# bruniss/multi-task-3d-resencoder-unet

Hardware: AMD Instinct MI355X
Metric: train patches/sec (b,c,z,y,x) ResEncM 1x128^3 (higher is better)
Workload: dtype bf16; 1 GPU; cfg2: ResEncM (6 stages, feats [32, 64, 128, 256, 512, 512], blocks [1, 3, 4, 6, 6, 6]), 1-in, heads ['sheet'], patch 128x128x128, batch 2/GPU, full train step (fwd+loss+bwd+allreduce+clip+AdamW); global_batch=2, parallelism=dp1

## Files before the change

include/rxunet.h:

```cpp
#ifndef RXUNET_H
#define RXUNET_H

#include <stddef.h>
#include <stdint.h>

#ifdef __cplusplus
extern "C" {
#endif

#define RX_OK 0
#define RX_EINVAL (-1)
#define RX_EUNSUPPORTED (-2)
#define RX_ELAUNCH (-3)
#define RX_EWORKSPACE (-4)

typedef enum { RX_F32 = 0, RX_BF16 = 1, RX_F16 = 2 } rx_dtype;
typedef enum { RX_ACT_NONE = 0, RX_ACT_SIGMOID = 1, RX_ACT_SOFTMAX = 2 } rx_head_act;

typedef struct {
  void* ptr;
  int32_t n, z, y, x, c, ld;
  int64_t cs;
} rx_act;

int rx_abi_version(void);
const char* rx_last_error(void);
int rx_device_arch_ok(void);
const char* rx_last_conv_kernel(void);

int rx_pack_conv_weight(rx_dtype dt, const float* w, int co, int ci, int taps, void* w_fwd, void* w_bwd,
                        void* stream);
int rx_pack_convT_weight(rx_dtype dt, const float* w, int ci, int co, int taps, void* w_fwd, void* w_bwd,
                         void* stream);
int rx_pack_multi(rx_dtype dt, int count, const float* const* w, const int* kind, const int* A, const int* B,
                  const int* taps, void* const* w_fwd, void* const* w_bwd, void* stream);

size_t rx_conv_workspace_hint(void);
int rx_conv3d_fwd(rx_dtype dt, const rx_act* x, const void* w_fwd, const float* bias, const rx_act* y,
                  const int32_t kernel[3], const int32_t stride[3], void* ws, size_t ws_bytes, void* stream);
int rx_conv3d_fwd_stats(rx_dtype dt, const rx_act* x, const void* w_fwd, const float* bias, const rx_act* y,
                        const int32_t kernel[3], const int32_t stride[3], float eps, float* stats, void* ws,
                        size_t ws_bytes, void* stream);
int rx_conv3d_bwd_data(rx_dtype dt, const rx_act* dy, const void* w_bwd, const rx_act* dx,
                       const int32_t kernel[3], const int32_t stride[3], int accumulate, void* ws,
                       size_t ws_bytes, void* stream);
int rx_conv3d_bwd_data_instats(rx_dtype dt, const rx_act* dy, const void* w_bwd, const rx_act* dx,
                               const int32_t kernel[3], const int32_t stride[3], int accumulate, const rx_act* in_y,
                               const float* in_stats, float slope, float* m12, int* fused, void* ws, size_t ws_bytes,
                               void* stream);
size_t rx_conv3d_bwd_weight_workspace(const rx_act* x, const rx_act* dy, const int32_t kernel[3]);
int rx_conv3d_bwd_weight(rx_dtype dt, const rx_act* x, const rx_act* dy, float* dw, const int32_t kernel[3],
                         const int32_t stride[3], void* ws, size_t ws_bytes, void* stream);

int rx_convT3d_fwd(rx_dtype dt, const rx_act* x, const void* w_fwd, const float* bias, const rx_act* y,
                   const int32_t stride[3], void* ws, size_t ws_bytes, void* stream);
int rx_convT3d_bwd_data(rx_dtype dt, const rx_act* dy, const void* w_bwd, const rx_act* dx,
                        const int32_t stride[3], int accumulate, void* ws, size_t ws_bytes, void* stream);
size_t rx_convT3d_bwd_weight_workspace(const rx_act* x, const rx_act* dy, const int32_t stride[3]);
int rx_convT3d_bwd_weight(rx_dtype dt, const rx_act* x, const rx_act* dy, float* dw, const int32_t stride[3],
                          void* ws, size_t ws_bytes, void* stream);

size_t rx_instnorm_stats_workspace(const rx_act* y);
int rx_instnorm_stats(rx_dtype dt, const rx_act* y, float eps, float* stats, void* ws, size_t ws_bytes,
                      void* stream);
int rx_instnorm_stats_mask(float* stats, const float* keep, int count, void* stream);
int rx_instnorm_act_fwd(rx_dtype dt, const rx_act* y, const float* stats, const rx_act* residual,
                        const rx_act* out, float slope, void* stream);
int rx_instnorm_fwd(rx_dtype dt, const rx_act* y, float eps, float* stats, const rx_act* residual,
                    const rx_act* out, float slope, void* ws, size_t ws_bytes, void* stream);
int rx_instnorm_act_bwd(rx_dtype dt, const rx_act* g, const rx_act* y, const float* stats, const rx_act* out,
                        float slope, const rx_act* dy, const rx_act* d_residual, int accumulate_residual,
                        void* ws, size_t ws_bytes, void* stream);

int rx_instnorm_act_bwd_res(rx_dtype dt, const rx_act* g, const rx_act* y, const float* stats, const rx_act* out,
                            float slope, const rx_act* pool_dy, const int32_t pool_stride[3], const rx_act* d_residual,
                            const rx_act* dy, void* ws, size_t ws_bytes, void* stream);

int rx_instnorm_act_bwd_apply(rx_dtype dt, const rx_act* g, const rx_act* y, const float* stats, const rx_act* out,
                              float slope, const float* m12, const rx_act* dy, const rx_act* d_residual,
                              int accumulate_residual, void* stream);

typedef struct {
  const float* w1;
  const float* b1;
  const float* w2;
  const float* b2;
  int32_t rd;
  int32_t keep_x;
} rx_se_params;
size_t rx_se_workspace(const rx_act* y);
int rx_se_gate_fwd(rx_dtype dt, const rx_act* y, const float* stats, const float* path_scale, const rx_se_params* se,
                   float* pooled, float* hidden, float* gate, float* mult, void* ws, size_t ws_bytes, void* stream);
int rx_instnorm_gate_act_fwd(rx_dtype dt, const rx_act* y, const float* stats, const float* mult, int keep_x,
                             const rx_act* residual, const rx_act* out, float slope, void* stream);
int rx_se_gate_bwd(rx_dtype dt, const rx_act* g, const rx_act* y, const float* stats, const rx_act* out, float slope,
                   const float* path_scale, const rx_se_params* se, const float* pooled, const float* hidden,
                   const float* gate, const float* mult, float* dadd, float* m12, float* dw1, float* db1, float* dw2,
                   float* db2, void* ws, size_t ws_bytes, void* stream);
int rx_instnorm_gate_act_bwd(rx_dtype dt, const rx_act* g, const rx_act* y, const float* stats, const rx_act* out,
                             float slope, const float* mult, const float* dadd, const float* m12, int keep_x,
                             const rx_act* dy, const rx_act* d_residual, int accumulate_residual, void* stream);

int rx_avgpool_fwd(rx_dtype dt, const rx_act* x, const rx_act* y, const int32_t stride[3], void* stream);
int rx_instnorm_act_pool_fwd(rx_dtype dt, const rx_act* y, const float* stats, const rx_act* residual,
                             const rx_act* out, const rx_act* pooled, const int32_t stride[3], float slope,
                             void* stream);
int rx_avgpool_bwd(rx_dtype dt, const rx_act* dy, const rx_act* dx, const int32_t stride[3], int accumulate,
                   void* stream);

int rx_stem_conv_fwd(rx_dtype dt, const float* x_ncdhw, int n, int cin, int z, int y, int x, const float* w,
                     const float* bias, const rx_act* out, const int32_t kernel[3], void* stream);
int rx_stem_conv_fwd_stats(rx_dtype dt, const float* x_ncdhw, int n, int cin, int z, int y, int x, const float* w,
                           const float* bias, const rx_act* out, const int32_t kernel[3], float eps, float* stats,
                           void* ws, size_t ws_bytes, void* stream);
size_t rx_stem_conv_bwd_weight_workspace(int cin, int cout, int taps);
int rx_stem_conv_bwd_weight(rx_dtype dt, const float* x_ncdhw, int n, int cin, int z, int y, int x,
                            const rx_act* dy, float* dw, const int32_t kernel[3], void* ws, size_t ws_bytes,
                            void* stream);

int rx_head_fwd(rx_dtype dt, const rx_act* x, const float* w, const float* b, int k, float* out_ncdhw,
                int act, void* stream);
size_t rx_head_bwd_workspace(const rx_act* x, int k);
int rx_head_bwd(rx_dtype dt, const float* dout_ncdhw, const rx_act* x, const float* w, int k, const rx_act* dx,
                float* dw, float* db, void* ws, size_t ws_bytes, void* stream);

int rx_instnorm_act_head_fwd(rx_dtype dt, const rx_act* y, const float* stats, const rx_act* out, float slope,
                             const float* head_w, const float* head_b, int k, float* out_ncdhw, int act, void* stream);

int rx_instnorm_act_bwd_head(rx_dtype dt, const float* dout_ncdhw, int k, const float* head_w, const rx_act* y,
                             const float* stats, float slope, const rx_act* dy, float* head_dw, float* head_db, void* ws,
                             size_t ws_bytes, void* stream);

size_t rx_channel_sum_workspace(const rx_act* x);
int rx_channel_sum(rx_dtype dt, const rx_act* x, float* out, void* ws, size_t ws_bytes, void* stream);

size_t rx_loss_workspace(int n, int c, long v);
int rx_bce_dice_loss_fwd(const float* logits, const float* target, int n, int c, long v, float alpha, float beta,
                         float smoothing, float eps, float* loss, float* coef, void* ws, size_t ws_bytes,
                         void* stream);
int rx_bce_dice_loss_bwd(const float* logits, const float* target, int n, int c, long v, float alpha, float beta,
                         float smoothing, const float* coef, const float* grad_loss, float* dlogits, void* stream);
int rx_masked_cosine_loss_fwd(const float* pred, const float* target, int n, int c, long v, float* loss, float* coef,
                              void* ws, size_t ws_bytes, void* stream);
int rx_masked_cosine_loss_bwd(const float* pred, const float* target, int n, int c, long v, const float* coef,
                              const float* grad_loss, float* dpred, void* stream);

int rx_adamw_pack(rx_dtype dt, float* p, const float* grad, float* exp_avg, float* exp_avg_sq, const float* clip, double lr,
                  double beta1, double beta2, double eps, double weight_decay, int step, int kind, int A, int B, int taps,
                  void* w_fwd, void* w_bwd, void* stream);
int rx_adamw_flat(float* p, const float* grad, float* exp_avg, float* exp_avg_sq, const float* clip, double lr, double beta1,
                  double beta2, double eps, double weight_decay, int step, long n, void* stream);
long rx_grad_norm_clip_partials(int count, const long* numel);
int rx_grad_norm_clip(int count, const float* const* grad, const long* numel, float max_norm, float* partial, long partial_len,
                      float* out, void* stream);
int rx_adamw_flat_multi(int count, float* const* p, const float* const* grad, float* const* exp_avg,
                        float* const* exp_avg_sq, const long* numel, const float* clip, double lr, double beta1,
                        double beta2, double eps, double weight_decay, int step, void* stream);

typedef struct rx_prog rx_prog;
rx_prog* rx_prog_create(void);
void rx_prog_destroy(rx_prog* p);
int rx_prog_begin(rx_prog* p, void* const* streams, int n_streams);
int rx_prog_end(rx_prog* p);
int rx_prog_len(const rx_prog* p);
const char* rx_prog_cmd_name(const rx_prog* p, int i);
const char* rx_prog_cmd_kernel(const rx_prog* p, int i);
int rx_prog_cmd_stream(const rx_prog* p, int i);
int rx_prog_run(rx_prog* p, int first, int last, void* const* streams, int n_streams, float* ms);
int rx_event_new(void);
int rx_event_free(int slot);
int rx_event_slots_in_use(void);
int rx_event_record(int slot, void* stream);
int rx_stream_wait(int slot, void* stream);

typedef enum { RX_SW_U8 = 0, RX_SW_U16 = 1, RX_SW_F32 = 2 } rx_sw_in_dtype;
typedef enum { RX_SW_SCALE = 0, RX_SW_ZSCORE = 1 } rx_sw_norm;
typedef enum { RX_SW_BLEND_AVERAGE = 0, RX_SW_BLEND_UNIT = 1, RX_SW_BLEND_NONE = 2 } rx_sw_blend;
typedef enum { RX_SW_CAST_U8 = 0, RX_SW_CAST_U16 = 1 } rx_sw_cast;
size_t rx_sw_gather_workspace(int batch, int cin, int pz, int py, int px);
int rx_sw_gather(int in_dtype, const void* slab, int cin, int ring, int y, int x, int batch, const int32_t* origins, int pz,
                 int py, int px, int norm, float* out, void* ws, size_t ws_bytes, void* stream);
int rx_sw_accumulate(const float* logits, int batch, int valid, int c, int pz, int py, int px, const int32_t* origins, int act,
                     const float* weight, float* sum, float* wsum, int ring, int y, int x, void* stream);
int rx_sw_finalize(float* sum, float* wsum, int c, int ring, int y, int x, int z0, int rows, int blend, int cast, int reset,
                   float* blended, void* final_out, float* wsum_out, void* stream);

#define RX_AUG_MAX_K 21
#define RX_AUG_MAX_BOXES 4
typedef enum { RX_AUG_PW_NONE = 0, RX_AUG_PW_AFFINE = 1, RX_AUG_PW_PLANE = 2, RX_AUG_PW_NOISE = 3 } rx_aug_pw_mode;
typedef enum { RX_AUG_G3_NONE = 0, RX_AUG_G3_FILTER = 1, RX_AUG_G3_DOWNSCALE = 2 } rx_aug_g3_mode;
typedef struct {
  int32_t pw_mode[2];
  float pw_a[2], pw_b[2];
  int32_t pw_off[2];
  uint32_t key_lo, key_hi;
  int32_t g3_mode, k, g3_off;
  int32_t nbox;
  int32_t box[RX_AUG_MAX_BOXES][6];
  float fill;
  int32_t pad_;
} rx_aug_sample;
size_t rx_aug_workspace(int batch, int c, int z, int y, int x);
int rx_aug_pointwise(const float* in, float* out, float* scratch, size_t scratch_bytes, int batch, int c, int z, int y, int x,
                     const rx_aug_sample* host_table, const void* table, long pool_words, void* stream);
int rx_aug_filter_zy(const float* scratch, float* out, int batch, int c, int z, int y, int x, const rx_aug_sample* host_table,
                     const void* table, long pool_words, void* stream);
int rx_aug_philox_u32(uint64_t key, long n, uint32_t* out, void* stream);

typedef struct {
  int32_t src_axis[3];
  int32_t flip[3];
  int32_t ch_src[3];
  int32_t ch_neg[3];
} rx_geom_sample;
int rx_geom_apply(const float* in, float* out, int batch, int c, int z, int y, int x, const rx_geom_sample* host_table,
                  int vector, void* stream);

#ifdef __cplusplus
}
#endif
#endif
```

multi-task-3d-resencoder-unet_amd/csrc/rx_elementwise.hip:

```cpp
#include <stdarg.h>

#include <math.h>

#include "rx_common.h"
#include <cstdlib>

static thread_local char g_err[512] = "";
void rx_set_error(const char* fmt, ...) {
  va_list ap;
  va_start(ap, fmt);
  vsnprintf(g_err, sizeof(g_err), fmt, ap);
  va_end(ap);
}
extern "C" const char* rx_last_error(void) { return g_err; }
static thread_local const char* g_last_kernel = "";
static thread_local int g_note_seq_ = 0;
void rx_note_kernel(const char* name) { g_last_kernel = name; ++g_note_seq_; }
int rx_note_seq(void) { return g_note_seq_; }
extern "C" const char* rx_last_conv_kernel(void) { return g_last_kernel; }
extern "C" int rx_abi_version(void) { return 1; }
extern "C" int rx_device_arch_ok(void) {
  int dev = 0;
  if (hipGetDevice(&dev) != hipSuccess) return 0;
  hipDeviceProp_t p;
// ... 284 lines not shown
  for (; i < total; i += step) {
    long v = i / CV;
    Vec16<T> a = ld16(yn + v * ldy + cv * P);
    Vec16<T> r;
    if (HAS_RES) r = ld16(rn + v * ldr + cv * P);
    Vec16<T> o;
#pragma unroll
    for (int j = 0; j < P; ++j) {
      float f = (Elem<T>::to_f(a.v[j]) - mean[j]) * rstd[j];
      if (HAS_RES) f += Elem<T>::to_f(r.v[j]);
      f = f > 0.f ? f : f * slope;
      o.v[j] = Elem<T>::from_f(f);
    }
    st16(on + v * ldo + cv * P, o);
  }
}

static inline int sweep_grid(long total_vec, int CV) {
  int g = CV, d = 256;
  while (g % 2 == 0 && d > 1) {
    g /= 2;
    d /= 2;
  }
  long want = (total_vec + 256 * 8 - 1) / (256 * 8);
  if (want < 1) want = 1;
  if (want > 2048) want = 2048;
  long G = (want + g - 1) / g * g;
  return (int)G;
}

static int same_geom(const rx_act* a, const rx_act* b) {
  return a->n == b->n && a->z == b->z && a->y == b->y && a->x == b->x && a->c == b->c;
}

extern "C" int rx_instnorm_act_fwd(rx_dtype dt, const rx_act* y, const float* stats, const rx_act* residual,
                                   const rx_act* out, float slope, void* stream) {
  RX_RECORD(stream, [=, y_ = RxActV(y), residual_ = RxActV(residual), out_ = RxActV(out)](void* s) { return rx_instnorm_act_fwd(dt, y_.p(), stats, residual_.p(), out_.p(), slope, s); });
  int rc = check_vec_channels(y, dt, "rx_instnorm_act_fwd(y)");
  if (rc) return rc;
  rc = check_vec_channels(out, dt, "rx_instnorm_act_fwd(out)");
  if (rc) return rc;
  if (!stats || !same_geom(y, out)) RX_FAIL(RX_EINVAL, "rx_instnorm_act_fwd: geometry mismatch / null stats");
  if (residual) {
    rc = check_vec_channels(residual, dt, "rx_instnorm_act_fwd(residual)");
    if (rc) return rc;
    if (!same_geom(y, residual)) RX_FAIL(RX_EINVAL, "rx_instnorm_act_fwd: residual geometry mismatch");
  }
  const long V = rx_act_voxels(y);
  hipStream_t st = (hipStream_t)stream;
  RX_DISPATCH_DTYPE(dt, T, {
    constexpr int P = Elem<T>::PER16;
    int CV = y->c / P;
    int G = sweep_grid(V * CV, CV);
    if (residual)
      hipLaunchKernelGGL((in_act_fwd_kernel<T, true>), dim3(G, y->n), dim3(256), 0, st, (const T*)y->ptr, y->ld, V * y->ld, stats,
                         (const T*)residual->ptr, residual->ld, V * residual->ld, (T*)out->ptr, out->ld, V * out->ld, (int)V,
                         y->c, slope);
    else
      hipLaunchKernelGGL((in_act_fwd_kernel<T, false>), dim3(G, y->n), dim3(256), 0, st, (const T*)y->ptr, y->ld, V * y->ld, stats,
                         (const T*)nullptr, 0, 0L, (T*)out->ptr, out->ld, V * out->ld, (int)V, y->c, slope);
  });
  RX_CHECK_LAUNCH("rx_instnorm_act_fwd");
  return RX_OK;
}

template <typename T>
struct InBwdOp {
  ActView<T> g, y, out;
  const float* stats;
  int C;
  float slope;
  bool use_mask;
  bool mask_xhat;
  float mean[Elem<T>::PER16], rstd[Elem<T>::PER16];
  __device__ inline void prepare(int n, int c0) {
#pragma unroll
    for (int j = 0; j < Elem<T>::PER16; ++j) {
      mean[j] = stats[2 * ((size_t)n * C + c0 + j)];
      rstd[j] = stats[2 * ((size_t)n * C + c0 + j) + 1];
    }
  }
  __device__ inline void accumulate(int n, int v, int c0, float (&acc)[2][Elem<T>::PER16]) const {
    constexpr int P = Elem<T>::PER16;
    Vec16<T> gv = ld16(g.at(n, v, c0));
    Vec16<T> yv = ld16(y.at(n, v, c0));
    Vec16<T> ov;
    if (use_mask) ov = ld16(out.at(n, v, c0));
#pragma unroll
    for (int j = 0; j < P; ++j) {
      float gg = Elem<T>::to_f(gv.v[j]);
      float xh = (Elem<T>::to_f(yv.v[j]) - mean[j]) * rstd[j];
      if (use_mask && !(Elem<T>::to_f(ov.v[j]) > 0.f)) gg *= slope;
      if (mask_xhat && !(xh > 0.f)) gg *= slope;
      acc[0][j] += gg;
      acc[1][j] += gg * xh;
    }
  }
};

template <typename T, bool HAS_DRES, bool ACC_DRES>
__global__ __launch_bounds__(256) void in_act_bwd_apply_kernel(const T* __restrict__ g, int ldg, long sg, const T* __restrict__ y, int ldy,
                                                               long sy, const T* __restrict__ out, int ldo, long so,
                                                               const float* __restrict__ stats, const float* __restrict__ m12,
                                                               T* __restrict__ dy, int lddy, long sdy, T* __restrict__ dres, int lddr,
                                                               long sdr, int V, int C, float slope, int use_mask) {
  constexpr int P = Elem<T>::PER16;
  const int CV = C / P;
  const int n = blockIdx.y;
  const long total = (long)V * CV;
  long i = (long)blockIdx.x * 256 + threadIdx.x;
  const long step = (long)gridDim.x * 256;
  const int cv = (int)(i % CV);
  float mean[P], rstd[P], m1[P], m2[P];
#pragma unroll
  for (int j = 0; j < P; ++j) {
    size_t k = (size_t)n * C + cv * P + j;
    mean[j] = stats[2 * k];
    rstd[j] = stats[2 * k + 1];
    m1[j] = m12[2 * k];
    m2[j] = m12[2 * k + 1];
  }
  for (; i < total; i += step) {
    long v = i / CV;
    Vec16<T> gv = ld16(g + n * sg + v * ldg + cv * P);
    Vec16<T> yv = ld16(y + n * sy + v * ldy + cv * P);
    Vec16<T> ov;
    if (use_mask == 1) ov = ld16(out + n * so + v * ldo + cv * P);
    Vec16<T> dv, rv;
    if (HAS_DRES && ACC_DRES) rv = ld16(dres + n * sdr + v * lddr + cv * P);
#pragma unroll
    for (int j = 0; j < P; ++j) {
      float gg = Elem<T>::to_f(gv.v[j]);
      float xh = (Elem<T>::to_f(yv.v[j]) - mean[j]) * rstd[j];
      if (use_mask == 1 && !(Elem<T>::to_f(ov.v[j]) > 0.f)) gg *= slope;
      if (use_mask == 2 && !(xh > 0.f)) gg *= slope;
      dv.v[j] = Elem<T>::from_f(rstd[j] * (gg - m1[j] - xh * m2[j]));
      if (HAS_DRES) {
        float r = gg;
        if (ACC_DRES) r += Elem<T>::to_f(rv.v[j]);
        rv.v[j] = Elem<T>::from_f(r);
      }
    }
    st16(dy + n * sdy + v * lddy + cv * P, dv);
    if (HAS_DRES) st16(dres + n * sdr + v * lddr + cv * P, rv);
  }
}

#define RX_LAUNCH_APPLY(HD, AD)                                                                                                   \
  hipLaunchKernelGGL((in_act_bwd_apply_kernel<T, HD, AD>), dim3(G, N), dim3(256), 0, st, (const T*)g->ptr, g->ld, V * g->ld,     \
                     (const T*)y->ptr, y->ld, V * y->ld, outp, ldo, V * ldo, stats, (const float*)m12, (T*)dy->ptr, dy->ld,       \
                     V * dy->ld, d_residual ? (T*)d_residual->ptr : (T*)nullptr, d_residual ? d_residual->ld : 0,                 \
                     d_residual ? V * d_residual->ld : 0L, (int)V, C, slope, use_mask ? 1 : (mask_xhat ? 2 : 0))

template <typename T, int G, bool HAS_RES>
__global__ __launch_bounds__(256) void in_small_fwd_kernel(const T* __restrict__ y, int ldy, long sy, const T* __restrict__ res, int ldr,
                                                           long sr, T* __restrict__ out, int ldo, long so, float* __restrict__ stats, int V,
                                                           int C, float eps, float slope) {
  constexpr int P = Elem<T>::PER16;
  constexpr int CPG = G / P;
  __shared__ double red[4][2][G];
  __shared__ float mr[2][G];
  const int tid = threadIdx.x, lane = tid & 63, wave = tid >> 6;
  const int n = blockIdx.y, c0 = blockIdx.x * G;
  const int ck = tid % CPG, vl = tid / CPG;
  const int VL = 256 / CPG;
  const T* yn = y + n * sy + c0 + ck * P;
  float s[P], q[P];
#pragma unroll
  for (int j = 0; j < P; ++j) s[j] = q[j] = 0.f;
  for (int v = vl; v < V; v += VL) {
    Vec16<T> a = ld16(yn + (long)v * ldy);
#pragma unroll
    for (int j = 0; j < P; ++j) {
      float f = Elem<T>::to_f(a.v[j]);
      s[j] += f;
      q[j] += f * f;
    }
  }
  for (int o = CPG; o < 64; o <<= 1) {
#pragma unroll
    for (int j = 0; j < P; ++j) {
      s[j] += __shfl_xor(s[j], o, 64);
      q[j] += __shfl_xor(q[j], o, 64);
    }
  }
  if (lane < CPG) {
#pragma unroll
    for (int j = 0; j < P; ++j) {
      red[wave][0][lane * P + j] = (double)s[j];
      red[wave][1][lane * P + j] = (double)q[j];
    }
  }
  __syncthreads();
  if (tid < G) {
    double s0 = red[0][0][tid] + red[1][0][tid] + red[2][0][tid] + red[3][0][tid];
    double s1 = red[0][1][tid] + red[1][1][tid] + red[2][1][tid] + red[3][1][tid];
    double mean = s0 / V, var = s1 / V - mean * mean;
    if (var < 0.0) var = 0.0;
    float m = (float)mean, r = (float)(1.0 / sqrt(var + (double)eps));
    mr[0][tid] = m;
    mr[1][tid] = r;
    stats[2 * ((size_t)n * C + c0 + tid)] = m;
    stats[2 * ((size_t)n * C + c0 + tid) + 1] = r;
  }
  __syncthreads();
  float mean[P], rstd[P];
#pragma unroll
  for (int j = 0; j < P; ++j) {
    mean[j] = mr[0][ck * P + j];
    rstd[j] = mr[1][ck * P + j];
  }
  const T* rn = HAS_RES ? res + n * sr + c0 + ck * P : nullptr;
  T* on = out + n * so + c0 + ck * P;
  for (int v = vl; v < V; v += VL) {
    Vec16<T> a = ld16(yn + (long)v * ldy);
    Vec16<T> r;
    if (HAS_RES) r = ld16(rn + (long)v * ldr);
    Vec16<T> o;
#pragma unroll
    for (int j = 0; j < P; ++j) {
      float f = (Elem<T>::to_f(a.v[j]) - mean[j]) * rstd[j];
      if (HAS_RES) f += Elem<T>::to_f(r.v[j]);
      f = f > 0.f ? f : f * slope;
      o.v[j] = Elem<T>::from_f(f);
    }
    st16(on + (long)v * ldo, o);
  }
}

template <typename T, int G>
__global__ __launch_bounds__(256) void in_small_bwd_kernel(const T* __restrict__ g, int ldg, long sg, const T* __restrict__ y, int ldy, long sy,
                                                           const T* __restrict__ out, int ldo, long so, const float* __restrict__ stats,
                                                           T* __restrict__ dy, int lddy, long sdy, T* __restrict__ dres, int lddr, long sdr,
                                                           int acc_res, int V, int C, float slope, int mask_mode) {
  constexpr int P = Elem<T>::PER16;
  constexpr int CPG = G / P;
  __shared__ double red[4][2][G];
  __shared__ float mm[2][G];
  const int tid = threadIdx.x, lane = tid & 63, wave = tid >> 6;
  const int n = blockIdx.y, c0 = blockIdx.x * G;
  const int ck = tid % CPG, vl = tid / CPG;
  const int VL = 256 / CPG;
  const long co = c0 + ck * P;
  float mean[P], rstd[P];
#pragma unroll
  for (int j = 0; j < P; ++j) {
    mean[j] = stats[2 * ((size_t)n * C + co + j)];
    rstd[j] = stats[2 * ((size_t)n * C + co + j) + 1];
  }
  auto gprime = [&](int v, float (&gg)[P], float (&xh)[P]) {
    Vec16<T> gv = ld16(g + n * sg + (long)v * ldg + co);
    Vec16<T> yv = ld16(y + n * sy + (long)v * ldy + co);
    Vec16<T> ov;
    if (mask_mode == 1) ov = ld16(out + n * so + (long)v * ldo + co);
#pragma unroll
    for (int j = 0; j < P; ++j) {
      gg[j] = Elem<T>::to_f(gv.v[j]);
      xh[j] = (Elem<T>::to_f(yv.v[j]) - mean[j]) * rstd[j];
      if (mask_mode == 1 && !(Elem<T>::to_f(ov.v[j]) > 0.f)) gg[j] *= slope;
      if (mask_mode == 2 && !(xh[j] > 0.f)) gg[j] *= slope;
    }
  };
  float s[P], q[P];
#pragma unroll
  for (int j = 0; j < P; ++j) s[j] = q[j] = 0.f;
  for (int v = vl; v < V; v += VL) {
    float gg[P], xh[P];
    gprime(v, gg, xh);
#pragma unroll
    for (int j = 0; j < P; ++j) {
      s[j] += gg[j];
      q[j] += gg[j] * xh[j];
    }
  }
  for (int o = CPG; o < 64; o <<= 1) {
#pragma unroll
    for (int j = 0; j < P; ++j) {
      s[j] += __shfl_xor(s[j], o, 64);
      q[j] += __shfl_xor(q[j], o, 64);
    }
  }
  if (lane < CPG) {
#pragma unroll
    for (int j = 0; j < P; ++j) {
      red[wave][0][lane * P + j] = (double)s[j];
      red[wave][1][lane * P + j] = (double)q[j];
    }
  }
  __syncthreads();
  if (tid < G) {
    mm[0][tid] = (float)((red[0][0][tid] + red[1][0][tid] + red[2][0][tid] + red[3][0][tid]) / V);
    mm[1][tid] = (float)((red[0][1][tid] + red[1][1][tid] + red[2][1][tid] + red[3][1][tid]) / V);
  }
  __syncthreads();
  float m1[P], m2[P];
#pragma unroll
  for (int j = 0; j < P; ++j) {
    m1[j] = mm[0][ck * P + j];
    m2[j] = mm[1][ck * P + j];
  }
  for (int v = vl; v < V; v += VL) {
    float gg[P], xh[P];
    gprime(v, gg, xh);
    Vec16<T> dv, rv;
    if (dres && acc_res) rv = ld16(dres + n * sdr + (long)v * lddr + co);
#pragma unroll
    for (int j = 0; j < P; ++j) {
      dv.v[j] = Elem<T>::from_f(rstd[j] * (gg[j] - m1[j] - xh[j] * m2[j]));
      if (dres) {
        float r = gg[j];
        if (acc_res) r += Elem<T>::to_f(rv.v[j]);
        rv.v[j] = Elem<T>::from_f(r);
      }
    }
    st16(dy + n * sdy + (long)v * lddy + co, dv);
    if (dres) st16(dres + n * sdr + (long)v * lddr + co, rv);
  }
}

constexpr long RX_IN_SMALL_MAX_VOXELS = 512;
constexpr long RX_IN_SMALL_NARROW_VOXELS = 256;

extern "C" int rx_instnorm_act_bwd(rx_dtype dt, const rx_act* g, const rx_act* y, const float* stats, const rx_act* out,
                                   float slope, const rx_act* dy, const rx_act* d_residual, int accumulate_residual, void* ws,
                                   size_t ws_bytes, void* stream) {
  RX_RECORD(stream, [=, g_ = RxActV(g), y_ = RxActV(y), out_ = RxActV(out), dy_ = RxActV(dy), d_residual_ = RxActV(d_residual)](void* s) { return rx_instnorm_act_bwd(dt, g_.p(), y_.p(), stats, out_.p(), slope, dy_.p(), d_residual_.p(), accumulate_residual, ws, ws_bytes, s); });
  int rc;
  if ((rc = check_vec_channels(g, dt, "rx_instnorm_act_bwd(g)"))) return rc;
  if ((rc = check_vec_channels(y, dt, "rx_instnorm_act_bwd(y)"))) return rc;
  if ((rc = check_vec_channels(dy, dt, "rx_instnorm_act_bwd(dy)"))) return rc;
  const bool mask_xhat = slope != 1.0f && out == nullptr;
  const bool use_mask = slope != 1.0f && out != nullptr;
  if (use_mask) {
    if ((rc = check_vec_channels(out, dt, "rx_instnorm_act_bwd(out)"))) return rc;
    if (!same_geom(y, out)) RX_FAIL(RX_EINVAL, "rx_instnorm_act_bwd: out geometry mismatch");
  }
  if (d_residual) {
    if ((rc = check_vec_channels(d_residual, dt, "rx_instnorm_act_bwd(d_residual)"))) return rc;
    if (!same_geom(y, d_residual)) RX_FAIL(RX_EINVAL, "rx_instnorm_act_bwd: d_residual geometry mismatch");
  }
  if (!stats || !ws || !same_geom(y, g) || !same_geom(y, dy)) RX_FAIL(RX_EINVAL, "rx_instnorm_act_bwd: bad arguments");
  const long V = rx_act_voxels(y);
  const int N = y->n, C = y->c;
  if (V <= RX_IN_SMALL_MAX_VOXELS && C % 32 == 0) {
    hipStream_t st1 = (hipStream_t)stream;
    const int mode = use_mask ? 1 : (mask_xhat ? 2 : 0);
    const bool narrow = dt != RX_F32 && V >= RX_IN_SMALL_NARROW_VOXELS;
    dim3 grid1(narrow ? C / 8 : C / 32, N);
#define RX_LAUNCH_IN_SMALL_BWD(G)                                                                                                     \
  hipLaunchKernelGGL((in_small_bwd_kernel<T, G>), grid1, dim3(256), 0, st1, (const T*)g->ptr, g->ld, V * g->ld, (const T*)y->ptr, y->ld, \
                     V * y->ld, use_mask ? (const T*)out->ptr : (const T*)nullptr, use_mask ? out->ld : 0,                           \
                     use_mask ? V * out->ld : 0L, stats, (T*)dy->ptr, dy->ld, V * dy->ld,                                             \
                     d_residual ? (T*)d_residual->ptr : (T*)nullptr, d_residual ? d_residual->ld : 0,                                 \
                     d_residual ? V * d_residual->ld : 0L, accumulate_residual, (int)V, C, slope, mode)
    RX_DISPATCH_DTYPE(dt, T, {
      if (narrow) RX_LAUNCH_IN_SMALL_BWD(8);
      else RX_LAUNCH_IN_SMALL_BWD(32);
    });
    RX_CHECK_LAUNCH("rx_instnorm_act_bwd(small)");
    return RX_OK;
  }
  size_t need = rx_reduce_ws_bytes(N, V, C, 2) + (size_t)N * C * 2 * sizeof(float);
  if (ws_bytes < need) RX_FAIL(RX_EWORKSPACE, "rx_instnorm_act_bwd: workspace too small (%zu < %zu)", ws_bytes, need);
  float* partial = (float*)ws;
  float* m12 = (float*)((char*)ws + rx_align_up(rx_reduce_ws_bytes(N, V, C, 2) - 256, 256));
  hipStream_t st = (hipStream_t)stream;
  RX_DISPATCH_DTYPE(dt, T, {
    constexpr int P = Elem<T>::PER16;
    ReducePlan p = rx_reduce_plan(V, C, P);
    int CV = C / P, VP = 256 / CV;
    InBwdOp<T> op{make_view<T>(g), make_view<T>(y), use_mask ? make_view<T>(out) : make_view<T>(y), stats, C, slope, use_mask, mask_xhat, {}, {}};
    size_t lds = (size_t)2 * (VP > 4 ? VP : 4) * C * sizeof(float);
    hipLaunchKernelGGL((colreduce_kernel<T, 2, InBwdOp<T>>), dim3(p.nchunks, N), dim3(256), lds, st, op, (int)V, C, p.chunk_vox,
                       partial);
    fin_launch(st, (const float*)partial, N, p.nchunks, 2, C,
                       (double)V, 0.f, (int)FIN_MEAN2, m12);
    int G = sweep_grid(V * CV, CV);
    const T* outp = use_mask ? (const T*)out->ptr : nullptr;
    int ldo = use_mask ? out->ld : 0;
    if (!d_residual)
      RX_LAUNCH_APPLY(false, false);
    else if (accumulate_residual)
      RX_LAUNCH_APPLY(true, true);
    else
      RX_LAUNCH_APPLY(true, false);
  });
  RX_CHECK_LAUNCH("rx_instnorm_act_bwd");
  return RX_OK;
}


template <typename T, bool POOL>
struct InBwdResOp {
  ActView<T> g, y, out, pool;
  T* gp;
  long gp_ss;
  int gp_ld;
  const float* stats;
  int C;
  float slope;
  int Yi, Xi, Yo, Xo, fz, fy, fx;
  float inv;
  float mean[Elem<T>::PER16], rstd[Elem<T>::PER16];
  __device__ inline void prepare(int n, int c0) {
#pragma unroll
    for (int j = 0; j < Elem<T>::PER16; ++j) {
      mean[j] = stats[2 * ((size_t)n * C + c0 + j)];
      rstd[j] = stats[2 * ((size_t)n * C + c0 + j) + 1];
    }
  }
  __device__ inline void accumulate(int n, int v, int c0, float (&acc)[2][Elem<T>::PER16]) const {
    constexpr int P = Elem<T>::PER16;
    Vec16<T> gv = ld16(g.at(n, v, c0));
    Vec16<T> yv = ld16(y.at(n, v, c0));
    Vec16<T> ov = ld16(out.at(n, v, c0));
    Vec16<T> pv;
    if (POOL) {
      const int xi = v % Xi, t = v / Xi;
      const int yi = t % Yi, zi = t / Yi;
      const int vo = ((zi / fz) * Yo + (yi / fy)) * Xo + (xi / fx);
      pv = ld16(pool.at(n, vo, c0));
    }
    Vec16<T> w;
#pragma unroll
    for (int j = 0; j < P; ++j) {
      float gg = Elem<T>::to_f(gv.v[j]);
      if (POOL) gg += Elem<T>::to_f(pv.v[j]) * inv;
      if (!(Elem<T>::to_f(ov.v[j]) > 0.f)) gg *= slope;
      w.v[j] = Elem<T>::from_f(gg);
      gg = Elem<T>::to_f(w.v[j]);
      const float xh = (Elem<T>::to_f(yv.v[j]) - mean[j]) * rstd[j];
      acc[0][j] += gg;
      acc[1][j] += gg * xh;
    }
    st16(gp + n * gp_ss + (long)v * gp_ld + c0, w);
  }
};

static int check_pool(const rx_act* big, const rx_act* small, const int32_t f[3], const char* who);

extern "C" int rx_instnorm_act_bwd_res(rx_dtype dt, const rx_act* g, const rx_act* y, const float* stats, const rx_act* out, float slope,
                                       const rx_act* pool_dy, const int32_t pool_stride[3], const rx_act* d_residual, const rx_act* dy,
                                       void* ws, size_t ws_bytes, void* stream) {
  static const int32_t one3[3] = {1, 1, 1};
  if (!pool_stride) pool_stride = one3;
  RX_RECORD(stream, [=, g_ = RxActV(g), y_ = RxActV(y), out_ = RxActV(out), pool_dy_ = RxActV(pool_dy), pool_stride_ = RxI3V(pool_stride), d_residual_ = RxActV(d_residual), dy_ = RxActV(dy)](void* s) { return rx_instnorm_act_bwd_res(dt, g_.p(), y_.p(), stats, out_.p(), slope, pool_dy_.p(), pool_stride_.v, d_residual_.p(), dy_.p(), ws, ws_bytes, s); });
  int rc;
  if ((rc = check_vec_channels(g, dt, "rx_instnorm_act_bwd_res(g)"))) return rc;
  if ((rc = check_vec_channels(y, dt, "rx_instnorm_act_bwd_res(y)"))) return rc;
  if ((rc = check_vec_channels(out, dt, "rx_instnorm_act_bwd_res(out)"))) return rc;
  if ((rc = check_vec_channels(dy, dt, "rx_instnorm_act_bwd_res(dy)"))) return rc;
  if ((rc = check_vec_channels(d_residual, dt, "rx_instnorm_act_bwd_res(d_residual)"))) return rc;
  if (!stats || !ws || !same_geom(y, g) || !same_geom(y, dy) || !same_geom(y, out) || !same_geom(y, d_residual))
    RX_FAIL(RX_EINVAL, "rx_instnorm_act_bwd_res: bad arguments");
  if (d_residual->ptr == dy->ptr) RX_FAIL(RX_EINVAL, "rx_instnorm_act_bwd_res: d_residual and dy must be different buffers");
  if (pool_dy) {
    if ((rc = check_vec_channels(pool_dy, dt, "rx_instnorm_act_bwd_res(pool_dy)"))) return rc;
    if ((rc = check_pool(y, pool_dy, pool_stride, "rx_instnorm_act_bwd_res"))) return rc;
  }
  const long V = rx_act_voxels(y);
  const int N = y->n, C = y->c;
  size_t need = rx_reduce_ws_bytes(N, V, C, 2) + (size_t)N * C * 2 * sizeof(float);
  if (ws_bytes < need) RX_FAIL(RX_EWORKSPACE, "rx_instnorm_act_bwd_res: workspace too small (%zu < %zu)", ws_bytes, need);
  float* partial = (float*)ws;
  float* m12 = (float*)((char*)ws + rx_align_up(rx_reduce_ws_bytes(N, V, C, 2) - 256, 256));
  hipStream_t st = (hipStream_t)stream;
  RX_DISPATCH_DTYPE(dt, T, {
    constexpr int P = Elem<T>::PER16;
    ReducePlan p = rx_reduce_plan(V, C, P);
    int CV = C / P, VP = 256 / CV;
    size_t lds = (size_t)2 * (VP > 4 ? VP : 4) * C * sizeof(float);
    if (pool_dy) {
      InBwdResOp<T, true> op{make_view<T>(g), make_view<T>(y), make_view<T>(out), make_view<T>(pool_dy), (T*)d_residual->ptr,
                             V * (long)d_residual->ld, d_residual->ld, stats, C, slope, y->y, y->x, pool_dy->y, pool_dy->x,
                             pool_stride[0], pool_stride[1], pool_stride[2], 1.f / (float)(pool_stride[0] * pool_stride[1] * pool_stride[2]), {}, {}};
      hipLaunchKernelGGL((colreduce_kernel<T, 2, InBwdResOp<T, true>>), dim3(p.nchunks, N), dim3(256), lds, st, op, (int)V, C, p.chunk_vox, partial);
    } else {
      InBwdResOp<T, false> op{make_view<T>(g), make_view<T>(y), make_view<T>(out), make_view<T>(y), (T*)d_residual->ptr,
                              V * (long)d_residual->ld, d_residual->ld, stats, C, slope, y->y, y->x, 1, 1, 1, 1, 1, 1.f, {}, {}};
      hipLaunchKernelGGL((colreduce_kernel<T, 2, InBwdResOp<T, false>>), dim3(p.nchunks, N), dim3(256), lds, st, op, (int)V, C, p.chunk_vox, partial);
    }
    fin_launch(st, (const float*)partial, N, p.nchunks, 2, C, (double)V, 0.f, (int)FIN_MEAN2, m12);
    int G = sweep_grid(V * CV, CV);
    hipLaunchKernelGGL((in_act_bwd_apply_kernel<T, false, false>), dim3(G, N), dim3(256), 0, st, (const T*)d_residual->ptr, d_residual->ld,
                       V * d_residual->ld, (const T*)y->ptr, y->ld, V * y->ld, (const T*)nullptr, 0, 0L, stats, (const float*)m12,
                       (T*)dy->ptr, dy->ld, V * dy->ld, (T*)nullptr, 0, 0L, (int)V, C, slope, 0);
  });
  RX_CHECK_LAUNCH("rx_instnorm_act_bwd_res");
  return RX_OK;
}

__global__ __launch_bounds__(256) void inbwd_fused_finalize(const float* __restrict__ partial, int N, int nchunks, int C, double V,
                                                            const float* __restrict__ stats, float* __restrict__ m12) {
  const int lane = threadIdx.x & 63;
  const int i = blockIdx.x * 4 + (threadIdx.x >> 6);
  if (i >= N * C) return;
  const int n = i / C, c = i - n * C;
  double s0 = 0.0, s1 = 0.0;
  for (int k = lane; k < nchunks; k += 64) {
    const float* p = partial + ((size_t)(n * nchunks + k) * 2) * C + c;
    s0 += (double)p[0];
    s1 += (double)p[C];
  }
  s0 = wave_sum_d(s0);
  s1 = wave_sum_d(s1);
  if (lane != 0) return;
  m12[2 * i] = (float)(s0 / V);
  m12[2 * i + 1] = (float)((double)stats[2 * i + 1] * s1 / V);
}
void rx_inbwd_fused_finalize_launch(const float* partial, int N, int nchunks, int C, double V, const float* stats, float* m12, hipStream_t st) {
  hipLaunchKernelGGL(inbwd_fused_finalize, dim3((N * C + 3) / 4), dim3(256), 0, st, partial, N, nchunks, C, V, stats, m12);
}

extern "C" int rx_instnorm_act_bwd_apply(rx_dtype dt, const rx_act* g, const rx_act* y, const float* stats, const rx_act* out, float slope,
                                         const float* m12, const rx_act* dy, const rx_act* d_residual, int accumulate_residual,
                                         void* stream) {
  RX_RECORD(stream, [=, g_ = RxActV(g), y_ = RxActV(y), out_ = RxActV(out), dy_ = RxActV(dy), d_residual_ = RxActV(d_residual)](void* s) { return rx_instnorm_act_bwd_apply(dt, g_.p(), y_.p(), stats, out_.p(), slope, m12, dy_.p(), d_residual_.p(), accumulate_residual, s); });
  int rc;
  if ((rc = check_vec_channels(g, dt, "rx_instnorm_act_bwd_apply(g)"))) return rc;
  if ((rc = check_vec_channels(y, dt, "rx_instnorm_act_bwd_apply(y)"))) return rc;
  if ((rc = check_vec_channels(dy, dt, "rx_instnorm_act_bwd_apply(dy)"))) return rc;
  const bool mask_xhat = slope != 1.0f && out == nullptr;
  const bool use_mask = slope != 1.0f && out != nullptr;
  if (use_mask) {
    if ((rc = check_vec_channels(out, dt, "rx_instnorm_act_bwd_apply(out)"))) return rc;
    if (!same_geom(y, out)) RX_FAIL(RX_EINVAL, "rx_instnorm_act_bwd_apply: out geometry mismatch");
  }
  if (d_residual) {
    if ((rc = check_vec_channels(d_residual, dt, "rx_instnorm_act_bwd_apply(d_residual)"))) return rc;
    if (!same_geom(y, d_residual)) RX_FAIL(RX_EINVAL, "rx_instnorm_act_bwd_apply: d_residual geometry mismatch");
  }
  if (!stats || !m12 || !same_geom(y, g) || !same_geom(y, dy)) RX_FAIL(RX_EINVAL, "rx_instnorm_act_bwd_apply: bad arguments");
  const long V = rx_act_voxels(y);
  const int N = y->n, C = y->c;
  hipStream_t st = (hipStream_t)stream;
  RX_DISPATCH_DTYPE(dt, T, {
    constexpr int P = Elem<T>::PER16;
    int CV = C / P;
    int G = sweep_grid(V * CV, CV);
    const T* outp = use_mask ? (const T*)out->ptr : nullptr;
    int ldo = use_mask ? out->ld : 0;
    if (!d_residual)
      RX_LAUNCH_APPLY(false, false);
    else if (accumulate_residual)
      RX_LAUNCH_APPLY(true, true);
    else
      RX_LAUNCH_APPLY(true, false);
  });
  RX_CHECK_LAUNCH("rx_instnorm_act_bwd_apply");
  return RX_OK;
}

extern "C" int rx_instnorm_fwd(rx_dtype dt, const rx_act* y, float eps, float* stats, const rx_act* residual, const rx_act* out,
                               float slope, void* ws, size_t ws_bytes, void* stream) {
  RX_RECORD(stream, [=, y_ = RxActV(y), residual_ = RxActV(residual), out_ = RxActV(out)](void* s) { return rx_instnorm_fwd(dt, y_.p(), eps, stats, residual_.p(), out_.p(), slope, ws, ws_bytes, s); });
  int rc;
  if ((rc = check_vec_channels(y, dt, "rx_instnorm_fwd(y)"))) return rc;
  const long V = rx_act_voxels(y);
  if (V > RX_IN_SMALL_MAX_VOXELS || y->c % 32) {
    if ((rc = rx_instnorm_stats(dt, y, eps, stats, ws, ws_bytes, stream))) return rc;
    return rx_instnorm_act_fwd(dt, y, stats, residual, out, slope, stream);
  }
  if ((rc = check_vec_channels(out, dt, "rx_instnorm_fwd(out)"))) return rc;
  if (!stats || !same_geom(y, out)) RX_FAIL(RX_EINVAL, "rx_instnorm_fwd: geometry mismatch / null stats");
  if (residual) {
    if ((rc = check_vec_channels(residual, dt, "rx_instnorm_fwd(residual)"))) return rc;
    if (!same_geom(y, residual)) RX_FAIL(RX_EINVAL, "rx_instnorm_fwd: residual geometry mismatch");
  }
  hipStream_t st = (hipStream_t)stream;
  const bool narrow = dt != RX_F32 && V >= RX_IN_SMALL_NARROW_VOXELS;
  dim3 grid(narrow ? y->c / 8 : y->c / 32, y->n);
#define RX_LAUNCH_IN_SMALL_FWD(G, RES)                                                                                              \
  hipLaunchKernelGGL((in_small_fwd_kernel<T, G, RES>), grid, dim3(256), 0, st, (const T*)y->ptr, y->ld, V * y->ld,                  \
                     RES ? (const T*)residual->ptr : (const T*)nullptr, RES ? residual->ld : 0, RES ? V * residual->ld : 0L,         \
                     (T*)out->ptr, out->ld, V * out->ld, stats, (int)V, y->c, eps, slope)
  RX_DISPATCH_DTYPE(dt, T, {
    if (residual && narrow) RX_LAUNCH_IN_SMALL_FWD(8, true);
    else if (residual) RX_LAUNCH_IN_SMALL_FWD(32, true);
    else if (narrow) RX_LAUNCH_IN_SMALL_FWD(8, false);
    else RX_LAUNCH_IN_SMALL_FWD(32, false);
  });
  RX_CHECK_LAUNCH("rx_instnorm_fwd");
  return RX_OK;
}

template <typename T>
__global__ __launch_bounds__(256) void avgpool_fwd_kernel(const T* __restrict__ x, int ldx, long sx, T* __restrict__ y, int ldy, long sy,
                                                          int Zo, int Yo, int Xo, int Yi, int Xi, int C, int fz, int fy, int fx) {
  constexpr int P = Elem<T>::PER16;
  const int CV = C / P;
  const int n = blockIdx.y;
  const long total = (long)Zo * Yo * Xo * CV;
  const float inv = 1.f / (float)(fz * fy * fx);
  for (long i = (long)blockIdx.x * 256 + threadIdx.x; i < total; i += (long)gridDim.x * 256) {
    int cv = (int)(i % CV);
    long vo = i / CV;
    int xo = (int)(vo % Xo);
    int yo = (int)((vo / Xo) % Yo);
    int zo = (int)(vo / ((long)Xo * Yo));
    float acc[P];
#pragma unroll
    for (int j = 0; j < P; ++j) acc[j] = 0.f;
    for (int a = 0; a < fz; ++a)
      for (int b = 0; b < fy; ++b)
        for (int c = 0; c < fx; ++c) {
          long vi = ((long)(zo * fz + a) * Yi + (yo * fy + b)) * Xi + (xo * fx + c);
          Vec16<T> t = ld16(x + n * sx + vi * ldx + cv * P);
#pragma unroll
          for (int j = 0; j < P; ++j) acc[j] += Elem<T>::to_f(t.v[j]);
        }
    Vec16<T> o;
#pragma unroll
    for (int j = 0; j < P; ++j) o.v[j] = Elem<T>::from_f(acc[j] * inv);
    st16(y + n * sy + vo * ldy + cv * P, o);
  }
}

template <typename T, bool ACC>
__global__ __launch_bounds__(256) void avgpool_bwd_kernel(const T* __restrict__ dy, int ldy, long sy, T* __restrict__ dx, int ldx, long sx,
                                                          int Zi, int Yi, int Xi, int Yo, int Xo, int C, int fz, int fy, int fx) {
  constexpr int P = Elem<T>::PER16;
  const int CV = C / P;
  const int n = blockIdx.y;
  const long total = (long)Zi * Yi * Xi * CV;
  const float inv = 1.f / (float)(fz * fy * fx);
  for (long i = (long)blockIdx.x * 256 + threadIdx.x; i < total; i += (long)gridDim.x * 256) {
    int cv = (int)(i % CV);
    long vi = i / CV;
    int xi = (int)(vi % Xi);
    int yi = (int)((vi / Xi) % Yi);
    int zi = (int)(vi / ((long)Xi * Yi));
    long vo = ((long)(zi / fz) * Yo + (yi / fy)) * Xo + (xi / fx);
    Vec16<T> t = ld16(dy + n * sy + vo * ldy + cv * P);
    Vec16<T> o;
    if (ACC) o = ld16(dx + n * sx + vi * ldx + cv * P);
#pragma unroll
    for (int j = 0; j < P; ++j) {
      float f = Elem<T>::to_f(t.v[j]) * inv;
      if (ACC) f += Elem<T>::to_f(o.v[j]);
      o.v[j] = Elem<T>::from_f(f);
    }
    st16(dx + n * sx + vi * ldx + cv * P, o);
  }
}

static int check_pool(const rx_act* big, const rx_act* small, const int32_t f[3], const char* who) {
  for (int i = 0; i < 3; ++i)
    if (f[i] < 1 || f[i] > RX_MAX_STRIDE) RX_FAIL(RX_EUNSUPPORTED, "%s: pool factor must be 1..%d per axis", who, RX_MAX_STRIDE);
  if (big->n != small->n || big->c != small->c || big->z != small->z * f[0] || big->y != small->y * f[1] || big->x != small->x * f[2])
    RX_FAIL(RX_EINVAL, "%s: geometry mismatch (%d,%d,%d)/(%d,%d,%d)", who, big->z, big->y, big->x, small->z, small->y, small->x);
  return RX_OK;
}

extern "C" int rx_avgpool_fwd(rx_dtype dt, const rx_act* x, const rx_act* y, const int32_t stride[3], void* stream) {
  RX_RECORD(stream, [=, x_ = RxActV(x), y_ = RxActV(y), stride_ = RxI3V(stride)](void* s) { return rx_avgpool_fwd(dt, x_.p(), y_.p(), stride_.v, s); });
  int rc;
  if ((rc = check_vec_channels(x, dt, "rx_avgpool_fwd(x)"))) return rc;
  if ((rc = check_vec_channels(y, dt, "rx_avgpool_fwd(y)"))) return rc;
  if ((rc = check_pool(x, y, stride, "rx_avgpool_fwd"))) return rc;
  hipStream_t st = (hipStream_t)stream;
  RX_DISPATCH_DTYPE(dt, T, {
    constexpr int P = Elem<T>::PER16;
    long total = rx_act_voxels(y) * (y->c / P);
    int G = (int)((total + 255) / 256 > 4096 ? 4096 : (total + 255) / 256);
    hipLaunchKernelGGL((avgpool_fwd_kernel<T>), dim3(G, x->n), dim3(256), 0, st, (const T*)x->ptr, x->ld, rx_act_voxels(x) * x->ld,
                       (T*)y->ptr, y->ld, rx_act_voxels(y) * y->ld, y->z, y->y, y->x, x->y, x->x, x->c, stride[0], stride[1], stride[2]);
  });
  RX_CHECK_LAUNCH("rx_avgpool_fwd");
  return RX_OK;
}

template <typename T, bool HAS_RES>
__global__ __launch_bounds__(256) void in_act_pool_fwd_kernel(const T* __restrict__ y, int ldy, long sy, const float* __restrict__ stats,
                                                              const T* __restrict__ res, int ldr, long sr, T* __restrict__ out, int ldo, long so,
                                                              T* __restrict__ pooled, int ldp, long sp, int Zo, int Yo, int Xo, int Yi, int Xi,
                                                              int C, int fz, int fy, int fx, float slope) {
  constexpr int P = Elem<T>::PER16;
  const int CV = C / P, n = blockIdx.y;
  const long total = (long)Zo * Yo * Xo * CV, step = (long)gridDim.x * 256;
  long i = (long)blockIdx.x * 256 + threadIdx.x;
  const int cv = (int)(i % CV);
  float mean[P], rstd[P];
#pragma unroll
  for (int j = 0; j < P; ++j) {
    mean[j] = stats[2 * ((size_t)n * C + cv * P + j)];
    rstd[j] = stats[2 * ((size_t)n * C + cv * P + j) + 1];
  }
  const float inv = 1.f / (float)(fz * fy * fx);
  for (; i < total; i += step) {
    const long vo = i / CV;
    const int xo = (int)(vo % Xo), yo = (int)((vo / Xo) % Yo), zo = (int)(vo / ((long)Xo * Yo));
    float acc[P];
#pragma unroll
    for (int j = 0; j < P; ++j) acc[j] = 0.f;
    for (int a = 0; a < fz; ++a)
      for (int b = 0; b < fy; ++b)
        for (int c = 0; c < fx; ++c) {
          const long vi = ((long)(zo * fz + a) * Yi + (yo * fy + b)) * Xi + (xo * fx + c);
          Vec16<T> t = ld16(y + n * sy + vi * ldy + cv * P), r, o;
          if (HAS_RES) r = ld16(res + n * sr + vi * ldr + cv * P);
#pragma unroll
          for (int j = 0; j < P; ++j) {
            float f = (Elem<T>::to_f(t.v[j]) - mean[j]) * rstd[j];
            if (HAS_RES) f += Elem<T>::to_f(r.v[j]);
            f = f > 0.f ? f : f * slope;
            o.v[j] = Elem<T>::from_f(f);
            acc[j] += Elem<T>::to_f(o.v[j]);
          }
          st16(out + n * so + vi * ldo + cv * P, o);
        }
    Vec16<T> p;
#pragma unroll
    for (int j = 0; j < P; ++j) p.v[j] = Elem<T>::from_f(acc[j] * inv);
    st16(pooled + n * sp + vo * ldp + cv * P, p);
  }
}

extern "C" int rx_instnorm_act_pool_fwd(rx_dtype dt, const rx_act* y, const float* stats, const rx_act* residual, const rx_act* out,
                                        const rx_act* pooled, const int32_t stride[3], float slope, void* stream) {
  RX_RECORD(stream, [=, y_ = RxActV(y), residual_ = RxActV(residual), out_ = RxActV(out), pooled_ = RxActV(pooled), stride_ = RxI3V(stride)](void* s) { return rx_instnorm_act_pool_fwd(dt, y_.p(), stats, residual_.p(), out_.p(), pooled_.p(), stride_.v, slope, s); });
  int rc;
  if ((rc = check_vec_channels(y, dt, "rx_instnorm_act_pool_fwd(y)"))) return rc;
  if ((rc = check_vec_channels(out, dt, "rx_instnorm_act_pool_fwd(out)"))) return rc;
  if ((rc = check_vec_channels(pooled, dt, "rx_instnorm_act_pool_fwd(pooled)"))) return rc;
  if (!stats || !same_geom(y, out)) RX_FAIL(RX_EINVAL, "rx_instnorm_act_pool_fwd: geometry mismatch / null stats");
  if ((rc = check_pool(out, pooled, stride, "rx_instnorm_act_pool_fwd"))) return rc;
  if (residual) {
    if ((rc = check_vec_channels(residual, dt, "rx_instnorm_act_pool_fwd(residual)"))) return rc;
    if (!same_geom(y, residual)) RX_FAIL(RX_EINVAL, "rx_instnorm_act_pool_fwd: residual geometry mismatch");
  }
  const long V = rx_act_voxels(y), Vp = rx_act_voxels(pooled);
  hipStream_t st = (hipStream_t)stream;
  RX_DISPATCH_DTYPE(dt, T, {
    constexpr int P = Elem<T>::PER16;
    const int CV = y->c / P;
// ... 1404 lines not shown
```

multi-task-3d-resencoder-unet_amd/csrc/rx_igemm.hip:

```cpp
#include <stdlib.h>

#include "rx_common.h"


struct IgemmPhase {
  int Qz, Qy, Qx, Vq;
  int opz, opy, opx;
  int tap0, ntaps;
  int mtile0, mtiles;
  long slab_off;
};

struct IgemmGeom {
  int Zi, Yi, Xi, Ci, ldi;
  long in_ss;
  int isz, isy, isx;
  int Zo, Yo, Xo, Co, ldo;
  long out_ss;
  int osz, osy, osx;
  int accumulate, ksplit, nph, total_mtiles;
  IgemmPhase ph[8];
  RxTap taps[RX_MAX_TAPS];
};

// ... 198 lines not shown
  u32x4* sX = reinterpret_cast<u32x4*>(smem_f);
  u32x4* sW = sX + BM * KC;

  const int tid = threadIdx.x, lane = tid & 63, wave = tid >> 6;
  const int mtiles = (NV + BM - 1) / BM;
  const int lid = rx_xcd_remap(blockIdx.y * gridDim.x + blockIdx.x, gridDim.x * gridDim.y);
  const int mtile = lid % mtiles, rest = lid / mtiles;
  const int split = rest % g.ksplit, n0 = (rest / g.ksplit) * BN;
  const IgemmPhase P_ = g.ph[0];
  const int chunk = tid & 15, rbase = tid >> 4;

  int gz[XP], gy[XP], gx[XP];
  long gbase[XP];
  bool rok[XP];
#pragma unroll
  for (int p = 0; p < XP; ++p) {
    const int Q = mtile * BM + rbase + 16 * p;
    rok[p] = Q < NV;
    const int n = Q / P_.Vq, q = Q - n * P_.Vq;
    const int qx = q % P_.Qx, t = q / P_.Qx;
    const int qy = t % P_.Qy, qz = t / P_.Qy;
    gz[p] = qz * g.isz, gy[p] = qy * g.isy, gx[p] = qx * g.isx;
    gbase[p] = (long)n * g.in_ss + chunk * P;
  }
  const int nkc = g.Ci / KE;
  const int st_begin = (int)((long)nsteps_total * split / g.ksplit);
  const int st_end = (int)((long)nsteps_total * (split + 1) / g.ksplit);

  u32x4 xr[XP], wr[WP];
  int xo[XP], wo = 0, cur_tap = -1;
  auto load_step = [&](int st) {
    const int tap = st / nkc, cc = st - tap * nkc;
    if (tap != cur_tap) {
      cur_tap = tap;
      const RxTap tp = g.taps[P_.tap0 + tap];
#pragma unroll
      for (int p = 0; p < XP; ++p) {
        const int z = gz[p] + tp.dz, y = gy[p] + tp.dy, x = gx[p] + tp.dx;
        const bool ok = rok[p] & ((unsigned)z < (unsigned)g.Zi) & ((unsigned)y < (unsigned)g.Yi) & ((unsigned)x < (unsigned)g.Xi);
        xo[p] = ok ? (int)(gbase[p] + ((long)(z * g.Yi + y) * g.Xi + x) * g.ldi) : -1;
      }
      wo = (int)(((long)tp.w * g.Co + n0 + rbase) * g.Ci + chunk * P);
    }
    const int ko = cc * KE;
    if (ABL & 1) {
#pragma unroll
      for (int p = 0; p < XP; ++p) xr[p] = u32x4{(unsigned)(xo[p] + ko), 1u, 2u, 3u};
#pragma unroll
      for (int p = 0; p < WP; ++p) wr[p] = u32x4{(unsigned)(wo + ko), 1u, 2u, 3u};
      return;
    }
#pragma unroll
    for (int p = 0; p < XP; ++p) {
      const int o = xo[p] < 0 ? 0 : xo[p] + ko;
      const u32x4 v = *reinterpret_cast<const u32x4*>(in + o);
      xr[p] = xo[p] < 0 ? u32x4{0u, 0u, 0u, 0u} : v;
    }
#pragma unroll
    for (int p = 0; p < WP; ++p) wr[p] = *reinterpret_cast<const u32x4*>(w + wo + (long)(16 * p) * g.Ci + ko);
  };
  auto store_step = [&]() {
    if (ABL & 4) {
      if (xr[0][0] == 0x7fffffffu && wr[0][0] == 0x7ffffffeu) sX[0] = xr[1];
      return;
    }
#pragma unroll
    for (int p = 0; p < XP; ++p) {
      const int row = rbase + 16 * p;
      sX[row * KC + (chunk ^ (row & 15))] = xr[p];
    }
#pragma unroll
    for (int p = 0; p < WP; ++p) {
      const int row = rbase + 16 * p;
      sW[row * KC + (chunk ^ (row & 15))] = wr[p];
    }
  };

  f32x16 acc[2];
#pragma unroll
  for (int a = 0; a < 2; ++a)
#pragma unroll
    for (int r = 0; r < 16; ++r) acc[a][r] = 0.f;

  const int fr = lane & 31, fh = lane >> 5;
  const int vrow = wave * 32 + lane_voxel_ig(fr);
  const u32x4* xrow = sX + vrow * KC;
  const u32x4* wrow0 = sW + fr * KC;
  const u32x4* wrow1 = sW + (32 + fr) * KC;
  const int xm = vrow & 15, wm = fr & 15;

  if (st_begin < st_end) load_step(st_begin);
  for (int st = st_begin; st < st_end; ++st) {
    __syncthreads();
    store_step();
    __syncthreads();
    if (st + 1 < st_end) load_step(st + 1);
#pragma unroll
    for (int ks = 0; ks < KC / 2; ++ks) {
      const int c = ks * 2 + fh;
      u32x4 b, a0, a1;
      if (ABL & 4) {
        b = u32x4{(unsigned)c, (unsigned)st, 2u, 3u}, a0 = b, a1 = b;
      } else {
        b = xrow[c ^ xm];
        a0 = wrow0[c ^ wm], a1 = wrow1[c ^ wm];
      }
      if (ABL & 2) {
        acc[0][ks] += __builtin_bit_cast(float, a0[0] ^ b[1]);
        acc[1][ks] += __builtin_bit_cast(float, a1[2] ^ b[3]);
      } else {
        Mma<T>::run(acc[0], a0, b);
        Mma<T>::run(acc[1], a1, b);
      }
    }
  }

  const int Q = mtile * BM + vrow;
  if (Q < NV) {
    float* sp = slab + ((long)split * NV + Q) * g.Co + n0;
#pragma unroll
    for (int a = 0; a < 2; ++a)
#pragma unroll
      for (int g4 = 0; g4 < 4; ++g4) {
        f32x4 v = {acc[a][4 * g4], acc[a][4 * g4 + 1], acc[a][4 * g4 + 2], acc[a][4 * g4 + 3]};
        *reinterpret_cast<f32x4*>(sp + a * 32 + 8 * g4 + 4 * fh) = v;
      }
  }
}


template <typename T>
static void igemm_dispatch_tile(int BM, int BN, dim3 grid, hipStream_t st, const void* in, const void* w, const float* bias, void* out,
                                void* ws, const IgemmGeom& g, int N, int ks) {
  rx_note_kernel(BM == 256 ? (BN == 64 ? "igemm_kernel<256,64>" : "igemm_kernel<256,32>")
                            : (BN == 64 ? "igemm_kernel<128,64>" : "igemm_kernel<128,32>"));
  if (BM == 256 && BN == 64)
    hipLaunchKernelGGL((igemm_kernel<T, 256, 64>), grid, dim3(256), 0, st, (const T*)in, (const T*)w, bias, (T*)out, (float*)ws, g);
  else if (BM == 256 && BN == 32)
    hipLaunchKernelGGL((igemm_kernel<T, 256, 32>), grid, dim3(256), 0, st, (const T*)in, (const T*)w, bias, (T*)out, (float*)ws, g);
  else if (BM == 128 && BN == 64)
    hipLaunchKernelGGL((igemm_kernel<T, 128, 64>), grid, dim3(256), 0, st, (const T*)in, (const T*)w, bias, (T*)out, (float*)ws, g);
  else
    hipLaunchKernelGGL((igemm_kernel<T, 128, 32>), grid, dim3(256), 0, st, (const T*)in, (const T*)w, bias, (T*)out, (float*)ws, g);
  if (ks > 1) {
    int vmax = 0;
    for (int i = 0; i < g.nph; ++i) vmax = g.ph[i].Vq > vmax ? g.ph[i].Vq : vmax;
    long total = (long)N * vmax * (g.Co / 4);
    int G = (int)((total + 255) / 256 > 2048 ? 2048 : (total + 255) / 256);
    hipLaunchKernelGGL((igemm_splitk_reduce<T>), dim3(G, g.nph), dim3(256), 0, st, (const float*)ws, bias, (T*)out, g, N);
  }
}

static int igemm_launch(rx_dtype dt, const void* in, const void* w, const float* bias, void* out, IgemmGeom& g, int N, void* ws,
                        size_t ws_bytes, hipStream_t st) {
  const int per16 = dt == RX_F32 ? 4 : 8;
  const int KB = 4 * per16;
  if (g.Ci % KB) RX_FAIL(RX_EUNSUPPORTED, "igemm: input channels must be a multiple of %d (got %d)", KB, g.Ci);
  if (g.Co % 32) RX_FAIL(RX_EUNSUPPORTED, "igemm: output channels must be a multiple of 32 (got %d)", g.Co);
  if (g.ldi % per16 || g.ldo % 4 || ((uintptr_t)in & 15) || ((uintptr_t)out & 7) || ((uintptr_t)w & 15))
    RX_FAIL(RX_EUNSUPPORTED, "igemm: misaligned operand (ldi=%d ldo=%d)", g.ldi, g.ldo);
  int vmax = 0, nkt_max = 0;
  for (int i = 0; i < g.nph; ++i) {
    vmax = g.ph[i].Vq > vmax ? g.ph[i].Vq : vmax;
    nkt_max = g.ph[i].ntaps > nkt_max ? g.ph[i].ntaps : nkt_max;
  }
  nkt_max *= g.Ci / KB;
  if (vmax <= 0 || g.nph <= 0) return RX_OK;
  {
    const int KE = 16 * per16;
    const long NV = (long)N * g.ph[0].Vq;
    if (dt != RX_F32 && g.nph == 1 && g.Ci % KE == 0 && g.Co % 64 == 0 && NV <= 2048 && ws &&
        g.ph[0].ntaps * (g.Ci / KE) >= 8 && g.ph[0].opz == 0 && g.ph[0].opy == 0 && g.ph[0].opx == 0 && g.osz == 1 && g.osy == 1 &&
        g.osx == 1) {
      const int mtiles = (int)((NV + 127) / 128);
      const int nsteps = g.ph[0].ntaps * (g.Ci / KE);
      const long base_wgs = (long)mtiles * (g.Co / 64);
      int ks = (int)((512 + base_wgs - 1) / base_wgs);
      if (ks > nsteps / 4) ks = nsteps / 4;
      if (ks < 1) ks = 1;
      while (ks > 1 && (size_t)ks * NV * g.Co * sizeof(float) > ws_bytes) --ks;
      if ((size_t)ks * NV * g.Co * sizeof(float) <= ws_bytes) {
        g.ksplit = ks;
        g.total_mtiles = mtiles;
        g.ph[0].mtile0 = 0, g.ph[0].mtiles = mtiles, g.ph[0].slab_off = 0;
        const size_t lds = (size_t)(128 + 64) * 256;
        rx_note_kernel("igemm_fat_kernel");
        dim3 grid(mtiles * ks, g.Co / 64);
        if (dt == RX_BF16) {
          (void)hipFuncSetAttribute(reinterpret_cast<const void*>(&igemm_fat_kernel<bf16_t>), hipFuncAttributeMaxDynamicSharedMemorySize, (int)lds);
#if RX_ABLATION
          {
            static const int abl = rx_env_mask("RX_FAT_ABL");
#define RX_FAT_L(A)                                                                                                                     \
  case A:                                                                                                                               \
    (void)hipFuncSetAttribute(reinterpret_cast<const void*>(&igemm_fat_kernel<bf16_t, A>), hipFuncAttributeMaxDynamicSharedMemorySize, (int)lds); \
    hipLaunchKernelGGL((igemm_fat_kernel<bf16_t, A>), grid, dim3(256), lds, st, (const bf16_t*)in, (const bf16_t*)w, (float*)ws, g, (int)NV, nsteps); \
    break;
            switch (abl) {
              RX_FAT_L(1) RX_FAT_L(2) RX_FAT_L(3) RX_FAT_L(4) RX_FAT_L(5) RX_FAT_L(6) RX_FAT_L(7)
              default:
                hipLaunchKernelGGL((igemm_fat_kernel<bf16_t>), grid, dim3(256), lds, st, (const bf16_t*)in, (const bf16_t*)w, (float*)ws, g, (int)NV, nsteps);
            }
#undef RX_FAT_L
          }
#else
          hipLaunchKernelGGL((igemm_fat_kernel<bf16_t>), grid, dim3(256), lds, st, (const bf16_t*)in, (const bf16_t*)w, (float*)ws, g, (int)NV, nsteps);
#endif
        } else {
          (void)hipFuncSetAttribute(reinterpret_cast<const void*>(&igemm_fat_kernel<f16_t>), hipFuncAttributeMaxDynamicSharedMemorySize, (int)lds);
          hipLaunchKernelGGL((igemm_fat_kernel<f16_t>), grid, dim3(256), lds, st, (const f16_t*)in, (const f16_t*)w, (float*)ws, g, (int)NV, nsteps);
        }
        const long total = NV * (g.Co / 4);
        const int G = (int)((total + 255) / 256 > 2048 ? 2048 : (total + 255) / 256);
        RX_DISPATCH_DTYPE(dt, T, hipLaunchKernelGGL((igemm_splitk_reduce<T>), dim3(G, 1), dim3(256), 0, st, (const float*)ws, bias, (T*)out, g, N));
        RX_CHECK_LAUNCH("igemm_fat");
        return RX_OK;
      }
    }
  }
  const int BN = (g.Co % 64 == 0) ? 64 : 32;
  const int BM = (vmax <= 128) ? 128 : 256;
  g.total_mtiles = 0;
  long vsum = 0;
  for (int i = 0; i < g.nph; ++i) {
    g.ph[i].mtile0 = g.total_mtiles;
    g.ph[i].mtiles = (g.ph[i].Vq + BM - 1) / BM;
    g.total_mtiles += g.ph[i].mtiles;
    vsum += g.ph[i].Vq;
  }
  const long wgs = (long)g.total_mtiles * (g.Co / BN) * N;
  int ks = 1;
  if (wgs < 192 && nkt_max >= 16 && ws) {
    ks = (int)((512 + wgs - 1) / wgs);
    if (ks > nkt_max / 4) ks = nkt_max / 4;
    if (ks > 32) ks = 32;
    size_t need = (size_t)ks * N * vsum * g.Co * sizeof(float);
    while (ks > 1 && need > ws_bytes) {
      --ks;
      need = (size_t)ks * N * vsum * g.Co * sizeof(float);
    }
    if (ks < 1) ks = 1;
  }
  long off = 0;
  for (int i = 0; i < g.nph; ++i) {
    g.ph[i].slab_off = off;
    off += (long)ks * N * g.ph[i].Vq * g.Co;
  }
  g.ksplit = ks;
  dim3 grid(g.total_mtiles * ks, g.Co / BN, N);
  RX_DISPATCH_DTYPE(dt, T, igemm_dispatch_tile<T>(BM, BN, grid, st, in, w, bias, out, ws, g, N, ks));
  RX_CHECK_LAUNCH("igemm");
  return RX_OK;
}

int rx_conv_halo_try(rx_dtype dt, const rx_act* in, const void* w, const float* bias, const rx_act* out, int flip, int accumulate,
                     hipStream_t st, float* stat_part, size_t stat_bytes, int* stat_chunks, const RxBwdStat* bs);
void rx_inbwd_fused_finalize_launch(const float* partial, int N, int nchunks, int C, double V, const float* stats, float* m12, hipStream_t st);
int rx_pointwise_try(rx_dtype dt, const rx_act* in, const void* w, const float* bias, const rx_act* out, const int32_t stride[3],
                     int accumulate, hipStream_t st);
int rx_dgrad_s2_halo_try(rx_dtype dt, const rx_act* dy, const void* w_bwd, const rx_act* dx, int accumulate, hipStream_t st);
void rx_stats_finalize_launch(const float* partial, int N, int nchunks, int C, double V, float eps, float* stats, hipStream_t st);
static bool is_333_s1(const int32_t k[3], const int32_t s[3]) {
  return k[0] == 3 && k[1] == 3 && k[2] == 3 && s[0] == 1 && s[1] == 1 && s[2] == 1;
}

static int check13(const int32_t k[3], const int32_t s[3], const char* who) {
  for (int i = 0; i < 3; ++i) {
    if (k[i] < 1 || k[i] > RX_MAX_KERNEL) RX_FAIL(RX_EUNSUPPORTED, "%s: kernel sizes must be 1..%d per axis (got %d)", who, RX_MAX_KERNEL, k[i]);
    if (s[i] < 1 || s[i] > RX_MAX_STRIDE) RX_FAIL(RX_EUNSUPPORTED, "%s: strides must be 1..%d per axis (got %d)", who, RX_MAX_STRIDE, s[i]);
  }
  return RX_OK;
}
static int conv_out_dim(int in, int k, int s) { return (in + 2 * ((k - 1) / 2) - k) / s + 1; }

static void geom_in(IgemmGeom& g, const rx_act* a) {
  g.Zi = a->z, g.Yi = a->y, g.Xi = a->x, g.Ci = a->c, g.ldi = a->ld;
  g.in_ss = rx_act_voxels(a) * (long)a->ld;
}
static void geom_out(IgemmGeom& g, const rx_act* a) {
  g.Zo = a->z, g.Yo = a->y, g.Xo = a->x, g.Co = a->c, g.ldo = a->ld;
  g.out_ss = rx_act_voxels(a) * (long)a->ld;
}

extern "C" int rx_conv3d_fwd(rx_dtype dt, const rx_act* x, const void* w_fwd, const float* bias, const rx_act* y,
                             const int32_t kernel[3], const int32_t stride[3], void* ws, size_t wsb, void* stream) {
  RX_RECORD(stream, [=, x_ = RxActV(x), y_ = RxActV(y), kernel_ = RxI3V(kernel), stride_ = RxI3V(stride)](void* s) { return rx_conv3d_fwd(dt, x_.p(), w_fwd, bias, y_.p(), kernel_.v, stride_.v, ws, wsb, s); });
  if (!rx_act_ok_planar(x) || !rx_act_ok(y) || !w_fwd) RX_FAIL(RX_EINVAL, "rx_conv3d_fwd: bad arguments");
  int rc = check13(kernel, stride, "rx_conv3d_fwd");
  if (rc) return rc;
  if (y->n != x->n || y->z != conv_out_dim(x->z, kernel[0], stride[0]) || y->y != conv_out_dim(x->y, kernel[1], stride[1]) ||
      y->x != conv_out_dim(x->x, kernel[2], stride[2]))
    RX_FAIL(RX_EINVAL, "rx_conv3d_fwd: output geometry mismatch");
  if (is_333_s1(kernel, stride)) {
    rc = rx_conv_halo_try(dt, x, w_fwd, bias, y, 0, 0, (hipStream_t)stream, nullptr, 0, nullptr, nullptr);
    if (rc < 0) return rc;
    if (rc == 1) return RX_OK;
  }
  if (x->cs) RX_FAIL(RX_EUNSUPPORTED, "rx_conv3d_fwd: a planar-concat input needs the 3x3x3 stride-1 halo kernel (Co = 32, X >= 16)");
  if (kernel[0] == 1 && kernel[1] == 1 && kernel[2] == 1 && stride[0] == 1 && stride[1] == 1 && stride[2] == 1) {
    const int32_t one[3] = {1, 1, 1};
    if (rx_pointwise_try(dt, x, w_fwd, bias, y, one, 0, (hipStream_t)stream) == 1) {
      RX_CHECK_LAUNCH("rx_conv3d_fwd(pointwise)");
      return RX_OK;
    }
  }
  IgemmGeom g;
  memset(&g, 0, sizeof(g));
  geom_in(g, x);
  geom_out(g, y);
  g.nph = 1;
  IgemmPhase& P = g.ph[0];
  P.Qz = y->z, P.Qy = y->y, P.Qx = y->x, P.Vq = (int)rx_act_voxels(y);
  g.isz = stride[0], g.isy = stride[1], g.isx = stride[2];
  g.osz = g.osy = g.osx = 1;
  const int pz = (kernel[0] - 1) / 2, py = (kernel[1] - 1) / 2, px = (kernel[2] - 1) / 2;
  for (int a = 0; a < kernel[0]; ++a)
    for (int b = 0; b < kernel[1]; ++b)
      for (int c = 0; c < kernel[2]; ++c) {
        RxTap& t = g.taps[P.ntaps];
        t.dz = (int8_t)(a - pz), t.dy = (int8_t)(b - py), t.dx = (int8_t)(c - px);
        t.w = (uint16_t)P.ntaps;
        ++P.ntaps;
      }
  return igemm_launch(dt, x->ptr, w_fwd, bias, y->ptr, g, x->n, ws, wsb, (hipStream_t)stream);
}

extern "C" int rx_conv3d_bwd_data_instats(rx_dtype dt, const rx_act* dy, const void* w_bwd, const rx_act* dx, const int32_t kernel[3],
                                          const int32_t stride[3], int accumulate, const rx_act* in_y, const float* in_stats, float slope,
                                          float* m12, int* fused, void* ws, size_t wsb, void* stream) {
  RX_RECORD(stream, [=, dy_ = RxActV(dy), dx_ = RxActV(dx), kernel_ = RxI3V(kernel), stride_ = RxI3V(stride), in_y_ = RxActV(in_y)](void* s) { int fused_dummy = 0; return rx_conv3d_bwd_data_instats(dt, dy_.p(), w_bwd, dx_.p(), kernel_.v, stride_.v, accumulate, in_y_.p(), in_stats, slope, m12, &fused_dummy, ws, wsb, s); });
  if (!fused || !m12 || !in_stats || !rx_act_ok(in_y) || !ws) RX_FAIL(RX_EINVAL, "rx_conv3d_bwd_data_instats: bad arguments");
  *fused = 0;
  if (!rx_act_ok(dy) || !rx_act_ok(dx) || !w_bwd) RX_FAIL(RX_EINVAL, "rx_conv3d_bwd_data_instats: bad arguments");
  int rc = check13(kernel, stride, "rx_conv3d_bwd_data_instats");
  if (rc) return rc;
  const bool same = in_y->n == dx->n && in_y->z == dx->z && in_y->y == dx->y && in_y->x == dx->x && in_y->c == dx->c;
  if (same && is_333_s1(kernel, stride) && dx->z == dy->z && dx->y == dy->y && dx->x == dy->x && in_y->ld % 4 == 0 &&
      !((uintptr_t)in_y->ptr & 7)) {
    RxBwdStat bs{in_y, in_stats, slope};
    int chunks = 0;
    rc = rx_conv_halo_try(dt, dy, w_bwd, nullptr, dx, 1, accumulate, (hipStream_t)stream, (float*)ws, wsb, &chunks, &bs);
    if (rc < 0) return rc;
    if (rc == 1) {
      if (chunks > 0) {
        rx_inbwd_fused_finalize_launch((const float*)ws, dx->n, chunks, dx->c, (double)rx_act_voxels(dx), in_stats, m12, (hipStream_t)stream);
        hipError_t e = hipGetLastError();
        if (e != hipSuccess) RX_FAIL(RX_ELAUNCH, "rx_conv3d_bwd_data_instats(finalize): %s", hipGetErrorString(e));
        *fused = 1;
      }
      return RX_OK;
    }
  }
  return rx_conv3d_bwd_data(dt, dy, w_bwd, dx, kernel, stride, accumulate, ws, wsb, stream);
}

extern "C" int rx_conv3d_fwd_stats(rx_dtype dt, const rx_act* x, const void* w_fwd, const float* bias, const rx_act* y,
                                   const int32_t kernel[3], const int32_t stride[3], float eps, float* stats, void* ws, size_t wsb,
                                   void* stream) {
  RX_RECORD(stream, [=, x_ = RxActV(x), y_ = RxActV(y), kernel_ = RxI3V(kernel), stride_ = RxI3V(stride)](void* s) { return rx_conv3d_fwd_stats(dt, x_.p(), w_fwd, bias, y_.p(), kernel_.v, stride_.v, eps, stats, ws, wsb, s); });
  if (!rx_act_ok_planar(x) || !rx_act_ok(y) || !w_fwd || !stats || !ws) RX_FAIL(RX_EINVAL, "rx_conv3d_fwd_stats: bad arguments");
  int rc = check13(kernel, stride, "rx_conv3d_fwd_stats");
  if (rc) return rc;
  if (is_333_s1(kernel, stride) && y->n == x->n && y->z == x->z && y->y == x->y && y->x == x->x) {
    int chunks = 0;
    rc = rx_conv_halo_try(dt, x, w_fwd, bias, y, 0, 0, (hipStream_t)stream, (float*)ws, wsb, &chunks, nullptr);
    if (rc < 0) return rc;
    if (rc == 1 && chunks > 0) {
      rx_stats_finalize_launch((const float*)ws, y->n, chunks, y->c, (double)rx_act_voxels(y), eps, stats, (hipStream_t)stream);
      hipError_t e = hipGetLastError();
      if (e != hipSuccess) RX_FAIL(RX_ELAUNCH, "rx_conv3d_fwd_stats(finalize): %s", hipGetErrorString(e));
      return RX_OK;
    }
    if (rc == 1) return rx_instnorm_stats(dt, y, eps, stats, ws, wsb, stream);
  }
  rc = rx_conv3d_fwd(dt, x, w_fwd, bias, y, kernel, stride, ws, wsb, stream);
  if (rc) return rc;
  return rx_instnorm_stats(dt, y, eps, stats, ws, wsb, stream);
}

extern "C" int rx_conv3d_bwd_data(rx_dtype dt, const rx_act* dy, const void* w_bwd, const rx_act* dx, const int32_t kernel[3],
                                  const int32_t stride[3], int accumulate, void* ws, size_t wsb, void* stream) {
  RX_RECORD(stream, [=, dy_ = RxActV(dy), dx_ = RxActV(dx), kernel_ = RxI3V(kernel), stride_ = RxI3V(stride)](void* s) { return rx_conv3d_bwd_data(dt, dy_.p(), w_bwd, dx_.p(), kernel_.v, stride_.v, accumulate, ws, wsb, s); });
  if (!rx_act_ok(dy) || !rx_act_ok_planar(dx) || !w_bwd) RX_FAIL(RX_EINVAL, "rx_conv3d_bwd_data: bad arguments");
  int rc = check13(kernel, stride, "rx_conv3d_bwd_data");
  if (rc) return rc;
  if (dy->n != dx->n || dy->z != conv_out_dim(dx->z, kernel[0], stride[0]) || dy->y != conv_out_dim(dx->y, kernel[1], stride[1]) ||
      dy->x != conv_out_dim(dx->x, kernel[2], stride[2]))
    RX_FAIL(RX_EINVAL, "rx_conv3d_bwd_data: geometry mismatch");
  if (is_333_s1(kernel, stride)) {
    rc = rx_conv_halo_try(dt, dy, w_bwd, nullptr, dx, 1, accumulate, (hipStream_t)stream, nullptr, 0, nullptr, nullptr);
    if (rc < 0) return rc;
    if (rc == 1) return RX_OK;
  }
  if (dx->cs) RX_FAIL(RX_EUNSUPPORTED, "rx_conv3d_bwd_data: a planar-concat dx needs the wave-specialised 64-channel halo kernel");
  if (kernel[0] == 1 && kernel[1] == 1 && kernel[2] == 1 && stride[0] == 1 && stride[1] == 1 && stride[2] == 1) {
    const int32_t one[3] = {1, 1, 1};
    if (rx_pointwise_try(dt, dy, w_bwd, nullptr, dx, one, accumulate, (hipStream_t)stream) == 1) {
      RX_CHECK_LAUNCH("rx_conv3d_bwd_data(pointwise)");
      return RX_OK;
    }
  }
  if (kernel[0] == 3 && kernel[1] == 3 && kernel[2] == 3 && stride[0] == 2 && stride[1] == 2 && stride[2] == 2) {
    rc = rx_dgrad_s2_halo_try(dt, dy, w_bwd, dx, accumulate, (hipStream_t)stream);
    if (rc < 0) return rc;
    if (rc == 1) return RX_OK;
  }
  const int k[3] = {kernel[0], kernel[1], kernel[2]}, s[3] = {stride[0], stride[1], stride[2]};
  const int p[3] = {(k[0] - 1) / 2, (k[1] - 1) / 2, (k[2] - 1) / 2};
  const int din[3] = {dx->z, dx->y, dx->x};
  IgemmGeom g;
  auto reset = [&]() {
    memset(&g, 0, sizeof(g));
    geom_in(g, dy);
    geom_out(g, dx);
    g.isz = g.isy = g.isx = 1;
    g.osz = s[0], g.osy = s[1], g.osx = s[2];
    g.accumulate = accumulate;
  };
  reset();
  int ntap_total = 0;
  for (int r0 = 0; r0 < s[0]; ++r0)
    for (int r1 = 0; r1 < s[1]; ++r1)
      for (int r2 = 0; r2 < s[2]; ++r2) {
        const int r[3] = {r0, r1, r2};
        int Q[3];
        for (int a = 0; a < 3; ++a) Q[a] = (din[a] - r[a] + s[a] - 1) / s[a];
        if (Q[0] * Q[1] * Q[2] <= 0) continue;
        int cnt = 0;
        for (int a = 0; a < k[0]; ++a)
          if ((r0 + p[0] - a) % s[0] == 0)
            for (int b = 0; b < k[1]; ++b)
              if ((r1 + p[1] - b) % s[1] == 0)
                for (int c = 0; c < k[2]; ++c)
                  if ((r2 + p[2] - c) % s[2] == 0) ++cnt;
        if (g.nph == 8 || ntap_total + cnt > RX_MAX_TAPS) {
          rc = igemm_launch(dt, dy->ptr, w_bwd, nullptr, dx->ptr, g, dx->n, ws, wsb, (hipStream_t)stream);
          if (rc) return rc;
          reset();
          ntap_total = 0;
        }
        IgemmPhase& P = g.ph[g.nph++];
        P.Qz = Q[0], P.Qy = Q[1], P.Qx = Q[2], P.Vq = Q[0] * Q[1] * Q[2];
        P.opz = r0, P.opy = r1, P.opx = r2;
        P.tap0 = ntap_total;
        for (int a = 0; a < k[0]; ++a) {
          if ((r0 + p[0] - a) % s[0]) continue;
          for (int b = 0; b < k[1]; ++b) {
            if ((r1 + p[1] - b) % s[1]) continue;
            for (int c = 0; c < k[2]; ++c) {
              if ((r2 + p[2] - c) % s[2]) continue;
              RxTap& t = g.taps[ntap_total++];
              t.dz = (int8_t)((r0 + p[0] - a) / s[0]);
              t.dy = (int8_t)((r1 + p[1] - b) / s[1]);
              t.dx = (int8_t)((r2 + p[2] - c) / s[2]);
              t.w = (uint16_t)((a * k[1] + b) * k[2] + c);
              ++P.ntaps;
            }
          }
        }
      }
  return igemm_launch(dt, dy->ptr, w_bwd, nullptr, dx->ptr, g, dx->n, ws, wsb, (hipStream_t)stream);
}

static int checkT(const int32_t s[3], const rx_act* small, const rx_act* big, const char* who) {
  for (int i = 0; i < 3; ++i)
    if (s[i] < 1 || s[i] > RX_MAX_STRIDE) RX_FAIL(RX_EUNSUPPORTED, "%s: strides must be 1..%d per axis", who, RX_MAX_STRIDE);
  if (small->n != big->n || big->z != small->z * s[0] || big->y != small->y * s[1] || big->x != small->x * s[2])
    RX_FAIL(RX_EINVAL, "%s: geometry mismatch", who);
  return RX_OK;
}

extern "C" int rx_convT3d_fwd(rx_dtype dt, const rx_act* x, const void* w_fwd, const float* bias, const rx_act* y,
                              const int32_t stride[3], void* ws, size_t wsb, void* stream) {
  RX_RECORD(stream, [=, x_ = RxActV(x), y_ = RxActV(y), stride_ = RxI3V(stride)](void* s) { return rx_convT3d_fwd(dt, x_.p(), w_fwd, bias, y_.p(), stride_.v, ws, wsb, s); });
  if (!rx_act_ok(x) || !rx_act_ok(y) || !w_fwd) RX_FAIL(RX_EINVAL, "rx_convT3d_fwd: bad arguments");
  int rc = checkT(stride, x, y, "rx_convT3d_fwd");
  if (rc) return rc;
  if (rx_pointwise_try(dt, x, w_fwd, bias, y, stride, 0, (hipStream_t)stream) == 1) {
    RX_CHECK_LAUNCH("rx_convT3d_fwd(pointwise)");
    return RX_OK;
  }
  IgemmGeom g;
  auto reset = [&]() {
    memset(&g, 0, sizeof(g));
    geom_in(g, x);
    geom_out(g, y);
    g.isz = g.isy = g.isx = 1;
    g.osz = stride[0], g.osy = stride[1], g.osx = stride[2];
  };
  reset();
  for (int a = 0; a < stride[0]; ++a)
    for (int b = 0; b < stride[1]; ++b)
      for (int c = 0; c < stride[2]; ++c) {
        if (g.nph == 8) {
          rc = igemm_launch(dt, x->ptr, w_fwd, bias, y->ptr, g, x->n, ws, wsb, (hipStream_t)stream);
          if (rc) return rc;
          reset();
        }
        IgemmPhase& P = g.ph[g.nph];
        P.Qz = x->z, P.Qy = x->y, P.Qx = x->x, P.Vq = (int)rx_act_voxels(x);
        P.opz = a, P.opy = b, P.opx = c;
        P.tap0 = g.nph, P.ntaps = 1;
        RxTap& t = g.taps[g.nph];
        t.dz = t.dy = t.dx = 0;
        t.w = (uint16_t)((a * stride[1] + b) * stride[2] + c);
        ++g.nph;
      }
  return igemm_launch(dt, x->ptr, w_fwd, bias, y->ptr, g, x->n, ws, wsb, (hipStream_t)stream);
}

extern "C" int rx_convT3d_bwd_data(rx_dtype dt, const rx_act* dy, const void* w_bwd, const rx_act* dx, const int32_t stride[3],
                                   int accumulate, void* ws, size_t wsb, void* stream) {
  RX_RECORD(stream, [=, dy_ = RxActV(dy), dx_ = RxActV(dx), stride_ = RxI3V(stride)](void* s) { return rx_convT3d_bwd_data(dt, dy_.p(), w_bwd, dx_.p(), stride_.v, accumulate, ws, wsb, s); });
  if (!rx_act_ok(dy) || !rx_act_ok(dx) || !w_bwd) RX_FAIL(RX_EINVAL, "rx_convT3d_bwd_data: bad arguments");
  int rc = checkT(stride, dx, dy, "rx_convT3d_bwd_data");
  if (rc) return rc;
  IgemmGeom g;
  memset(&g, 0, sizeof(g));
  geom_in(g, dy);
  geom_out(g, dx);
  g.nph = 1;
  IgemmPhase& P = g.ph[0];
  P.Qz = dx->z, P.Qy = dx->y, P.Qx = dx->x, P.Vq = (int)rx_act_voxels(dx);
  g.isz = stride[0], g.isy = stride[1], g.isx = stride[2];
  g.osz = g.osy = g.osx = 1;
  g.accumulate = accumulate;
  for (int a = 0; a < stride[0]; ++a)
    for (int b = 0; b < stride[1]; ++b)
      for (int c = 0; c < stride[2]; ++c) {
        RxTap& t = g.taps[P.ntaps];
        t.dz = (int8_t)a, t.dy = (int8_t)b, t.dx = (int8_t)c;
        t.w = (uint16_t)P.ntaps;
        ++P.ntaps;
      }
  return igemm_launch(dt, dy->ptr, w_bwd, nullptr, dx->ptr, g, dx->n, ws, wsb, (hipStream_t)stream);
}

extern "C" size_t rx_conv_workspace_hint(void) { return (size_t)96 << 20; }
```

multi-task-3d-resencoder-unet_amd/engine/lib.py:

```python
import ctypes
import os
from ctypes import POINTER, c_char_p, c_double, c_float, c_int, c_int32, c_long, c_size_t, c_void_p

import torch

_HERE = os.path.dirname(os.path.abspath(__file__))
LIB_PATH = os.environ.get("RX_LIBRARY") or os.path.join(os.path.dirname(_HERE), "csrc", "librxunet.so")

RX_F32, RX_BF16, RX_F16 = 0, 1, 2
RX_ACT_NONE, RX_ACT_SIGMOID, RX_ACT_SOFTMAX = 0, 1, 2
DTYPE_CODE = {torch.float32: RX_F32, torch.bfloat16: RX_BF16, torch.float16: RX_F16}
RX_SW_U8, RX_SW_U16, RX_SW_F32 = 0, 1, 2
RX_SW_SCALE, RX_SW_ZSCORE = 0, 1
RX_SW_BLEND_AVERAGE, RX_SW_BLEND_UNIT, RX_SW_BLEND_NONE = 0, 1, 2
RX_SW_CAST_U8, RX_SW_CAST_U16 = 0, 1
RX_AUG_PW_NONE, RX_AUG_PW_AFFINE, RX_AUG_PW_PLANE, RX_AUG_PW_NOISE = 0, 1, 2, 3
RX_AUG_G3_NONE, RX_AUG_G3_FILTER, RX_AUG_G3_DOWNSCALE = 0, 1, 2
RX_AUG_MAX_K, RX_AUG_MAX_BOXES = 21, 4


class RxError(RuntimeError):
    pass


class RxAct(ctypes.Structure):
    _fields_ = [("ptr", c_void_p), ("n", c_int32), ("z", c_int32), ("y", c_int32), ("x", c_int32),
                ("c", c_int32), ("ld", c_int32), ("cs", ctypes.c_int64)]


class RxSeParams(ctypes.Structure):
    _fields_ = [("w1", c_void_p), ("b1", c_void_p), ("w2", c_void_p), ("b2", c_void_p), ("rd", c_int32),
                ("keep_x", c_int32)]


I3 = c_int32 * 3
_P = POINTER(RxAct)
_PSE = POINTER(RxSeParams)

_SIGNATURES = {
    "rx_abi_version": (c_int, []),
    "rx_last_error": (c_char_p, []),
    "rx_device_arch_ok": (c_int, []),
    "rx_last_conv_kernel": (c_char_p, []),
    "rx_pack_conv_weight": (c_int, [c_int, c_void_p, c_int, c_int, c_int, c_void_p, c_void_p, c_void_p]),
    "rx_pack_convT_weight": (c_int, [c_int, c_void_p, c_int, c_int, c_int, c_void_p, c_void_p, c_void_p]),
    "rx_pack_multi": (c_int, [c_int, c_int, c_void_p, c_void_p, c_void_p, c_void_p, c_void_p, c_void_p, c_void_p, c_void_p]),
    "rx_conv_workspace_hint": (c_size_t, []),
    "rx_conv3d_fwd": (c_int, [c_int, _P, c_void_p, c_void_p, _P, I3, I3, c_void_p, c_size_t, c_void_p]),
    "rx_conv3d_fwd_stats": (c_int, [c_int, _P, c_void_p, c_void_p, _P, I3, I3, c_float, c_void_p, c_void_p, c_size_t, c_void_p]),
    "rx_conv3d_bwd_data": (c_int, [c_int, _P, c_void_p, _P, I3, I3, c_int, c_void_p, c_size_t, c_void_p]),
    "rx_conv3d_bwd_data_instats": (c_int, [c_int, _P, c_void_p, _P, I3, I3, c_int, _P, c_void_p, c_float, c_void_p, POINTER(c_int),
                                           c_void_p, c_size_t, c_void_p]),
    "rx_instnorm_act_bwd_apply": (c_int, [c_int, _P, _P, c_void_p, _P, c_float, c_void_p, _P, _P, c_int, c_void_p]),
    "rx_conv3d_bwd_weight_workspace": (c_size_t, [_P, _P, I3]),
    "rx_conv3d_bwd_weight": (c_int, [c_int, _P, _P, c_void_p, I3, I3, c_void_p, c_size_t, c_void_p]),
    "rx_convT3d_fwd": (c_int, [c_int, _P, c_void_p, c_void_p, _P, I3, c_void_p, c_size_t, c_void_p]),
    "rx_convT3d_bwd_data": (c_int, [c_int, _P, c_void_p, _P, I3, c_int, c_void_p, c_size_t, c_void_p]),
    "rx_convT3d_bwd_weight_workspace": (c_size_t, [_P, _P, I3]),
    "rx_convT3d_bwd_weight": (c_int, [c_int, _P, _P, c_void_p, I3, c_void_p, c_size_t, c_void_p]),
    "rx_instnorm_stats_workspace": (c_size_t, [_P]),
    "rx_instnorm_stats": (c_int, [c_int, _P, c_float, c_void_p, c_void_p, c_size_t, c_void_p]),
    "rx_instnorm_act_fwd": (c_int, [c_int, _P, c_void_p, _P, _P, c_float, c_void_p]),
    "rx_instnorm_stats_mask": (c_int, [c_void_p, c_void_p, c_int, c_void_p]),
    "rx_instnorm_fwd": (c_int, [c_int, _P, c_float, c_void_p, _P, _P, c_float, c_void_p, c_size_t, c_void_p]),
    "rx_instnorm_act_bwd": (c_int, [c_int, _P, _P, c_void_p, _P, c_float, _P, _P, c_int, c_void_p, c_size_t,
                                    c_void_p]),
    "rx_instnorm_act_bwd_res": (c_int, [c_int, _P, _P, c_void_p, _P, c_float, _P, I3, _P, _P, c_void_p, c_size_t, c_void_p]),
    "rx_se_workspace": (c_size_t, [_P]),
    "rx_se_gate_fwd": (c_int, [c_int, _P, c_void_p, c_void_p, _PSE, c_void_p, c_void_p, c_void_p, c_void_p, c_void_p, c_size_t,
                               c_void_p]),
    "rx_instnorm_gate_act_fwd": (c_int, [c_int, _P, c_void_p, c_void_p, c_int, _P, _P, c_float, c_void_p]),
    "rx_se_gate_bwd": (c_int, [c_int, _P, _P, c_void_p, _P, c_float, c_void_p, _PSE, c_void_p, c_void_p, c_void_p, c_void_p,
                               c_void_p, c_void_p, c_void_p, c_void_p, c_void_p, c_void_p, c_void_p, c_size_t, c_void_p]),
    "rx_instnorm_gate_act_bwd": (c_int, [c_int, _P, _P, c_void_p, _P, c_float, c_void_p, c_void_p, c_void_p, c_int, _P, _P,
                                         c_int, c_void_p]),
    "rx_avgpool_fwd": (c_int, [c_int, _P, _P, I3, c_void_p]),
    "rx_instnorm_act_pool_fwd": (c_int, [c_int, _P, c_void_p, _P, _P, _P, I3, c_float, c_void_p]),
    "rx_avgpool_bwd": (c_int, [c_int, _P, _P, I3, c_int, c_void_p]),
    "rx_stem_conv_fwd": (c_int, [c_int, c_void_p, c_int, c_int, c_int, c_int, c_int, c_void_p, c_void_p, _P, I3,
                                 c_void_p]),
    "rx_stem_conv_fwd_stats": (c_int, [c_int, c_void_p, c_int, c_int, c_int, c_int, c_int, c_void_p, c_void_p, _P, I3,
                                       c_float, c_void_p, c_void_p, c_size_t, c_void_p]),
    "rx_stem_conv_bwd_weight_workspace": (c_size_t, [c_int, c_int, c_int]),
    "rx_stem_conv_bwd_weight": (c_int, [c_int, c_void_p, c_int, c_int, c_int, c_int, c_int, _P, c_void_p, I3,
                                        c_void_p, c_size_t, c_void_p]),
    "rx_head_fwd": (c_int, [c_int, _P, c_void_p, c_void_p, c_int, c_void_p, c_int, c_void_p]),
    "rx_head_bwd_workspace": (c_size_t, [_P, c_int]),
    "rx_instnorm_act_head_fwd": (c_int, [c_int, _P, c_void_p, _P, c_float, c_void_p, c_void_p, c_int, c_void_p, c_int, c_void_p]),
    "rx_instnorm_act_bwd_head": (c_int, [c_int, c_void_p, c_int, c_void_p, _P, c_void_p, c_float, _P, c_void_p, c_void_p, c_void_p, c_size_t,
                                         c_void_p]),
    "rx_grad_norm_clip_partials": (ctypes.c_long, [c_int, c_void_p]),
    "rx_grad_norm_clip": (c_int, [c_int, c_void_p, c_void_p, c_float, c_void_p, ctypes.c_long, c_void_p, c_void_p]),
    "rx_head_bwd": (c_int, [c_int, c_void_p, _P, c_void_p, c_int, _P, c_void_p, c_void_p, c_void_p, c_size_t,
                            c_void_p]),
    "rx_channel_sum_workspace": (c_size_t, [_P]),
    "rx_channel_sum": (c_int, [c_int, _P, c_void_p, c_void_p, c_size_t, c_void_p]),
    "rx_loss_workspace": (c_size_t, [c_int, c_int, c_long]),
    "rx_bce_dice_loss_fwd": (c_int, [c_void_p, c_void_p, c_int, c_int, c_long, c_float, c_float, c_float, c_float, c_void_p,
                                     c_void_p, c_void_p, c_size_t, c_void_p]),
    "rx_bce_dice_loss_bwd": (c_int, [c_void_p, c_void_p, c_int, c_int, c_long, c_float, c_float, c_float, c_void_p, c_void_p,
                                     c_void_p, c_void_p]),
    "rx_masked_cosine_loss_fwd": (c_int, [c_void_p, c_void_p, c_int, c_int, c_long, c_void_p, c_void_p, c_void_p, c_size_t,
                                          c_void_p]),
    "rx_masked_cosine_loss_bwd": (c_int, [c_void_p, c_void_p, c_int, c_int, c_long, c_void_p, c_void_p, c_void_p, c_void_p]),
    "rx_adamw_pack": (c_int, [c_int, c_void_p, c_void_p, c_void_p, c_void_p, c_void_p, c_double, c_double, c_double, c_double, c_double,
                              c_int, c_int, c_int, c_int, c_int, c_void_p, c_void_p, c_void_p]),
    "rx_adamw_flat_multi": (c_int, [c_int, c_void_p, c_void_p, c_void_p, c_void_p, c_void_p, c_void_p, c_double, c_double, c_double,
                                    c_double, c_double, c_int, c_void_p]),
    "rx_prog_create": (c_void_p, []),
    "rx_prog_destroy": (None, [c_void_p]),
    "rx_prog_begin": (c_int, [c_void_p, c_void_p, c_int]),
    "rx_prog_end": (c_int, [c_void_p]),
    "rx_prog_len": (c_int, [c_void_p]),
    "rx_prog_cmd_name": (c_char_p, [c_void_p, c_int]),
    "rx_prog_cmd_kernel": (c_char_p, [c_void_p, c_int]),
    "rx_prog_cmd_stream": (c_int, [c_void_p, c_int]),
    "rx_prog_run": (c_int, [c_void_p, c_int, c_int, c_void_p, c_int, c_void_p]),
    "rx_event_new": (c_int, []),
    "rx_event_free": (c_int, [c_int]),
    "rx_event_slots_in_use": (c_int, []),
    "rx_event_record": (c_int, [c_int, c_void_p]),
    "rx_stream_wait": (c_int, [c_int, c_void_p]),
    "rx_adamw_flat": (c_int, [c_void_p, c_void_p, c_void_p, c_void_p, c_void_p, c_double, c_double, c_double, c_double, c_double, c_int,
                              c_long, c_void_p]),
    "rx_sw_gather_workspace": (c_size_t, [c_int, c_int, c_int, c_int, c_int]),
    "rx_sw_gather": (c_int, [c_int, c_void_p, c_int, c_int, c_int, c_int, c_int, c_void_p, c_int, c_int, c_int, c_int, c_void_p,
                             c_void_p, c_size_t, c_void_p]),
    "rx_sw_accumulate": (c_int, [c_void_p, c_int, c_int, c_int, c_int, c_int, c_int, c_void_p, c_int, c_void_p, c_void_p, c_void_p,
                                 c_int, c_int, c_int, c_void_p]),
    "rx_sw_finalize": (c_int, [c_void_p, c_void_p, c_int, c_int, c_int, c_int, c_int, c_int, c_int, c_int, c_int, c_void_p, c_void_p,
                               c_void_p, c_void_p]),
    "rx_aug_workspace": (c_size_t, [c_int, c_int, c_int, c_int, c_int]),
    "rx_aug_pointwise": (c_int, [c_void_p, c_void_p, c_void_p, c_size_t, c_int, c_int, c_int, c_int, c_int, c_void_p, c_void_p, c_long,
                                 c_void_p]),
    "rx_aug_filter_zy": (c_int, [c_void_p, c_void_p, c_int, c_int, c_int, c_int, c_int, c_void_p, c_void_p, c_long, c_void_p]),
    "rx_aug_philox_u32": (c_int, [ctypes.c_uint64, c_long, c_void_p, c_void_p]),
    "rx_geom_apply": (c_int, [c_void_p, c_void_p, c_int, c_int, c_int, c_int, c_int, c_void_p, c_int, c_void_p]),
}

_lib = None


def load():
    global _lib
    if _lib is not None:
        return _lib
    if not os.path.exists(LIB_PATH):
        raise RxError(f"{LIB_PATH} not found: build it with `python __graft_entry__.py` "
                      "(hipcc --offload-arch=gfx950); this engine has no PyTorch/CPU fallback")
    lib = ctypes.CDLL(LIB_PATH)
    for name, (res, args) in _SIGNATURES.items():
        fn = getattr(lib, name)
        fn.restype = res
        fn.argtypes = args
    _lib = lib
    return lib


def exported_symbols():
    return sorted(_SIGNATURES)


def check(rc, what=""):
    if rc != 0:
        msg = load().rx_last_error().decode("utf-8", "replace")
        raise RxError(f"{what} failed with status {rc}: {msg}")


def require_device():
    if not torch.cuda.is_available():
        raise RxError("no HIP device visible: the rxunet engine runs only on an MI355X (gfx950)")
    if not load().rx_device_arch_ok():
        raise RxError("current HIP device is not gfx950")


_raw_stream = getattr(torch._C, "_cuda_getCurrentRawStream", None)
_cur_device = getattr(torch._C, "_cuda_getDevice", None)


def stream_ptr():
    if _raw_stream is not None and _cur_device is not None:
        return c_void_p(_raw_stream(_cur_device()))
    return c_void_p(torch.cuda.current_stream().cuda_stream)
```

multi-task-3d-resencoder-unet_amd/engine/ops.py:

```python
from ctypes import byref, c_void_p

import numpy as np
import torch

from . import lib as _l
from .lib import I3, RxAct, check, load, stream_ptr

_WS = {}
_PROF = None


def set_profiler(p):
    global _PROF
    _PROF = p


class LaunchProfiler:

    def __init__(self):
        self.pending = []
        self.groups = {}
        self.pending_hbm = []
        self.hbm = {}

# ... 145 lines not shown
        return Act(torch.empty((n, z, y, x, c), dtype=dtype, device=device))

    @staticmethod
    def zeros(n, z, y, x, c, dtype, device="cuda"):
        return Act(torch.zeros((n, z, y, x, c), dtype=dtype, device=device))

    def slice(self, c0, c):
        if self.is_planar_cat:
            assert c == 32 and c0 % 32 == 0, "a planar concat is sliced plane by plane"
            return Act.planar(self.root, c0 // 32)
        a = Act(self.t, self.c0 + c0, c)
        a.root, a.plane = self.root, self.plane
        return a

    @property
    def dtype(self):
        return self.t.dtype

    @property
    def dims(self):
        return tuple(self.t.shape[:4])

    @property
    def voxels(self):
        s = self.t.shape
        return s[1] * s[2] * s[3]

    def desc(self):
        d = self._d
        if d is None:
            s = self.t.shape
            if self.is_planar_cat:
                d = RxAct(self.root.data_ptr(), s[0], s[1], s[2], s[3], self.c, 32, self.root.stride(0))
            else:
                d = RxAct(self.t.data_ptr() + self.c0 * self.t.element_size(), s[0], s[1], s[2], s[3], self.c, s[4], 0)
            self._d = d
        return d

    def like(self, root_or_t):
        if self.root is not None:
            return Act.planar(root_or_t, self.plane)
        return Act(root_or_t, self.c0, self.c)

    def tensor(self):
        if self.is_planar_cat:
            return torch.cat(list(self.root), dim=-1)
        return self.t[..., self.c0:self.c0 + self.c]

    def to_ncdhw(self):
        return self.tensor().permute(0, 4, 1, 2, 3).contiguous()

    @staticmethod
    def from_ncdhw(x, dtype=None):
        return Act(x.permute(0, 2, 3, 4, 1).contiguous().to(dtype or x.dtype))


def _code(dtype):
    return _l.DTYPE_CODE[dtype]


def _ptr(t):
    return c_void_p(t.data_ptr()) if t is not None else c_void_p(0)


def _ws_args(ws):
    return c_void_p(ws.data_ptr()), ws.numel()


def pack_conv_weight(w, dtype, w_fwd=None, w_bwd=None, want_fwd=True, want_bwd=True):
    co, ci = w.shape[0], w.shape[1]
    taps = w[0, 0].numel()
    if want_fwd and w_fwd is None:
        w_fwd = torch.empty((taps, co, ci), dtype=dtype, device=w.device)
    if want_bwd and w_bwd is None:
        w_bwd = torch.empty((taps, ci, co), dtype=dtype, device=w.device)
    check(load().rx_pack_conv_weight(_code(dtype), _ptr(w), co, ci, taps, _ptr(w_fwd if want_fwd else None),
                                     _ptr(w_bwd if want_bwd else None), stream_ptr()), "rx_pack_conv_weight")
    return w_fwd, w_bwd


def pack_convT_weight(w, dtype, w_fwd=None, w_bwd=None, want_fwd=True, want_bwd=True):
    ci, co = w.shape[0], w.shape[1]
    taps = w[0, 0].numel()
    if want_fwd and w_fwd is None:
        w_fwd = torch.empty((taps, co, ci), dtype=dtype, device=w.device)
    if want_bwd and w_bwd is None:
        w_bwd = torch.empty((taps, ci, co), dtype=dtype, device=w.device)
    check(load().rx_pack_convT_weight(_code(dtype), _ptr(w), ci, co, taps, _ptr(w_fwd if want_fwd else None),
                                      _ptr(w_bwd if want_bwd else None), stream_ptr()), "rx_pack_convT_weight")
    return w_fwd, w_bwd


def pack_weights_multi(items, dtype):
    import ctypes
    n = len(items)
    if n == 0:
        return
    VP, IA = ctypes.c_void_p * n, ctypes.c_int * n
    wp = VP(*[w.data_ptr() for w, _, _, _ in items])
    kind = IA(*[k for _, k, _, _ in items])
    A = IA(*[w.shape[0] for w, _, _, _ in items])
    B = IA(*[w.shape[1] for w, _, _, _ in items])
    T = IA(*[w[0, 0].numel() for w, _, _, _ in items])
    fw = VP(*[(f.data_ptr() if f is not None else None) for _, _, f, _ in items])
    bw = VP(*[(b.data_ptr() if b is not None else None) for _, _, _, b in items])
    esz = torch.empty((), dtype=dtype).element_size()
    nbytes = sum(w.numel() * (4 + (esz if f is not None else 0) + (esz if b is not None else 0)) for w, _, f, b in items)
    timed_bytes("pack", nbytes, lambda: check(load().rx_pack_multi(_code(dtype), n, wp, kind, A, B, T, fw, bw, stream_ptr()),
                                             "rx_pack_multi"))


def _taps(kernel):
    return kernel[0] * kernel[1] * kernel[2]


def conv3d_fwd(x, w_fwd, bias, y, kernel, stride, ws=None):
    ws = workspace() if ws is None else ws

    def go():
        check(load().rx_conv3d_fwd(_code(x.dtype), byref(x.desc()), _ptr(w_fwd), _ptr(bias), byref(y.desc()),
                                   I3(*kernel), I3(*stride), *_ws_args(ws), stream_ptr()), "rx_conv3d_fwd")
    if _PROF is None:
        return go()
    n = y.dims[0]
    _PROF.run("fwd:" + LaunchProfiler.igemm_name(y.voxels, y.c), 2.0 * n * y.voxels * y.c * x.c * _taps(kernel), 1, go)


def conv3d_fwd_stats(x, w_fwd, bias, y, kernel, stride, stats, eps=1e-5, ws=None):
    ws = workspace() if ws is None else ws

    def go():
        check(load().rx_conv3d_fwd_stats(_code(x.dtype), byref(x.desc()), _ptr(w_fwd), _ptr(bias), byref(y.desc()),
                                         I3(*kernel), I3(*stride), float(eps), _ptr(stats), *_ws_args(ws), stream_ptr()),
              "rx_conv3d_fwd_stats")
    if _PROF is None:
        return go()
    n = y.dims[0]
    _PROF.run("fwd:" + LaunchProfiler.igemm_name(y.voxels, y.c), 2.0 * n * y.voxels * y.c * x.c * _taps(kernel), 1, go)


def conv3d_bwd_data(dy, w_bwd, dx, kernel, stride, accumulate=False, ws=None):
    ws = workspace() if ws is None else ws

    def go():
        check(load().rx_conv3d_bwd_data(_code(dy.dtype), byref(dy.desc()), _ptr(w_bwd), byref(dx.desc()), I3(*kernel),
                                        I3(*stride), int(accumulate), *_ws_args(ws), stream_ptr()),
              "rx_conv3d_bwd_data")
    if _PROF is None:
        return go()
    n = dy.dims[0]
    _PROF.run("dgrad:" + LaunchProfiler.igemm_name(dx.voxels, dx.c), 2.0 * n * dy.voxels * dy.c * dx.c * _taps(kernel), 1, go)


def conv3d_bwd_data_instats(dy, w_bwd, dx, kernel, stride, accumulate, in_y, in_stats, slope, m12, ws=None):
    from ctypes import c_int
    ws = workspace() if ws is None else ws
    fused = c_int(0)

    def go():
        check(load().rx_conv3d_bwd_data_instats(_code(dy.dtype), byref(dy.desc()), _ptr(w_bwd), byref(dx.desc()), I3(*kernel),
                                                I3(*stride), int(accumulate), byref(in_y.desc()), _ptr(in_stats), float(slope),
                                                _ptr(m12), byref(fused), *_ws_args(ws), stream_ptr()), "rx_conv3d_bwd_data_instats")
    if _PROF is None:
        go()
    else:
        n = dx.dims[0]
        _PROF.run("dgrad:" + LaunchProfiler.igemm_name(dx.voxels, dx.c), 2.0 * n * dx.voxels * dx.c * dy.c * _taps(kernel), 1, go)
    return bool(fused.value)


def instnorm_act_bwd_apply(g, y, stats, out, dy, m12, slope=0.01, d_residual=None, accumulate_residual=False):
    check(load().rx_instnorm_act_bwd_apply(_code(y.dtype), byref(g.desc()), byref(y.desc()), _ptr(stats),
                                           byref(out.desc()) if out is not None else None, float(slope), _ptr(m12),
                                           byref(dy.desc()),
                                           byref(d_residual.desc()) if d_residual is not None else None,
                                           int(accumulate_residual), stream_ptr()), "rx_instnorm_act_bwd_apply")


def conv3d_bwd_weight(x, dy, dw, kernel, stride, ws=None):
    need = load().rx_conv3d_bwd_weight_workspace(byref(x.desc()), byref(dy.desc()), I3(*kernel))
    ws = workspace(need) if ws is None else ws

    def go():
        check(load().rx_conv3d_bwd_weight(_code(x.dtype), byref(x.desc()), byref(dy.desc()), _ptr(dw), I3(*kernel),
                                          I3(*stride), *_ws_args(ws), stream_ptr()), "rx_conv3d_bwd_weight")
    if _PROF is None:
        return go()
    n = dy.dims[0]
    name = f"wgrad:wgrad_kernel<{64 if dy.c % 64 == 0 else 32},{64 if x.c % 64 == 0 else 32}>"
    _PROF.run(name, 2.0 * n * dy.voxels * dy.c * x.c * _taps(kernel), 1, go)


def convT3d_fwd(x, w_fwd, bias, y, stride, ws=None):
    ws = workspace() if ws is None else ws
    check(load().rx_convT3d_fwd(_code(x.dtype), byref(x.desc()), _ptr(w_fwd), _ptr(bias), byref(y.desc()),
                                I3(*stride), *_ws_args(ws), stream_ptr()), "rx_convT3d_fwd")


def convT3d_bwd_data(dy, w_bwd, dx, stride, accumulate=False, ws=None):
    ws = workspace() if ws is None else ws
    check(load().rx_convT3d_bwd_data(_code(dy.dtype), byref(dy.desc()), _ptr(w_bwd), byref(dx.desc()), I3(*stride),
                                     int(accumulate), *_ws_args(ws), stream_ptr()), "rx_convT3d_bwd_data")


def convT3d_bwd_weight(x, dy, dw, stride, ws=None):
    need = load().rx_convT3d_bwd_weight_workspace(byref(x.desc()), byref(dy.desc()), I3(*stride))
    ws = workspace(need) if ws is None else ws
    check(load().rx_convT3d_bwd_weight(_code(x.dtype), byref(x.desc()), byref(dy.desc()), _ptr(dw), I3(*stride),
                                       *_ws_args(ws), stream_ptr()), "rx_convT3d_bwd_weight")


def instnorm_stats(y, stats, eps=1e-5, ws=None):
    ws = workspace() if ws is None else ws
    check(load().rx_instnorm_stats(_code(y.dtype), byref(y.desc()), eps, _ptr(stats), *_ws_args(ws), stream_ptr()),
          "rx_instnorm_stats")


def instnorm_stats_mask(stats, keep):
    check(load().rx_instnorm_stats_mask(_ptr(stats), _ptr(keep), int(keep.numel()), stream_ptr()), "rx_instnorm_stats_mask")


def instnorm_act_fwd(y, stats, out, slope=0.01, residual=None):
    check(load().rx_instnorm_act_fwd(_code(y.dtype), byref(y.desc()), _ptr(stats),
                                     byref(residual.desc()) if residual is not None else None, byref(out.desc()),
                                     float(slope), stream_ptr()), "rx_instnorm_act_fwd")


def instnorm_fwd(y, stats, out, slope=0.01, residual=None, eps=1e-5, ws=None):
    ws = workspace() if ws is None else ws
    check(load().rx_instnorm_fwd(_code(y.dtype), byref(y.desc()), eps, _ptr(stats),
                                 byref(residual.desc()) if residual is not None else None, byref(out.desc()),
                                 float(slope), *_ws_args(ws), stream_ptr()), "rx_instnorm_fwd")


def instnorm_act_bwd(g, y, stats, out, dy, slope=0.01, d_residual=None, accumulate_residual=False, ws=None):
    ws = workspace() if ws is None else ws
    check(load().rx_instnorm_act_bwd(_code(y.dtype), byref(g.desc()), byref(y.desc()), _ptr(stats),
                                     byref(out.desc()) if out is not None else None, float(slope), byref(dy.desc()),
                                     byref(d_residual.desc()) if d_residual is not None else None,
                                     int(accumulate_residual), *_ws_args(ws), stream_ptr()), "rx_instnorm_act_bwd")


def instnorm_act_bwd_res(g, y, stats, out, dy, d_residual, slope=0.01, pool_dy=None, pool_stride=(1, 1, 1), ws=None):
    ws = workspace() if ws is None else ws
    check(load().rx_instnorm_act_bwd_res(_code(y.dtype), byref(g.desc()), byref(y.desc()), _ptr(stats), byref(out.desc()),
                                         float(slope), byref(pool_dy.desc()) if pool_dy is not None else None, I3(*pool_stride),
                                         byref(d_residual.desc()), byref(dy.desc()), *_ws_args(ws), stream_ptr()),
          "rx_instnorm_act_bwd_res")


def _se_params(se):
    if se is None:
        return None
    return byref(_l.RxSeParams(se["w1"].data_ptr(), se["b1"].data_ptr(), se["w2"].data_ptr(), se["b2"].data_ptr(),
                               int(se["rd"]), int(se["keep_x"])))


def se_workspace_bytes(y):
    return load().rx_se_workspace(byref(y.desc()))


def se_gate_fwd(y, stats, se, pooled, hidden, gate, mult, path_scale=None, ws=None):
    ws = workspace(se_workspace_bytes(y)) if ws is None else ws
    check(load().rx_se_gate_fwd(_code(y.dtype), byref(y.desc()), _ptr(stats), _ptr(path_scale), _se_params(se), _ptr(pooled),
                                _ptr(hidden), _ptr(gate), _ptr(mult), *_ws_args(ws), stream_ptr()), "rx_se_gate_fwd")


def instnorm_gate_act_fwd(y, stats, mult, keep_x, out, slope=0.01, residual=None):
    check(load().rx_instnorm_gate_act_fwd(_code(y.dtype), byref(y.desc()), _ptr(stats), _ptr(mult), int(keep_x),
                                          byref(residual.desc()) if residual is not None else None, byref(out.desc()),
                                          float(slope), stream_ptr()), "rx_instnorm_gate_act_fwd")


def se_gate_bwd(g, y, stats, out, slope, se, pooled, hidden, gate, mult, dadd, m12, dw1=None, db1=None, dw2=None, db2=None,
                path_scale=None, ws=None):
    ws = workspace(se_workspace_bytes(y)) if ws is None else ws
    check(load().rx_se_gate_bwd(_code(y.dtype), byref(g.desc()), byref(y.desc()), _ptr(stats),
                                byref(out.desc()) if out is not None else None, float(slope), _ptr(path_scale), _se_params(se),
                                _ptr(pooled), _ptr(hidden), _ptr(gate), _ptr(mult), _ptr(dadd), _ptr(m12), _ptr(dw1), _ptr(db1),
                                _ptr(dw2), _ptr(db2), *_ws_args(ws), stream_ptr()), "rx_se_gate_bwd")


def instnorm_gate_act_bwd(g, y, stats, out, slope, mult, dadd, m12, keep_x, dy, d_residual=None, accumulate_residual=False):
    check(load().rx_instnorm_gate_act_bwd(_code(y.dtype), byref(g.desc()), byref(y.desc()), _ptr(stats),
                                          byref(out.desc()) if out is not None else None, float(slope), _ptr(mult), _ptr(dadd),
                                          _ptr(m12), int(keep_x), byref(dy.desc()),
                                          byref(d_residual.desc()) if d_residual is not None else None,
                                          int(accumulate_residual), stream_ptr()), "rx_instnorm_gate_act_bwd")


def avgpool_fwd(x, y, stride):
    check(load().rx_avgpool_fwd(_code(x.dtype), byref(x.desc()), byref(y.desc()), I3(*stride), stream_ptr()),
          "rx_avgpool_fwd")


def instnorm_act_pool_fwd(y, stats, out, pooled, stride, slope=0.01, residual=None):
    check(load().rx_instnorm_act_pool_fwd(_code(y.dtype), byref(y.desc()), _ptr(stats),
                                          byref(residual.desc()) if residual is not None else None, byref(out.desc()),
                                          byref(pooled.desc()), I3(*stride), float(slope), stream_ptr()), "rx_instnorm_act_pool_fwd")


def avgpool_bwd(dy, dx, stride, accumulate=False):
    check(load().rx_avgpool_bwd(_code(dy.dtype), byref(dy.desc()), byref(dx.desc()), I3(*stride), int(accumulate),
                                stream_ptr()), "rx_avgpool_bwd")


def stem_conv_fwd(x_ncdhw, w, bias, out, kernel):
    n, cin, z, y, x = x_ncdhw.shape
    assert x_ncdhw.dtype == torch.float32 and x_ncdhw.is_contiguous()
    check(load().rx_stem_conv_fwd(_code(out.dtype), _ptr(x_ncdhw), n, cin, z, y, x, _ptr(w), _ptr(bias),
                                  byref(out.desc()), I3(*kernel), stream_ptr()), "rx_stem_conv_fwd")


def stem_conv_fwd_stats(x_ncdhw, w, bias, out, kernel, stats, eps=1e-5, ws=None):
    n, cin, z, y, x = x_ncdhw.shape
    assert x_ncdhw.dtype == torch.float32 and x_ncdhw.is_contiguous()
    ws = workspace() if ws is None else ws
    check(load().rx_stem_conv_fwd_stats(_code(out.dtype), _ptr(x_ncdhw), n, cin, z, y, x, _ptr(w), _ptr(bias),
                                        byref(out.desc()), I3(*kernel), float(eps), _ptr(stats), *_ws_args(ws), stream_ptr()),
          "rx_stem_conv_fwd_stats")


def stem_conv_bwd_weight(x_ncdhw, dy, dw, kernel, ws=None):
    n, cin, z, y, x = x_ncdhw.shape
    need = load().rx_stem_conv_bwd_weight_workspace(cin, dy.c, 27)
    ws = workspace(need) if ws is None else ws
    check(load().rx_stem_conv_bwd_weight(_code(dy.dtype), _ptr(x_ncdhw), n, cin, z, y, x, byref(dy.desc()), _ptr(dw),
                                         I3(*kernel), *_ws_args(ws), stream_ptr()), "rx_stem_conv_bwd_weight")


def head_fwd(x, w, b, out_ncdhw, act=_l.RX_ACT_NONE):
    k = w.shape[0]
    check(load().rx_head_fwd(_code(x.dtype), byref(x.desc()), _ptr(w), _ptr(b), k, _ptr(out_ncdhw), int(act),
                             stream_ptr()), "rx_head_fwd")


def head_bwd(dout_ncdhw, x, w, dx, dw, db, ws=None):
    k = w.shape[0]
    need = load().rx_head_bwd_workspace(byref(x.desc()), k)
    ws = workspace(need) if ws is None else ws
    check(load().rx_head_bwd(_code(x.dtype), _ptr(dout_ncdhw), byref(x.desc()), _ptr(w), k,
                             byref(dx.desc()) if dx is not None else None, _ptr(dw), _ptr(db), *_ws_args(ws),
                             stream_ptr()), "rx_head_bwd")


def instnorm_act_head_fwd(y, stats, out, w, b, out_ncdhw, act, slope=0.01):
    check(load().rx_instnorm_act_head_fwd(_code(y.dtype), byref(y.desc()), _ptr(stats), byref(out.desc()) if out is not None else None,
                                          float(slope), _ptr(w), _ptr(b), w.shape[0], _ptr(out_ncdhw), int(act), stream_ptr()),
          "rx_instnorm_act_head_fwd")


def instnorm_act_bwd_head(dout_ncdhw, w, y, stats, dy, slope=0.01, ws=None, dw=None, db=None):
    ws = workspace() if ws is None else ws
    check(load().rx_instnorm_act_bwd_head(_code(y.dtype), _ptr(dout_ncdhw), w.shape[0], _ptr(w), byref(y.desc()), _ptr(stats),
                                          float(slope), byref(dy.desc()), _ptr(dw), _ptr(db), *_ws_args(ws), stream_ptr()),
          "rx_instnorm_act_bwd_head")


def channel_sum(x, out, ws=None):
    ws = workspace() if ws is None else ws
    check(load().rx_channel_sum(_code(x.dtype), byref(x.desc()), _ptr(out), *_ws_args(ws), stream_ptr()),
          "rx_channel_sum")


def _ncv(t):
    n, c = t.shape[0], t.shape[1]
    return n, c, t.numel() // (n * c)


def bce_dice_loss_fwd(logits, target, alpha, beta, smoothing=0.1, eps=1e-6):
    n, c, v = _ncv(logits)
    loss = torch.empty((), dtype=torch.float32, device=logits.device)
    coef = torch.empty(2 * c, dtype=torch.float32, device=logits.device)
    ws = workspace(load().rx_loss_workspace(n, c, v))
    check(load().rx_bce_dice_loss_fwd(_ptr(logits), _ptr(target), n, c, v, alpha, beta, smoothing, eps, _ptr(loss), _ptr(coef),
                                      *_ws_args(ws), stream_ptr()), "rx_bce_dice_loss_fwd")
    return loss, coef


def bce_dice_loss_bwd(logits, target, coef, grad_loss, alpha, beta, smoothing=0.1):
    n, c, v = _ncv(logits)
    dlogits = torch.empty_like(logits)
    check(load().rx_bce_dice_loss_bwd(_ptr(logits), _ptr(target), n, c, v, alpha, beta, smoothing, _ptr(coef), _ptr(grad_loss),
                                      _ptr(dlogits), stream_ptr()), "rx_bce_dice_loss_bwd")
    return dlogits


def masked_cosine_loss_fwd(pred, target):
    n, c, v = _ncv(pred)
    loss = torch.empty((), dtype=torch.float32, device=pred.device)
    coef = torch.empty(1, dtype=torch.float32, device=pred.device)
    ws = workspace(load().rx_loss_workspace(n, c, v))
    check(load().rx_masked_cosine_loss_fwd(_ptr(pred), _ptr(target), n, c, v, _ptr(loss), _ptr(coef), *_ws_args(ws), stream_ptr()),
          "rx_masked_cosine_loss_fwd")
    return loss, coef


def masked_cosine_loss_bwd(pred, target, coef, grad_loss):
    n, c, v = _ncv(pred)
    dpred = torch.empty_like(pred)
    check(load().rx_masked_cosine_loss_bwd(_ptr(pred), _ptr(target), n, c, v, _ptr(coef), _ptr(grad_loss), _ptr(dpred),
                                           stream_ptr()), "rx_masked_cosine_loss_bwd")
    return dpred


def aug_pointwise(image, out, scratch, host_table, table, pool_words):
    b, c, z, y, x = image.shape
    check(load().rx_aug_pointwise(_ptr(image), _ptr(out), _ptr(scratch) if scratch is not None else None,
                                  scratch.numel() * scratch.element_size() if scratch is not None else 0, b, c, z, y, x,
                                  c_void_p(host_table.data_ptr()), _ptr(table), pool_words, stream_ptr()), "rx_aug_pointwise")


def aug_filter_zy(scratch, out, host_table, table, pool_words):
    b, c, z, y, x = out.shape
    check(load().rx_aug_filter_zy(_ptr(scratch), _ptr(out), b, c, z, y, x, c_void_p(host_table.data_ptr()), _ptr(table), pool_words,
                                  stream_ptr()), "rx_aug_filter_zy")


def augment_batch(image, host_table, table, pool_words, any_group3):
    if not image.is_cuda:
        raise _l.RxError("augment_batch: the image batch must be a device tensor")
    out = torch.empty_like(image)
    scratch = None
    if any_group3:
        b, c, z, y, x = image.shape
        assert load().rx_aug_workspace(b, c, z, y, x) == image.numel() * 4
        scratch = torch.empty_like(image)
    aug_pointwise(image, out, scratch, host_table, table, pool_words)
    if any_group3:
        aug_filter_zy(scratch, out, host_table, table, pool_words)
    return out


def geom_table(geom_ops):
    rows = [o.row() if hasattr(o, "row") else o for o in geom_ops]
    table = np.ascontiguousarray(np.asarray(rows, dtype=np.int32).reshape(len(rows), 12))
    return table


def geom_apply(tensor, geom_ops, vector):
    if not isinstance(tensor, torch.Tensor) or not tensor.is_cuda:
        raise _l.RxError("geom_apply: the batch must be a device tensor (the host classes are training/transforms/geometric)")
    if tensor.dim() != 5 or tensor.dtype != torch.float32:
        raise _l.RxError(f"geom_apply: expected a float32 (B, C, Z, Y, X) batch, got {tensor.dtype} {tuple(tensor.shape)}")
    tensor = tensor.contiguous()
    table = geom_table(geom_ops)
    b, c, z, y, x = tensor.shape
    if table.shape[0] != b:
        raise _l.RxError(f"geom_apply: {table.shape[0]} records for a batch of {b}")
    out = torch.empty_like(tensor)
    check(load().rx_geom_apply(_ptr(tensor), _ptr(out), b, c, z, y, x, table.ctypes.data, 1 if vector else 0, stream_ptr()),
          "rx_geom_apply")
    return out


def aug_philox_u32(key, n, device):
    out = torch.empty(n, dtype=torch.int32, device=device)
    check(load().rx_aug_philox_u32(int(key), n, _ptr(out), stream_ptr()), "rx_aug_philox_u32")
    return out.to(torch.int64) & 0xFFFFFFFF


def timed_bytes(name, nbytes, fn):
    if _PROF is None:
        return fn()
    return _PROF.run_bytes(name, nbytes, fn)


def _tb(a):
    return 0 if a is None else a.dims[0] * a.voxels * a.c * a.t.element_size()


def _hbm(label, nbytes):
    def deco(f):
        def wrapped(*a, **k):
            if _PROF is None:
                return f(*a, **k)
            return _PROF.run_bytes(label, nbytes(*a, **k), lambda: f(*a, **k))
        wrapped.__name__, wrapped.__doc__ = f.__name__, f.__doc__
        return wrapped
    return deco


def _bwd_bytes(g, y, out, dy, d_residual, acc):
    return _tb(g) + _tb(y) + _tb(dy) + _tb(out) + _tb(d_residual) * (2 if acc else 1)


def _pack_bytes(w, dtype, w_fwd=None, w_bwd=None, want_fwd=True, want_bwd=True):
    e = torch.empty((), dtype=dtype).element_size()
    return w.numel() * (4 + (e if want_fwd else 0) + (e if want_bwd else 0))


instnorm_stats = _hbm("in_stats(colreduce)", lambda y, stats, eps=1e-5, ws=None: _tb(y))(instnorm_stats)
instnorm_act_fwd = _hbm("in_act_fwd", lambda y, stats, out, slope=0.01, residual=None: _tb(y) + _tb(out) + _tb(residual))(instnorm_act_fwd)
instnorm_fwd = _hbm("in_fwd(stats+apply)", lambda y, stats, out, slope=0.01, residual=None, eps=1e-5, ws=None:
                    _tb(y) + _tb(out) + _tb(residual))(instnorm_fwd)
instnorm_act_bwd = _hbm("in_act_bwd(colreduce+apply)",
                        lambda g, y, stats, out, dy, slope=0.01, d_residual=None, accumulate_residual=False, ws=None:
                        _bwd_bytes(g, y, out, dy, d_residual, accumulate_residual))(instnorm_act_bwd)
instnorm_act_bwd_res = _hbm("in_act_bwd_res(colreduce+apply)",
                            lambda g, y, stats, out, dy, d_residual, slope=0.01, pool_dy=None, pool_stride=(1, 1, 1), ws=None:
                            _tb(g) + _tb(y) + _tb(out) + _tb(dy) + _tb(d_residual) + _tb(pool_dy))(instnorm_act_bwd_res)
instnorm_act_bwd_apply = _hbm("in_act_bwd_apply",
                              lambda g, y, stats, out, dy, m12, slope=0.01, d_residual=None, accumulate_residual=False:
                              _bwd_bytes(g, y, out, dy, d_residual, accumulate_residual))(instnorm_act_bwd_apply)
se_gate_fwd = _hbm("se_gate_fwd(linesum+gate)", lambda y, *a, **k: _tb(y))(se_gate_fwd)
instnorm_gate_act_fwd = _hbm("in_gate_act_fwd", lambda y, stats, mult, keep_x, out, slope=0.01, residual=None:
                             _tb(y) + _tb(out) + _tb(residual))(instnorm_gate_act_fwd)
se_gate_bwd = _hbm("se_gate_bwd(linesums+gate)", lambda g, y, stats, out, *a, **k: _tb(g) + _tb(y) + _tb(out))(se_gate_bwd)
instnorm_gate_act_bwd = _hbm("in_gate_act_bwd",
                             lambda g, y, stats, out, slope, mult, dadd, m12, keep_x, dy, d_residual=None, accumulate_residual=False:
                             _bwd_bytes(g, y, out, dy, d_residual, accumulate_residual))(instnorm_gate_act_bwd)
avgpool_fwd = _hbm("avgpool_fwd", lambda x, y, stride: _tb(x) + _tb(y))(avgpool_fwd)
instnorm_act_pool_fwd = _hbm("in_act_pool_fwd", lambda y, stats, out, pooled, stride, slope=0.01, residual=None:
                             _tb(y) + _tb(out) + _tb(pooled) + _tb(residual))(instnorm_act_pool_fwd)
avgpool_bwd = _hbm("avgpool_bwd", lambda dy, dx, stride, accumulate=False: _tb(dy) + _tb(dx) * (2 if accumulate else 1))(avgpool_bwd)
head_fwd = _hbm("head_fwd", lambda x, w, b, out_ncdhw, act=0: _tb(x) + out_ncdhw.numel() * 4)(head_fwd)
head_bwd = _hbm("head_bwd", lambda dout_ncdhw, x, w, dx, dw, db, ws=None: dout_ncdhw.numel() * 4 + _tb(x) + _tb(dx))(head_bwd)
instnorm_act_head_fwd = _hbm("in_act_head_fwd", lambda y, stats, out, w, b, out_ncdhw, act, slope=0.01:
                             _tb(y) + _tb(out) + out_ncdhw.numel() * 4)(instnorm_act_head_fwd)
instnorm_act_bwd_head = _hbm("in_act_bwd_head(colreduce+apply)", lambda dout_ncdhw, w, y, stats, dy, slope=0.01, ws=None, dw=None, db=None:
                             dout_ncdhw.numel() * 4 + _tb(y) + _tb(dy))(instnorm_act_bwd_head)
channel_sum = _hbm("channel_sum", lambda x, out, ws=None: _tb(x))(channel_sum)
pack_conv_weight = _hbm("pack", _pack_bytes)(pack_conv_weight)
pack_convT_weight = _hbm("pack", _pack_bytes)(pack_convT_weight)
stem_conv_fwd = _hbm("stem_conv_fwd", lambda x_ncdhw, w, bias, out, kernel: x_ncdhw.numel() * 4 + _tb(out))(stem_conv_fwd)
stem_conv_fwd_stats = _hbm("stem_conv_fwd", lambda x_ncdhw, w, bias, out, kernel, stats, eps=1e-5, ws=None: x_ncdhw.numel() * 4 + _tb(out))(stem_conv_fwd_stats)
stem_conv_bwd_weight = _hbm("stem_conv_bwd_weight", lambda x_ncdhw, dy, dw, kernel, ws=None: x_ncdhw.numel() * 4 + _tb(dy))(stem_conv_bwd_weight)
convT3d_fwd = _hbm("convT_fwd", lambda x, w_fwd, bias, y, stride, ws=None: _tb(x) + _tb(y))(convT3d_fwd)
convT3d_bwd_data = _hbm("convT_bwd_data", lambda dy, w_bwd, dx, stride, accumulate=False, ws=None:
                        _tb(dy) + _tb(dx) * (2 if accumulate else 1))(convT3d_bwd_data)
convT3d_bwd_weight = _hbm("convT_bwd_weight", lambda x, dy, dw, stride, ws=None: _tb(x) + _tb(dy))(convT3d_bwd_weight)
```

multi-task-3d-resencoder-unet_amd/engine/plan.py:

```python
from dataclasses import dataclass, field
from typing import Callable, Dict, List, Optional

import os

import torch
from torch import nn

from . import lib as _l
from . import ops
from .ops import Act


class UnsupportedConfig(NotImplementedError):
    pass


_SIDE_STREAMS: Dict[str, "torch.cuda.Stream"] = {}


def side_stream(device):
    key = str(device)
    st = _SIDE_STREAMS.get(key)
    if st is None:
        st = _SIDE_STREAMS[key] = torch.cuda.Stream(device=device)
# ... 364 lines not shown
        if x is None and (not blk.skip_ops or isinstance(blk.skip_ops[0], (nn.AvgPool3d, nn.AvgPool2d))):
            r = self._image_act(tape)
        for op in blk.skip_ops:
            if isinstance(op, (nn.AvgPool3d, nn.AvgPool2d)):
                st = self._k3(op.stride if isinstance(op.stride, (list, tuple)) else [op.stride] * (2 if self.two_d else 3))
                odims = tuple(d // s for d, s in zip(r.act.dims[1:], st))
                p = self._new(odims, r.act.c, f"pool:{len(tape)}", needs_grad=r.needs_grad)
                tape.append(Rec("pool", dict(x=r, y=p, stride=st)))
                r = p
            else:
                r = self._emit_cdnr(tape, op, r)
        path = blk.main_path()
        h = x
        for m in path[:-1]:
            h = self._emit_cdnr(tape, m, h)
        se = blk.squeeze_excitation if getattr(blk, "apply_se", False) else None
        drop_p = blk.drop_path.drop_prob if getattr(blk, "apply_stochastic_depth", False) else 0.0
        return self._emit_cdnr(tape, path[-1], h, out=out, residual=r, final_slope=_slope_of(blk.final_nonlin()),
                               se=se, drop_p=drop_p)

    def _build(self):
        net = self.net
        enc = net.shared_encoder
        tasks = list(net.task_decoders.keys())
        n_st = len(enc.stages)
        feats = list(enc.output_channels)
        featsp = [self._cp(f) for f in feats]

        dims = [None] * n_st
        cur = self.spatial
        for s in range(n_st):
            st = self._k3(enc.strides[s])
            kz = self._k3(enc.kernel_sizes[s] if isinstance(enc.kernel_sizes[s], (list, tuple)) else
                          [enc.kernel_sizes[s]] * (2 if self.two_d else 3))
            cur = self._out_dims(cur, kz, st)
            dims[s] = cur

        cats: List[List[AT]] = []
        for d in range(len(tasks)):
            row = []
            for j in range(n_st - 1):
                es = n_st - 2 - j
                st_mod = net.task_decoders[tasks[d]].stages[j]
                first = None if hasattr(st_mod, "blocks") else st_mod.convs[0]
                halo_ok = first is not None and list(self._k3(first.spec()["kernel"])) == [3, 3, 3]
                cat = self._new_cat(dims[es], featsp[es], f"cat{d}.{j}", allow_planar=halo_ok)
                cat.segs = [(0, feats[es], 0), (feats[es], feats[es], featsp[es])]
                row.append(cat)
            cats.append(row)

        def skip_home(es):
            if es == n_st - 1 or not tasks:
                return None
            cat = cats[0][n_st - 2 - es]
            c = featsp[es]
            return AT(cat.act.slice(c, c), f"skip{es}")

        tape = self.enc_tape
        x = None
        h = None
        for m in (list(enc.stem.convs) if enc.stem is not None else []):
            h = self._emit_cdnr(tape, m, h)
        skips: List[AT] = []
        for s in range(n_st):
            stage = enc.stages[s]
            home = skip_home(s)
            if enc.is_residual:
                blocks = list(stage.blocks)
                for bi, blk in enumerate(blocks):
                    h = self._emit_block(tape, blk, h, out=home if bi == len(blocks) - 1 else None)
            else:
                mods = list(stage[0].convs)
                for mi, m in enumerate(mods):
                    h = self._emit_cdnr(tape, m, h, out=home if mi == len(mods) - 1 else None)
            skips.append(h)
        self.enc_skips = [(at, feats[i]) for i, at in enumerate(skips)]

        self.head_recs = []
        for d, name in enumerate(tasks):
            dec = net.task_decoders[name]
            tape = []
            self.dec_tapes.append(tape)
            low = skips[-1]
            for j in range(n_st - 1):
                es = n_st - 2 - j
                c = featsp[es]
                cat = cats[d][j]
                up = AT(cat.act.slice(0, c), f"up{d}.{j}")
                tconv = dec.transpconvs[j]
                stride = self._k3(tconv.stride)
                if list(tconv.kernel_size) != list(tconv.stride):
                    raise UnsupportedConfig("ConvTranspose with kernel != stride")
                ti, to = tconv.in_channels, tconv.out_channels
                if self._cp(ti) != low.act.c or self._cp(to) != c:
                    raise RuntimeError("plan bug: transposed-conv channel extents")
                w_k = self._shadow(tconv.weight, (low.act.c, c, *tconv.weight.shape[2:]),
                                   [((slice(0, ti), slice(0, to)), (slice(None), slice(None)))])
                b_k = self._shadow(tconv.bias, (c,), [((slice(0, to),), (slice(None),))])
                pk = self._pack(w_k, "convT")
                widx = self._param(tconv.weight)
                bidx = self._param(tconv.bias) if tconv.bias is not None else None
                tape.append(Rec("convT", dict(x=low, y=up, pk=pk, b=b_k, widx=widx, bidx=bidx, stride=stride,
                                              cat=cat)))
                if d > 0:
                    dst = AT(cat.act.slice(c, c), f"skipcopy{d}.{j}")
                    tape.append(Rec("copy", dict(x=skips[es], y=dst, cat=cat)))
                st_mod = dec.stages[j]
                h = cat
                if hasattr(st_mod, "blocks"):
                    for blk in st_mod.blocks:
                        h = self._emit_block(tape, blk, h)
                else:
                    for m in st_mod.convs:
                        h = self._emit_cdnr(tape, m, h)
                low = h
            head = dec.seg_layers[-1]
            k = head.out_channels
            if k > 1024:
                raise UnsupportedConfig("task heads with more than 1024 channels have no HIP kernel")
            out = torch.empty((self.B, k, *low.act.dims[1:]), dtype=torch.float32, device=self.device)
            self.outputs[name] = out
            act_mod = net.task_activations[name] if name in net.task_activations else None
            act_code = _l.RX_ACT_NONE
            if isinstance(act_mod, nn.Sigmoid):
                act_code = _l.RX_ACT_SIGMOID
            elif isinstance(act_mod, nn.Softmax):
                act_code = _l.RX_ACT_SOFTMAX
            hw_k = self._shadow(head.weight, (k, low.act.c, *head.weight.shape[2:]),
                                [((slice(None), slice(0, head.in_channels)), (slice(None), slice(None)))])
            tape.append(Rec("head", dict(x=low, w=hw_k, b=head.bias, widx=self._param(head.weight),
                                         bidx=self._param(head.bias), k=k, name=name, out=out, act=act_code)))

        self._gen_forward()
        if self.needs_grad:
            self._gen_backward()

    def _gen_forward(self):
        P = self
        f = self.fwd
        self.n_fwd_enc = None
        self.fwd_dec_start = []
        for tape in [self.enc_tape] + self.dec_tapes:
            if tape is not self.enc_tape and self.n_fwd_enc is None:
                self.n_fwd_enc = len(f)
            if tape is not self.enc_tape:
                self.fwd_dec_start.append(len(f))
            for i, rec in enumerate(tape[:-1]):
                nxt = tape[i + 1]
                if (rec.kind == "conv" and nxt.kind == "inact" and nxt.a["y"] is rec.a["y"] and self.dtype != torch.float32
                        and list(rec.a["kernel"]) == [3, 3, 3] and list(rec.a["stride"]) == [1, 1, 1]
                        and rec.a["y"].act.voxels > 512 and rec.a["y"].act.dims[3] >= 16):
                    rec.a["stats_to"] = nxt.a
                    nxt.a["stats_done"] = True
                if (rec.kind == "stem" and nxt.kind == "inact" and nxt.a["y"] is rec.a["y"] and self.dtype != torch.float32
                        and rec.a["y"].act.voxels > 512):
                    rec.a["stats_to"] = nxt.a
                    nxt.a["stats_done"] = True
            producers = {id(r.a["out"]): r for r in tape if r.kind == "inact" and r.a["gate"] is None}
            for rec in tape:
                if rec.kind == "pool" and id(rec.a["x"]) in producers and rec.a["x"].act.voxels > 512:
                    src = producers[id(rec.a["x"])]
                    if "pool_to" not in src.a:
                        src.a["pool_to"] = rec.a
                        rec.a["fused"] = True
            if self.dtype != torch.float32:
                for rec in tape:
                    if rec.kind != "head" or rec.a["k"] > 4:
                        continue
                    prods = [r for r in tape if r.kind == "inact" and r.a["out"] is rec.a["x"]]
                    if len(prods) != 1:
                        continue
                    pa = prods[0].a
                    c = pa["out"].act.c
                    if (pa["gate"] is None and pa["res"] is None and "pool_to" not in pa and not pa.get("norm_done")
                            and pa["out"].act.voxels > 512 and c % 8 == 0 and 64 % (c // 8) == 0):
                        pa["head_to"] = rec.a
                        rec.a["fwd_fused"] = True
            for rec in tape:
                a = rec.a
                if (tape is self.enc_tape and self._pack_delay_at is None and rec.kind in ("conv", "pool")
                        and rec.a["y"].act.voxels < self.spatial[0] * self.spatial[1] * self.spatial[2]):
                    self._pack_delay_at = len(f)
                if rec.kind == "stem":
                    def sstep(a=a):
                        st = a.get("stats_to")
                        if st is not None:
                            ops.stem_conv_fwd_stats(P._x, a["w"], a["b"], a["y"].act, a["kernel"], st["stats"], P._eps_now(st))
                            P._mask_dropped(st)
                        else:
                            ops.stem_conv_fwd(P._x, a["w"], a["b"], a["y"].act, a["kernel"])
                    f.append(sstep)
                elif rec.kind == "image":
                    f.append(lambda a=a: ops.stem_conv_fwd(P._x, a["w"], None, a["y"].act, [1, 1, 1]))
                elif rec.kind == "conv":
                    def cstep(a=a):
                        P._await_pack(a["pk"])
                        st = a.get("stats_to")
                        if st is not None:
                            ops.conv3d_fwd_stats(a["x"].act, a["pk"]["w_fwd"], a["b"], a["y"].act, a["kernel"], a["stride"],
                                                 st["stats"], P._eps_now(st))
                            P._mask_dropped(st)
                        else:
                            ops.conv3d_fwd(a["x"].act, a["pk"]["w_fwd"], a["b"], a["y"].act, a["kernel"], a["stride"])
                    f.append(cstep)
                elif rec.kind == "convT":
                    def tstep(a=a):
                        P._await_pack(a["pk"])
                        ops.convT3d_fwd(a["x"].act, a["pk"]["w_fwd"], a["b"], a["y"].act, a["stride"])
                    f.append(tstep)
                elif rec.kind == "inact" and a["gate"] is not None:
                    def gstep(a=a):
                        g = a["gate"]
                        res = a["res"].act if a["res"] is not None else None
                        if g["se"] is None and g["scale_now"] is None:
                            ops.instnorm_fwd(a["y"].act, a["stats"], a["out"].act, a["slope"], res, a["eps"])
                            return
                        if not a.get("stats_done"):
                            ops.instnorm_stats(a["y"].act, a["stats"], a["eps"])
                        ops.se_gate_fwd(a["y"].act, a["stats"], P._se_args(g), g["pooled"], g["hidden"], g["gate"], g["mult"],
                                        g["scale_now"])
                        ops.instnorm_gate_act_fwd(a["y"].act, a["stats"], g["mult"], g["keep_x"], a["out"].act, a["slope"], res)
                    f.append(gstep)
                elif rec.kind == "inact":
                    def step(a=a):
                        res = a["res"].act if a["res"] is not None else None
                        head = a.get("head_to")
                        if head is not None:
                            if not a.get("stats_done"):
                                ops.instnorm_stats(a["y"].act, a["stats"], P._eps_now(a))
                                P._mask_dropped(a)
                            keep = P.needs_grad and not a.get("head_dw_fused")
                            ops.instnorm_act_head_fwd(a["y"].act, a["stats"], a["out"].act if keep else None, head["w"].view(head["k"], -1),
                                                      head["b"], head["out"], head["act"] if P._apply_act else _l.RX_ACT_NONE, a["slope"])
                            return
                        pool = a.get("pool_to")
                        if pool is not None:
                            if not a.get("stats_done"):
                                ops.instnorm_stats(a["y"].act, a["stats"], P._eps_now(a))
                                P._mask_dropped(a)
                            ops.instnorm_act_pool_fwd(a["y"].act, a["stats"], a["out"].act, pool["y"].act, pool["stride"], a["slope"], res)
                        elif a.get("stats_done"):
                            ops.instnorm_act_fwd(a["y"].act, a["stats"], a["out"].act, a["slope"], res)
                        elif a["drop"] is not None and a["drop"]["active"]:
                            ops.instnorm_stats(a["y"].act, a["stats"], P._eps_now(a))
                            P._mask_dropped(a)
                            ops.instnorm_act_fwd(a["y"].act, a["stats"], a["out"].act, a["slope"], res)
                        else:
                            ops.instnorm_fwd(a["y"].act, a["stats"], a["out"].act, a["slope"], res, a["eps"])
                    f.append(step)
                elif rec.kind == "pool":
                    if not a.get("fused"):
                        f.append(lambda a=a: ops.avgpool_fwd(a["x"].act, a["y"].act, a["stride"]))
                elif rec.kind == "copy":
                    f.append(lambda a=a: ops.avgpool_fwd(a["x"].act, a["y"].act, (1, 1, 1)))
                elif rec.kind == "head":
                    if a.get("fwd_fused"):
                        continue

                    def step(a=a):
                        w2 = a["w"].view(a["k"], -1)
                        ops.head_fwd(a["x"].act, w2, a["b"], a["out"], a["act"] if P._apply_act else _l.RX_ACT_NONE)
                    f.append(step)

    def _dy_for(self, y: AT):
        key = (y.act.dims, y.act.c)
        turn = self._dy_turn.get(key, 0)
        self._dy_turn[key] = (turn + 1) % self.dy_ring
        slot = key + (turn,)
        if slot not in self.dy_pool:
            t = torch.empty((*y.act.dims, y.act.c), dtype=self.dtype, device=self.device)
            self.bytes_alloc += t.numel() * t.element_size()
            self.dy_pool[slot] = Act(t)
        return self.dy_pool[slot]

    def _gen_backward(self):
        P = self
        b = self.bwd
        cat_written = {}

        def mark_cat(cat):
            cat_written[cat.act.key] = True

        def view_written(at):
            return at.written or cat_written.get(at.act.key, False)

        def new_grad(idx):
            sync = P.grad_sync
            ent = P._pad_idx.get(idx)
            if ent is not None:
                if ent["gpad"] is None:
                    ent["gpad"] = torch.empty(tuple(ent["sh"].shape), dtype=torch.float32, device=P.device)
                P._pad_done.append(idx)
                return ent["gpad"]
            if sync is not None:
                g = sync.alloc(idx)
            elif P._use_gstore:
                g = P._gviews[idx]
            else:
                g = torch.empty_like(P.params[idx], memory_format=torch.contiguous_format)
            P._grads[idx] = g
            return g

        skip = set(filter(None, os.environ.get("RX_SKIP", "").split(",")))
        if skip and os.environ.get("RX_ABLATION", "0") != "1":
            raise _l.RxError("RX_SKIP drops launches from the backward pass (timing ablations, wrong gradients): "
                             "set RX_ABLATION=1 as well to confirm, or unset RX_SKIP")

        def done(idx):
            if idx in P._pad_idx:
                return
            if P._recording is not None:
                P._marks.append((len(P._recording), idx, P._on_side))
            if P.grad_sync is not None:
                P.grad_sync.ready(idx)

        dy_free = self._dy_free

        def side_run(fn, dy_act):
            if not (P.overlap_wgrad and P._side is not None):
                fn(ops.workspace())
                return
            ops.event_record(P._ev_fork)
            ops.stream_wait(P._ev_fork, P._side)
            key = id(dy_act.t)
            slot = P._dy_ev.get(key)
            if slot is None:
                slot = P._dy_ev[key] = ops.event_new()
            P._on_side = True
            try:
                with torch.cuda.stream(P._side):
                    fn(P._ws2)
                    ops.event_record(slot)
            finally:
                P._on_side = False
            dy_free[key] = slot

        def before_dy_write(dy_act):
            slot = dy_free.pop(id(dy_act.t), None)
            if slot is not None:
                ops.stream_wait(slot)

        order = self.grad_order

        def wrote(at, kind, info=None):
            at._gw = (kind, info)

        for tape in self.dec_tapes + [self.enc_tape]:
            for rec in reversed(tape):
                a = rec.a
                if rec.kind == "head":
                    x = a["x"]
                    assert not view_written(x)
                    gx = self._grad_buf(x)
                    x.written = True
                    hinfo = {"fused": False}
                    wrote(x, "head", hinfo)
                    a["hinfo"] = hinfo

                    def step(a=a, gx=gx, hinfo=hinfo):
                        dl = P._dlogits.get(a["name"])
                        if dl is None:
                            gx.t.zero_()
                            if P.grad_sync is not None:
                                for i in (a["widx"], a["bidx"]):
                                    new_grad(i).zero_()
                                    done(i)
                            return
                        if hinfo.get("dw_fused"):
                            return
                        dw, db = new_grad(a["widx"]), new_grad(a["bidx"])
                        ops.head_bwd(dl, a["x"].act, a["w"].view(a["k"], -1), None if hinfo["fused"] else gx, dw, db)
                        done(a["widx"])
                        done(a["bidx"])
                    order += [a["widx"], a["bidx"]]
                    b.append(step)
                elif rec.kind == "inact":
                    out, y, res = a["out"], a["y"], a["res"]
                    gout = self._grad_buf(out) if out.gact is None else out.gact
                    if not view_written(out):
                        raise RuntimeError(f"plan bug: gradient of {out.name} is consumed before it is produced")
                    dy = self._dy_for(y)
                    y.gact = dy
                    gres, acc = None, False
                    if res is not None and res.needs_grad:
                        gres = self._grad_buf(res)
                        acc = view_written(res)
                        res.written = True
                        wrote(res, "gres")
                    gw = getattr(out, "_gw", (None, None))
                    if (gw[0] == "head" and a["gate"] is None and res is None and self.dtype != torch.float32
                            and out.act.voxels > 512):
                        heads = [r.a for r in tape if r.kind == "head" and r.a["x"] is out]
                        if len(heads) == 1 and heads[0]["k"] <= 4:
                            a["head_src"] = heads[0]
                            gw[1]["fused"] = True
                            if heads[0].get("fwd_fused") and heads[0]["w"] is self.params[heads[0]["widx"]]:
                                a["head_dw_fused"] = True
                                gw[1]["dw_fused"] = True
                    if (gw[0] == "conv" and a["gate"] is None and res is None and self.dtype != torch.float32
                            and out.act.full_buffer and out.act.root is None and out.act.c % 32 == 0 and out.act.voxels > 512
                            and out.act.dims[3] >= 16):
                        a["m12"] = torch.empty((self.B, out.act.c, 2), dtype=torch.float32, device=self.device)
                        a["m12_valid"] = False
                        gw[1]["inact"] = a
                    def gistep(a=a, gout=gout, dy=dy, gres=gres, acc=acc):
                        g = a["gate"]
                        before_dy_write(dy)
                        if g["se"] is None and g.get("scale_now") is None:
                            ops.instnorm_act_bwd(gout, a["y"].act, a["stats"],
                                                 a["out"].act if (a["slope"] != 1.0 and a["res"] is not None) else None, dy,
                                                 a["slope"], gres, acc)
                            return
                        grads = [new_grad(i) for i in g["se"]["idx"]] if g["se"] is not None else [None] * 4
                        ops.se_gate_bwd(gout, a["y"].act, a["stats"], a["out"].act, a["slope"], P._se_args(g), g["pooled"],
                                        g["hidden"], g["gate"], g["mult"], g["dadd"], g["m12"], *grads,
                                        path_scale=g.get("scale_now"))
                        ops.instnorm_gate_act_bwd(gout, a["y"].act, a["stats"], a["out"].act, a["slope"], g["mult"], g["dadd"],
                                                  g["m12"], g["keep_x"], dy, gres, acc)
                        if g["se"] is not None:
                            for i in g["se"]["idx"]:
                                done(i)
                    if a["gate"] is not None:
                        if a["gate"]["se"] is not None:
                            order += a["gate"]["se"]["idx"]
                        b.append(gistep)
                        continue

                    pend = getattr(out, "_pool_pending", None)
                    out._pool_pending = None
                    fuse_res = gres is not None and not acc and res is not None and y.act.voxels > 512
                    if pend is not None and not fuse_res:
                        b.append(lambda pend=pend: ops.avgpool_bwd(pend["gy"], pend["gx"], pend["stride"], True))
                        pend = None
                    if fuse_res:
                        def rstep(a=a, gout=gout, dy=dy, gres=gres, pend=pend):
                            before_dy_write(dy)
                            ops.instnorm_act_bwd_res(gout, a["y"].act, a["stats"], a["out"].act, dy, gres, a["slope"],
                                                     pool_dy=pend["gy"] if pend is not None else None,
                                                     pool_stride=pend["stride"] if pend is not None else (1, 1, 1))
                        b.append(rstep)
                        continue

                    def istep(a=a, gout=gout, dy=dy, gres=gres, acc=acc):
                        before_dy_write(dy)
                        mask_out = a["out"].act if (a["slope"] != 1.0 and a["res"] is not None) else None
                        hs = a.get("head_src")
                        dl = P._dlogits.get(hs["name"]) if hs is not None else None
                        if dl is not None and a.get("head_dw_fused"):
                            dw, db = new_grad(hs["widx"]), new_grad(hs["bidx"])
                            ops.instnorm_act_bwd_head(dl, hs["w"].view(hs["k"], -1), a["y"].act, a["stats"], dy, a["slope"],
                                                      dw=dw.view(hs["k"], -1), db=db)
                            done(hs["widx"])
                            done(hs["bidx"])
                        elif dl is not None:
                            ops.instnorm_act_bwd_head(dl, hs["w"].view(hs["k"], -1), a["y"].act, a["stats"], dy, a["slope"])
                        elif a.get("m12_valid"):
                            a["m12_valid"] = False
                            ops.instnorm_act_bwd_apply(gout, a["y"].act, a["stats"], mask_out, dy, a["m12"], a["slope"], gres, acc)
                        elif "inbwd_reduce" in skip and a["y"].act.voxels > 512:
                            if "m12x" not in a:
                                a["m12x"] = torch.zeros((self.B, a["y"].act.c, 2), dtype=torch.float32, device=self.device)
                            ops.instnorm_act_bwd_apply(gout, a["y"].act, a["stats"], mask_out, dy, a["m12x"], a["slope"], gres, acc)
                        else:
                            ops.instnorm_act_bwd(gout, a["y"].act, a["stats"], mask_out, dy, a["slope"], gres, acc)
                    b.append(istep)
                elif rec.kind in ("conv", "stem"):
                    y = a["y"]
                    dy = y.gact

                    def wstep(a=a, dy=dy, kind=rec.kind):
                        dw = new_grad(a["widx"])
                        db = new_grad(a["bidx"]) if a["bidx"] is not None else None

                        def launches(ws):
                            if "wgrad" in skip and kind != "stem":
                                pass
                            elif kind == "stem":
                                ops.stem_conv_bwd_weight(P._x, dy, dw, a["kernel"], ws)
                            else:
                                ops.conv3d_bwd_weight(a["x"].act, dy, dw, a["kernel"], a["stride"], ws)
                            done(a["widx"])
                            if db is not None:
                                ops.channel_sum(dy, db, ws)
                                done(a["bidx"])
                        side_run(launches, dy)
                    order += [a["widx"]] + ([a["bidx"]] if a["bidx"] is not None else [])
                    b.append(wstep)
                    if rec.kind == "conv" and a["x"].needs_grad:
                        x = a["x"]
                        gx = self._grad_buf(x)
                        acc = view_written(x)
                        x.written = True
                        if x.act.full_buffer:
                            mark_cat(x)
                        bsinfo = {"inact": None}
                        wrote(x, "conv", bsinfo)

                        def dstep(a=a, dy=dy, gx=gx, acc=acc, bsinfo=bsinfo):
                            if "dgrad" in skip:
                                return
                            ia = bsinfo["inact"]
                            if ia is None:
                                ops.conv3d_bwd_data(dy, a["pk"]["w_bwd"], gx, a["kernel"], a["stride"], acc)
                            else:
                                ia["m12_valid"] = ops.conv3d_bwd_data_instats(dy, a["pk"]["w_bwd"], gx, a["kernel"], a["stride"], acc,
                                                                              ia["y"].act, ia["stats"], ia["slope"], ia["m12"])
                        b.append(dstep)
                elif rec.kind == "convT":
                    x, y = a["x"], a["y"]
                    if not view_written(y):
                        raise RuntimeError("plan bug: concat gradient not initialised before the transposed conv")
                    gy = y.act.like(a["cat"].gact.root if a["cat"].gact.root is not None else a["cat"].gact.t)
                    gx = self._grad_buf(x)
                    acc = view_written(x)
                    x.written = True
                    wrote(x, "convT")

                    def step(a=a, gy=gy, gx=gx, acc=acc):
                        dw = new_grad(a["widx"])
                        db = new_grad(a["bidx"]) if a["bidx"] is not None else None

                        def launches(ws):
                            ops.convT3d_bwd_weight(a["x"].act, gy, dw, a["stride"], ws)
                            done(a["widx"])
                            if db is not None:
                                ops.channel_sum(gy, db, ws)
                                done(a["bidx"])
                        side_run(launches, gy)
                        ops.convT3d_bwd_data(gy, a["pk"]["w_bwd"], gx, a["stride"], acc)
                    order += [a["widx"]] + ([a["bidx"]] if a["bidx"] is not None else [])
                    b.append(step)
                elif rec.kind == "pool":
                    x, y = a["x"], a["y"]
                    if not x.needs_grad:
                        continue
                    gx = self._grad_buf(x)
                    acc = view_written(x)
                    x.written = True
                    wrote(x, "pool")
                    assert y.gact is not None, "plan bug: pooled tensor has no gradient"
                    ti = next(i for i, r in enumerate(tape) if r is rec)
                    prev = tape[ti - 1] if ti > 0 else None
                    if (acc and prev is not None and prev.kind == "inact" and prev.a["out"] is x and prev.a["res"] is not None
                            and prev.a["gate"] is None and x.act.voxels > 512):
                        x._pool_pending = dict(gy=y.gact, gx=gx, stride=a["stride"])
                        continue
                    b.append(lambda a=a, gy=y.gact, gx=gx, acc=acc: ops.avgpool_bwd(gy, gx, a["stride"], acc))
                elif rec.kind == "copy":
                    x, y = a["x"], a["y"]
                    gy = y.act.like(a["cat"].gact.root if a["cat"].gact.root is not None else a["cat"].gact.t)
                    gx = self._grad_buf(x)
                    acc = view_written(x)
                    x.written = True
                    wrote(x, "copy")
                    b.append(lambda gy=gy, gx=gx, acc=acc: ops.avgpool_bwd(gy, gx, (1, 1, 1), acc))

    def _grad_buf(self, at: AT):
        if at.gact is not None:
            return at.gact
        base = at.act.root if at.act.root is not None else at.act.t
        if at.act.key not in self._gbase:
            t = torch.empty_like(base)
            self.bytes_alloc += t.numel() * t.element_size()
            self._gbase[at.act.key] = t
        at.gact = at.act.like(self._gbase[at.act.key])
        return at.gact

    def _ensure_side(self):
        if self.device.type == "cuda" and self.overlap_wgrad and self._side is None:
            self._side = side_stream(self.device)
            self._ws2 = torch.empty(ops.workspace().numel(), dtype=torch.uint8, device=self.device)
        if self._ev_fork is None and self.device.type == "cuda":
            self._ev_fork, self._ev_join = ops.event_new(), ops.event_new()

    def _await_pack(self, ent):
        if ent.get("deferred") and self._pack_deferred is not None:
            self._issue_deferred_packs()
        slot = ent.get("event")
        if slot is not None:
            ops.stream_wait(slot)
            for e in ent["group"]:
                e["event"] = None

    def _packs_stale(self, force=False):
        epoch = getattr(self.net, "_weights_epoch", 0)
        return [e for e in self.packs
                if force or e.get("epoch") != epoch
                or not (e["version"] == e["param"]._version and e.get("ptr") == e["param"].data_ptr())]

    def refresh_packs(self, force=False):
        stale = self._packs_stale(force)
        if not stale:
            return
        side = None
        if self.device.type == "cuda" and self.overlap_wgrad:
            self._ensure_side()
            side = self._side
            ops.event_record(self._ev_fork)
            ops.stream_wait(self._ev_fork, side)
        self._pack_entries(stale, side, defer=True)

    def _issue_deferred_packs(self):
        d, self._pack_deferred = self._pack_deferred, None
        if d is not None:
            groups, side = d
            ops.event_record(self._ev_fork)
            ops.stream_wait(self._ev_fork, side)
            self._pack_groups_now(groups, side, 1)

    def _pack_entries(self, entries, side, defer=False):
        limit = 96 << 20
        groups, cur, cur_bytes = [], [], 0
        for ent in entries:
            nb = ent["param"].numel() * 4
            if cur and cur_bytes + nb > limit and len(groups) < 3:
                groups.append(cur)
                cur, cur_bytes = [], 0
            cur.append(ent)
            cur_bytes += nb
        if cur:
            groups.append(cur)
        self._pack_deferred = None
        if defer and side is not None and len(groups) > 1 and self._pack_delay_at is not None:
            self._pack_deferred = (groups[1:], side)
            for grp in groups[1:]:
                for ent in grp:
                    ent["deferred"] = True
            groups = groups[:1]
        self._pack_groups_now(groups, side, 0)

    def _pack_groups_now(self, groups, side, gi0):
        ctx = torch.cuda.stream(side) if side is not None else _NullCtx()
        with ctx:
            for gi, grp in enumerate(groups, gi0):
                items = []
                for ent in grp:
                    w = ent["param"].detach()
                    if w.dtype != torch.float32 or not w.is_contiguous():
                        w = w.float().contiguous()
                        self._unstable_params = True
                    if self.two_d:
                        w = w.unsqueeze(2)
                    items.append((w, 0 if ent["kind"] == "conv" else 1, ent["w_fwd"], ent["w_bwd"]))
                ops.pack_weights_multi(items, self.dtype)
                slot = None
                if side is not None:
                    while len(self._pack_slots) <= gi:
                        self._pack_slots.append(ops.event_new())
                    slot = self._pack_slots[gi]
                    ops.event_record(slot)
                for ent in grp:
                    p = ent["param"]
                    ent["deferred"] = False
                    ent["event"], ent["group"] = slot, grp
                    ent["version"], ent["ptr"] = p._version, p.data_ptr()
# ... 338 lines not shown
```

Measured before the change: 118.7 patches/s.

## Fold split-K conv reduction into the following small-tensor instance-norm kernels

For small-volume layers (at most 512 voxels, channels divisible by 32, 16-bit dtypes), the split-K igemm no longer runs its own reduce kernel. It hands back the fp32 partial slabs, and the next instance-norm forward, or the instance-norm-activation backward, sums the slabs, adds bias and any accumulated value, writes the conv output, and computes stats in the same pass. This removes one kernel launch and one full write-then-read of the conv output per affected conv, in both the forward and the dgrad path. In exchange it adds plan-level coupling between the conv step and the norm step, and repeats the slab reads inside the norm kernel's first pass.

```diff
diff --git a/include/rxunet.h b/include/rxunet.h
--- a/include/rxunet.h
+++ b/include/rxunet.h
@@ -71,6 +71,25 @@
 int rx_instnorm_act_bwd(rx_dtype dt, const rx_act* g, const rx_act* y, const float* stats, const rx_act* out,
                         float slope, const rx_act* dy, const rx_act* d_residual, int accumulate_residual,
                         void* ws, size_t ws_bytes, void* stream);
+
+typedef struct {
+  const float* slab;
+  const float* bias;
+  void* out;
+  int32_t ksplit;
+  int32_t nv, co, accumulate;
+} rx_slab;
+int rx_conv3d_fwd_slab(rx_dtype dt, const rx_act* x, const void* w_fwd, const float* bias, const rx_act* y,
+                       const int32_t kernel[3], const int32_t stride[3], void* ws, size_t ws_bytes, rx_slab* slab,
+                       void* stream);
+int rx_conv3d_bwd_data_slab(rx_dtype dt, const rx_act* dy, const void* w_bwd, const rx_act* dx,
+                            const int32_t kernel[3], const int32_t stride[3], int accumulate, void* ws, size_t ws_bytes,
+                            rx_slab* slab, void* stream);
+int rx_instnorm_fwd_slab(rx_dtype dt, const rx_slab* slab, const rx_act* y, float eps, float* stats,
+                         const rx_act* residual, const rx_act* out, float slope, void* stream);
+int rx_instnorm_act_bwd_slab(rx_dtype dt, const rx_slab* slab, const rx_act* g, const rx_act* y, const float* stats,
+                             const rx_act* out, float slope, const rx_act* dy, const rx_act* d_residual,
+                             int accumulate_residual, void* stream);
 
 int rx_instnorm_act_bwd_res(rx_dtype dt, const rx_act* g, const rx_act* y, const float* stats, const rx_act* out,
                             float slope, const rx_act* pool_dy, const int32_t pool_stride[3], const rx_act* d_residual,
diff --git a/multi-task-3d-resencoder-unet_amd/csrc/rx_elementwise.hip b/multi-task-3d-resencoder-unet_amd/csrc/rx_elementwise.hip
--- a/multi-task-3d-resencoder-unet_amd/csrc/rx_elementwise.hip
+++ b/multi-task-3d-resencoder-unet_amd/csrc/rx_elementwise.hip
@@ -460,10 +460,41 @@
                      V * dy->ld, d_residual ? (T*)d_residual->ptr : (T*)nullptr, d_residual ? d_residual->ld : 0,                 \
                      d_residual ? V * d_residual->ld : 0L, (int)V, C, slope, use_mask ? 1 : (mask_xhat ? 2 : 0))
 
-template <typename T, int G, bool HAS_RES>
+struct InSlab {
+  const float* slab;
+  const float* bias;
+  long kstride;
+  int ksplit, accumulate;
+};
+
+template <typename T>
+__device__ inline Vec16<T> slab_reduce16(const InSlab& sl, long nv, int C, int c, T* dst) {
+  constexpr int P = Elem<T>::PER16;
+  static_assert(P == 8, "slab consumers exist for the 16-bit types only");
+  const float* sp = sl.slab + nv * C + c;
+  f32x4 a = {0.f, 0.f, 0.f, 0.f}, b = {0.f, 0.f, 0.f, 0.f};
+#pragma unroll 4
+  for (int k = 0; k < sl.ksplit; ++k) {
+    a += *reinterpret_cast<const f32x4*>(sp + k * sl.kstride);
+    b += *reinterpret_cast<const f32x4*>(sp + k * sl.kstride + 4);
+  }
+  Vec16<T> old, r;
+  if (sl.accumulate) old = ld16(dst);
+#pragma unroll
+  for (int j = 0; j < P; ++j) {
+    float f = j < 4 ? a[j & 3] : b[j & 3];
+    if (sl.bias) f += sl.bias[c + j];
+    if (sl.accumulate) f += Elem<T>::to_f(old.v[j]);
+    r.v[j] = Elem<T>::from_f(f);
+  }
+  st16(dst, r);
+  return r;
+}
+
+template <typename T, int G, bool HAS_RES, bool FROM_SLAB = false>
 __global__ __launch_bounds__(256) void in_small_fwd_kernel(const T* __restrict__ y, int ldy, long sy, const T* __restrict__ res, int ldr,
                                                            long sr, T* __restrict__ out, int ldo, long so, float* __restrict__ stats, int V,
-                                                           int C, float eps, float slope) {
+                                                           int C, float eps, float slope, T* yw = nullptr, const InSlab sl = InSlab{}) {
   constexpr int P = Elem<T>::PER16;
   constexpr int CPG = G / P;
   __shared__ double red[4][2][G];
@@ -472,12 +503,15 @@
   const int n = blockIdx.y, c0 = blockIdx.x * G;
   const int ck = tid % CPG, vl = tid / CPG;
   const int VL = 256 / CPG;
-  const T* yn = y + n * sy + c0 + ck * P;
+  const T* yn = FROM_SLAB ? nullptr : y + n * sy + c0 + ck * P;
+  T* ywn = FROM_SLAB ? yw + n * sy + c0 + ck * P : nullptr;
   float s[P], q[P];
 #pragma unroll
   for (int j = 0; j < P; ++j) s[j] = q[j] = 0.f;
   for (int v = vl; v < V; v += VL) {
-    Vec16<T> a = ld16(yn + (long)v * ldy);
+    Vec16<T> a;
+    if constexpr (FROM_SLAB) a = slab_reduce16<T>(sl, (long)n * V + v, C, c0 + ck * P, ywn + (long)v * ldy);
+    else a = ld16(yn + (long)v * ldy);
 #pragma unroll
     for (int j = 0; j < P; ++j) {
       float f = Elem<T>::to_f(a.v[j]);
@@ -521,7 +555,7 @@
   const T* rn = HAS_RES ? res + n * sr + c0 + ck * P : nullptr;
   T* on = out + n * so + c0 + ck * P;
   for (int v = vl; v < V; v += VL) {
-    Vec16<T> a = ld16(yn + (long)v * ldy);
+    Vec16<T> a = FROM_SLAB ? ld16(ywn + (long)v * ldy) : ld16(yn + (long)v * ldy);
     Vec16<T> r;
     if (HAS_RES) r = ld16(rn + (long)v * ldr);
     Vec16<T> o;
@@ -536,11 +570,12 @@
   }
 }
 
-template <typename T, int G>
+template <typename T, int G, bool FROM_SLAB = false>
 __global__ __launch_bounds__(256) void in_small_bwd_kernel(const T* __restrict__ g, int ldg, long sg, const T* __restrict__ y, int ldy, long sy,
                                                            const T* __restrict__ out, int ldo, long so, const float* __restrict__ stats,
                                                            T* __restrict__ dy, int lddy, long sdy, T* __restrict__ dres, int lddr, long sdr,
-                                                           int acc_res, int V, int C, float slope, int mask_mode) {
+                                                           int acc_res, int V, int C, float slope, int mask_mode, T* gw = nullptr,
+                                                           const InSlab sl = InSlab{}) {
   constexpr int P = Elem<T>::PER16;
   constexpr int CPG = G / P;
   __shared__ double red[4][2][G];
@@ -556,8 +591,14 @@
     mean[j] = stats[2 * ((size_t)n * C + co + j)];
     rstd[j] = stats[2 * ((size_t)n * C + co + j) + 1];
   }
-  auto gprime = [&](int v, float (&gg)[P], float (&xh)[P]) {
-    Vec16<T> gv = ld16(g + n * sg + (long)v * ldg + co);
+  auto gprime = [&](int v, float (&gg)[P], float (&xh)[P], bool first) {
+    Vec16<T> gv;
+    if constexpr (FROM_SLAB) {
+      T* gp = gw + n * sg + (long)v * ldg + co;
+      gv = first ? slab_reduce16<T>(sl, (long)n * V + v, C, (int)co, gp) : ld16(gp);
+    } else {
+      gv = ld16(g + n * sg + (long)v * ldg + co);
+    }
     Vec16<T> yv = ld16(y + n * sy + (long)v * ldy + co);
     Vec16<T> ov;
     if (mask_mode == 1) ov = ld16(out + n * so + (long)v * ldo + co);
@@ -574,7 +615,7 @@
   for (int j = 0; j < P; ++j) s[j] = q[j] = 0.f;
   for (int v = vl; v < V; v += VL) {
     float gg[P], xh[P];
-    gprime(v, gg, xh);
+    gprime(v, gg, xh, true);
 #pragma unroll
     for (int j = 0; j < P; ++j) {
       s[j] += gg[j];
@@ -609,7 +650,7 @@
   }
   for (int v = vl; v < V; v += VL) {
     float gg[P], xh[P];
-    gprime(v, gg, xh);
+    gprime(v, gg, xh, false);
     Vec16<T> dv, rv;
     if (dres && acc_res) rv = ld16(dres + n * sdr + (long)v * lddr + co);
 #pragma unroll
@@ -697,6 +738,65 @@
   return RX_OK;
 }
 
+bool rx_in_small_slab_ok(rx_dtype dt, const rx_act* y) {
+  return dt != RX_F32 && rx_act_voxels(y) <= RX_IN_SMALL_MAX_VOXELS && y->c % 32 == 0 && y->c / 8 <= 256 && y->ld % 8 == 0 &&
+         !((uintptr_t)y->ptr & 15);
+}
+static int check_slab(rx_dtype dt, const rx_slab* s, const rx_act* t, const char* who) {
+  if (!s || !s->slab || s->ksplit < 1) RX_FAIL(RX_EINVAL, "%s: no slabs (the conv completed its output itself)", who);
+  if (!rx_in_small_slab_ok(dt, t)) RX_FAIL(RX_EUNSUPPORTED, "%s: tensor outside the single-launch 16-bit path", who);
+  if (s->out != t->ptr || s->co != t->c || (long)s->nv != (long)t->n * rx_act_voxels(t))
+    RX_FAIL(RX_EINVAL, "%s: the slabs describe another tensor", who);
+  return RX_OK;
+}
+
+extern "C" int rx_instnorm_act_bwd_slab(rx_dtype dt, const rx_slab* slab, const rx_act* g, const rx_act* y, const float* stats,
+                                        const rx_act* out, float slope, const rx_act* dy, const rx_act* d_residual,
+                                        int accumulate_residual, void* stream) {
+  RX_RECORD(stream, [=, slab_ = slab ? *slab : rx_slab{}, g_ = RxActV(g), y_ = RxActV(y), out_ = RxActV(out), dy_ = RxActV(dy), d_residual_ = RxActV(d_residual)](void* s) { return rx_instnorm_act_bwd_slab(dt, &slab_, g_.p(), y_.p(), stats, out_.p(), slope, dy_.p(), d_residual_.p(), accumulate_residual, s); });
+  int rc;
+  if ((rc = check_vec_channels(g, dt, "rx_instnorm_act_bwd_slab(g)"))) return rc;
+  if ((rc = check_vec_channels(y, dt, "rx_instnorm_act_bwd_slab(y)"))) return rc;
+  if ((rc = check_vec_channels(dy, dt, "rx_instnorm_act_bwd_slab(dy)"))) return rc;
+  const bool mask_xhat = slope != 1.0f && out == nullptr;
+  const bool use_mask = slope != 1.0f && out != nullptr;
+  if (use_mask) {
+    if ((rc = check_vec_channels(out, dt, "rx_instnorm_act_bwd_slab(out)"))) return rc;
+    if (!same_geom(y, out)) RX_FAIL(RX_EINVAL, "rx_instnorm_act_bwd_slab: out geometry mismatch");
+  }
+  if (d_residual) {
+    if ((rc = check_vec_channels(d_residual, dt, "rx_instnorm_act_bwd_slab(d_residual)"))) return rc;
+    if (!same_geom(y, d_residual)) RX_FAIL(RX_EINVAL, "rx_instnorm_act_bwd_slab: d_residual geometry mismatch");
+    if (d_residual->ptr == g->ptr) RX_FAIL(RX_EINVAL, "rx_instnorm_act_bwd_slab: d_residual and g must be different buffers");
+  }
+  if (!stats || !same_geom(y, g) || !same_geom(y, dy) || dy->ptr == g->ptr) RX_FAIL(RX_EINVAL, "rx_instnorm_act_bwd_slab: bad arguments");
+  if ((rc = check_slab(dt, slab, g, "rx_instnorm_act_bwd_slab"))) return rc;
+  const long V = rx_act_voxels(y);
+  const int N = y->n, C = y->c;
+  hipStream_t st1 = (hipStream_t)stream;
+  const int mode = use_mask ? 1 : (mask_xhat ? 2 : 0);
+  const bool narrow = V >= RX_IN_SMALL_NARROW_VOXELS;
+  dim3 grid1(narrow ? C / 8 : C / 32, N);
+  const InSlab sl{slab->slab, slab->bias, (long)slab->nv * C, slab->ksplit, slab->accumulate};
+#define RX_LAUNCH_IN_SMALL_BWD_SLAB(G)                                                                                                 \
+  hipLaunchKernelGGL((in_small_bwd_kernel<T, G, true>), grid1, dim3(256), 0, st1, (const T*)nullptr, g->ld, V * g->ld, (const T*)y->ptr,  \
+                     y->ld, V * y->ld, use_mask ? (const T*)out->ptr : (const T*)nullptr, use_mask ? out->ld : 0,                     \
+                     use_mask ? V * out->ld : 0L, stats, (T*)dy->ptr, dy->ld, V * dy->ld,                                             \
+                     d_residual ? (T*)d_residual->ptr : (T*)nullptr, d_residual ? d_residual->ld : 0,                                 \
+                     d_residual ? V * d_residual->ld : 0L, accumulate_residual, (int)V, C, slope, mode, (T*)g->ptr, sl)
+  if (dt == RX_BF16) {
+    using T = bf16_t;
+    if (narrow) RX_LAUNCH_IN_SMALL_BWD_SLAB(8);
+    else RX_LAUNCH_IN_SMALL_BWD_SLAB(32);
+  } else {
+    using T = f16_t;
+    if (narrow) RX_LAUNCH_IN_SMALL_BWD_SLAB(8);
+    else RX_LAUNCH_IN_SMALL_BWD_SLAB(32);
+  }
+  RX_CHECK_LAUNCH("rx_instnorm_act_bwd_slab");
+  return RX_OK;
+}
+
 
 template <typename T, bool POOL>
 struct InBwdResOp {
@@ -889,6 +989,46 @@
     else RX_LAUNCH_IN_SMALL_FWD(32, false);
   });
   RX_CHECK_LAUNCH("rx_instnorm_fwd");
+  return RX_OK;
+}
+
+extern "C" int rx_instnorm_fwd_slab(rx_dtype dt, const rx_slab* slab, const rx_act* y, float eps, float* stats, const rx_act* residual,
+                                    const rx_act* out, float slope, void* stream) {
+  RX_RECORD(stream, [=, slab_ = slab ? *slab : rx_slab{}, y_ = RxActV(y), residual_ = RxActV(residual), out_ = RxActV(out)](void* s) { return rx_instnorm_fwd_slab(dt, &slab_, y_.p(), eps, stats, residual_.p(), out_.p(), slope, s); });
+  int rc;
+  if ((rc = check_vec_channels(y, dt, "rx_instnorm_fwd_slab(y)"))) return rc;
+  if ((rc = check_vec_channels(out, dt, "rx_instnorm_fwd_slab(out)"))) return rc;
+  if (!stats || !same_geom(y, out) || out->ptr == y->ptr) RX_FAIL(RX_EINVAL, "rx_instnorm_fwd_slab: geometry mismatch / null stats");
+  if (residual) {
+    if ((rc = check_vec_channels(residual, dt, "rx_instnorm_fwd_slab(residual)"))) return rc;
+    if (!same_geom(y, residual)) RX_FAIL(RX_EINVAL, "rx_instnorm_fwd_slab: residual geometry mismatch");
+  }
+  if ((rc = check_slab(dt, slab, y, "rx_instnorm_fwd_slab"))) return rc;
+  if (slab->accumulate) RX_FAIL(RX_EINVAL, "rx_instnorm_fwd_slab: a forward conv does not accumulate");
+  const long V = rx_act_voxels(y);
+  hipStream_t st = (hipStream_t)stream;
+  const bool narrow = V >= RX_IN_SMALL_NARROW_VOXELS;
+  dim3 grid(narrow ? y->c / 8 : y->c / 32, y->n);
+  const InSlab sl{slab->slab, slab->bias, (long)slab->nv * y->c, slab->ksplit, 0};
+#define RX_LAUNCH_IN_SMALL_FWD_SLAB(G, RES)                                                                                         \
+  hipLaunchKernelGGL((in_small_fwd_kernel<T, G, RES, true>), grid, dim3(256), 0, st, (const T*)nullptr, y->ld, V * y->ld,            \
+                     RES ? (const T*)residual->ptr : (const T*)nullptr, RES ? residual->ld : 0, RES ? V * residual->ld : 0L,         \
+                     (T*)out->ptr, out->ld, V * out->ld, stats, (int)V, y->c, eps, slope, (T*)y->ptr, sl)
+#define RX_IN_SMALL_FWD_SLAB_ALL()                                    \
+  do {                                                                \
+    if (residual && narrow) RX_LAUNCH_IN_SMALL_FWD_SLAB(8, true);     \
+    else if (residual) RX_LAUNCH_IN_SMALL_FWD_SLAB(32, true);         \
+    else if (narrow) RX_LAUNCH_IN_SMALL_FWD_SLAB(8, false);           \
+    else RX_LAUNCH_IN_SMALL_FWD_SLAB(32, false);                      \
+  } while (0)
+  if (dt == RX_BF16) {
+    using T = bf16_t;
+    RX_IN_SMALL_FWD_SLAB_ALL();
+  } else {
+    using T = f16_t;
+    RX_IN_SMALL_FWD_SLAB_ALL();
+  }
+  RX_CHECK_LAUNCH("rx_instnorm_fwd_slab");
   return RX_OK;
 }
 
diff --git a/multi-task-3d-resencoder-unet_amd/csrc/rx_igemm.hip b/multi-task-3d-resencoder-unet_amd/csrc/rx_igemm.hip
--- a/multi-task-3d-resencoder-unet_amd/csrc/rx_igemm.hip
+++ b/multi-task-3d-resencoder-unet_amd/csrc/rx_igemm.hip
@@ -374,7 +374,7 @@
 }
 
 static int igemm_launch(rx_dtype dt, const void* in, const void* w, const float* bias, void* out, IgemmGeom& g, int N, void* ws,
-                        size_t ws_bytes, hipStream_t st) {
+                        size_t ws_bytes, hipStream_t st, rx_slab* so = nullptr) {
   const int per16 = dt == RX_F32 ? 4 : 8;
   const int KB = 4 * per16;
   if (g.Ci % KB) RX_FAIL(RX_EUNSUPPORTED, "igemm: input channels must be a multiple of %d (got %d)", KB, g.Ci);
@@ -432,6 +432,12 @@
           (void)hipFuncSetAttribute(reinterpret_cast<const void*>(&igemm_fat_kernel<f16_t>), hipFuncAttributeMaxDynamicSharedMemorySize, (int)lds);
           hipLaunchKernelGGL((igemm_fat_kernel<f16_t>), grid, dim3(256), lds, st, (const f16_t*)in, (const f16_t*)w, (float*)ws, g, (int)NV, nsteps);
         }
+        if (so) {
+          so->slab = (const float*)ws, so->bias = bias, so->out = out;
+          so->ksplit = ks, so->nv = (int32_t)NV, so->co = g.Co, so->accumulate = g.accumulate;
+          RX_CHECK_LAUNCH("igemm_fat(slab)");
+          return RX_OK;
+        }
         const long total = NV * (g.Co / 4);
         const int G = (int)((total + 255) / 256 > 2048 ? 2048 : (total + 255) / 256);
         RX_DISPATCH_DTYPE(dt, T, hipLaunchKernelGGL((igemm_splitk_reduce<T>), dim3(G, 1), dim3(256), 0, st, (const float*)ws, bias, (T*)out, g, N));
@@ -504,9 +510,27 @@
   g.out_ss = rx_act_voxels(a) * (long)a->ld;
 }
 
+bool rx_in_small_slab_ok(rx_dtype dt, const rx_act* y);
+
+static int conv3d_fwd_impl(rx_dtype dt, const rx_act* x, const void* w_fwd, const float* bias, const rx_act* y, const int32_t kernel[3],
+                           const int32_t stride[3], void* ws, size_t wsb, void* stream, rx_slab* so);
+
 extern "C" int rx_conv3d_fwd(rx_dtype dt, const rx_act* x, const void* w_fwd, const float* bias, const rx_act* y,
                              const int32_t kernel[3], const int32_t stride[3], void* ws, size_t wsb, void* stream) {
   RX_RECORD(stream, [=, x_ = RxActV(x), y_ = RxActV(y), kernel_ = RxI3V(kernel), stride_ = RxI3V(stride)](void* s) { return rx_conv3d_fwd(dt, x_.p(), w_fwd, bias, y_.p(), kernel_.v, stride_.v, ws, wsb, s); });
+  return conv3d_fwd_impl(dt, x, w_fwd, bias, y, kernel, stride, ws, wsb, stream, nullptr);
+}
+
+extern "C" int rx_conv3d_fwd_slab(rx_dtype dt, const rx_act* x, const void* w_fwd, const float* bias, const rx_act* y,
+                                  const int32_t kernel[3], const int32_t stride[3], void* ws, size_t wsb, rx_slab* slab, void* stream) {
+  RX_RECORD(stream, [=, x_ = RxActV(x), y_ = RxActV(y), kernel_ = RxI3V(kernel), stride_ = RxI3V(stride)](void* s) { rx_slab slab_dummy; return rx_conv3d_fwd_slab(dt, x_.p(), w_fwd, bias, y_.p(), kernel_.v, stride_.v, ws, wsb, &slab_dummy, s); });
+  if (!slab) RX_FAIL(RX_EINVAL, "rx_conv3d_fwd_slab: bad arguments");
+  memset(slab, 0, sizeof(*slab));
+  return conv3d_fwd_impl(dt, x, w_fwd, bias, y, kernel, stride, ws, wsb, stream, rx_act_ok(y) && rx_in_small_slab_ok(dt, y) ? slab : nullptr);
+}
+
+static int conv3d_fwd_impl(rx_dtype dt, const rx_act* x, const void* w_fwd, const float* bias, const rx_act* y, const int32_t kernel[3],
+                           const int32_t stride[3], void* ws, size_t wsb, void* stream, rx_slab* so) {
   if (!rx_act_ok_planar(x) || !rx_act_ok(y) || !w_fwd) RX_FAIL(RX_EINVAL, "rx_conv3d_fwd: bad arguments");
   int rc = check13(kernel, stride, "rx_conv3d_fwd");
   if (rc) return rc;
@@ -544,7 +568,7 @@
         t.w = (uint16_t)P.ntaps;
         ++P.ntaps;
       }
-  return igemm_launch(dt, x->ptr, w_fwd, bias, y->ptr, g, x->n, ws, wsb, (hipStream_t)stream);
+  return igemm_launch(dt, x->ptr, w_fwd, bias, y->ptr, g, x->n, ws, wsb, (hipStream_t)stream, so);
 }
 
 extern "C" int rx_conv3d_bwd_data_instats(rx_dtype dt, const rx_act* dy, const void* w_bwd, const rx_act* dx, const int32_t kernel[3],
@@ -600,9 +624,26 @@
   return rx_instnorm_stats(dt, y, eps, stats, ws, wsb, stream);
 }
 
+static int conv3d_bwd_data_impl(rx_dtype dt, const rx_act* dy, const void* w_bwd, const rx_act* dx, const int32_t kernel[3],
+                                const int32_t stride[3], int accumulate, void* ws, size_t wsb, void* stream, rx_slab* so);
+
 extern "C" int rx_conv3d_bwd_data(rx_dtype dt, const rx_act* dy, const void* w_bwd, const rx_act* dx, const int32_t kernel[3],
                                   const int32_t stride[3], int accumulate, void* ws, size_t wsb, void* stream) {
   RX_RECORD(stream, [=, dy_ = RxActV(dy), dx_ = RxActV(dx), kernel_ = RxI3V(kernel), stride_ = RxI3V(stride)](void* s) { return rx_conv3d_bwd_data(dt, dy_.p(), w_bwd, dx_.p(), kernel_.v, stride_.v, accumulate, ws, wsb, s); });
+  return conv3d_bwd_data_impl(dt, dy, w_bwd, dx, kernel, stride, accumulate, ws, wsb, stream, nullptr);
+}
+
+extern "C" int rx_conv3d_bwd_data_slab(rx_dtype dt, const rx_act* dy, const void* w_bwd, const rx_act* dx, const int32_t kernel[3],
+                                       const int32_t stride[3], int accumulate, void* ws, size_t wsb, rx_slab* slab, void* stream) {
+  RX_RECORD(stream, [=, dy_ = RxActV(dy), dx_ = RxActV(dx), kernel_ = RxI3V(kernel), stride_ = RxI3V(stride)](void* s) { rx_slab slab_dummy; return rx_conv3d_bwd_data_slab(dt, dy_.p(), w_bwd, dx_.p(), kernel_.v, stride_.v, accumulate, ws, wsb, &slab_dummy, s); });
+  if (!slab) RX_FAIL(RX_EINVAL, "rx_conv3d_bwd_data_slab: bad arguments");
+  memset(slab, 0, sizeof(*slab));
+  return conv3d_bwd_data_impl(dt, dy, w_bwd, dx, kernel, stride, accumulate, ws, wsb, stream,
+                              rx_act_ok(dx) && rx_in_small_slab_ok(dt, dx) ? slab : nullptr);
+}
+
+static int conv3d_bwd_data_impl(rx_dtype dt, const rx_act* dy, const void* w_bwd, const rx_act* dx, const int32_t kernel[3],
+                                const int32_t stride[3], int accumulate, void* ws, size_t wsb, void* stream, rx_slab* so) {
   if (!rx_act_ok(dy) || !rx_act_ok_planar(dx) || !w_bwd) RX_FAIL(RX_EINVAL, "rx_conv3d_bwd_data: bad arguments");
   int rc = check13(kernel, stride, "rx_conv3d_bwd_data");
   if (rc) return rc;
@@ -681,7 +722,7 @@
           }
         }
       }
-  return igemm_launch(dt, dy->ptr, w_bwd, nullptr, dx->ptr, g, dx->n, ws, wsb, (hipStream_t)stream);
+  return igemm_launch(dt, dy->ptr, w_bwd, nullptr, dx->ptr, g, dx->n, ws, wsb, (hipStream_t)stream, so);
 }
 
 static int checkT(const int32_t s[3], const rx_act* small, const rx_act* big, const char* who) {
diff --git a/multi-task-3d-resencoder-unet_amd/engine/lib.py b/multi-task-3d-resencoder-unet_amd/engine/lib.py
--- a/multi-task-3d-resencoder-unet_amd/engine/lib.py
+++ b/multi-task-3d-resencoder-unet_amd/engine/lib.py
@@ -33,8 +33,14 @@
                 ("keep_x", c_int32)]
 
 
+class RxSlab(ctypes.Structure):
+    _fields_ = [("slab", c_void_p), ("bias", c_void_p), ("out", c_void_p), ("ksplit", c_int32), ("nv", c_int32),
+                ("co", c_int32), ("accumulate", c_int32)]
+
+
 I3 = c_int32 * 3
 _P = POINTER(RxAct)
+_PSL = POINTER(RxSlab)
 _PSE = POINTER(RxSeParams)
 
 _SIGNATURES = {
@@ -51,6 +57,10 @@
     "rx_conv3d_bwd_data": (c_int, [c_int, _P, c_void_p, _P, I3, I3, c_int, c_void_p, c_size_t, c_void_p]),
     "rx_conv3d_bwd_data_instats": (c_int, [c_int, _P, c_void_p, _P, I3, I3, c_int, _P, c_void_p, c_float, c_void_p, POINTER(c_int),
                                            c_void_p, c_size_t, c_void_p]),
+    "rx_conv3d_fwd_slab": (c_int, [c_int, _P, c_void_p, c_void_p, _P, I3, I3, c_void_p, c_size_t, _PSL, c_void_p]),
+    "rx_conv3d_bwd_data_slab": (c_int, [c_int, _P, c_void_p, _P, I3, I3, c_int, c_void_p, c_size_t, _PSL, c_void_p]),
+    "rx_instnorm_fwd_slab": (c_int, [c_int, _PSL, _P, c_float, c_void_p, _P, _P, c_float, c_void_p]),
+    "rx_instnorm_act_bwd_slab": (c_int, [c_int, _PSL, _P, _P, c_void_p, _P, c_float, _P, _P, c_int, c_void_p]),
     "rx_instnorm_act_bwd_apply": (c_int, [c_int, _P, _P, c_void_p, _P, c_float, c_void_p, _P, _P, c_int, c_void_p]),
     "rx_conv3d_bwd_weight_workspace": (c_size_t, [_P, _P, I3]),
     "rx_conv3d_bwd_weight": (c_int, [c_int, _P, _P, c_void_p, I3, I3, c_void_p, c_size_t, c_void_p]),
diff --git a/multi-task-3d-resencoder-unet_amd/engine/ops.py b/multi-task-3d-resencoder-unet_amd/engine/ops.py
--- a/multi-task-3d-resencoder-unet_amd/engine/ops.py
+++ b/multi-task-3d-resencoder-unet_amd/engine/ops.py
@@ -321,6 +321,37 @@
     _PROF.run("dgrad:" + LaunchProfiler.igemm_name(dx.voxels, dx.c), 2.0 * n * dy.voxels * dy.c * dx.c * _taps(kernel), 1, go)
 
 
+def conv3d_fwd_slab(x, w_fwd, bias, y, kernel, stride, ws=None):
+    ws = workspace() if ws is None else ws
+    slab = _l.RxSlab()
+
+    def go():
+        check(load().rx_conv3d_fwd_slab(_code(x.dtype), byref(x.desc()), _ptr(w_fwd), _ptr(bias), byref(y.desc()), I3(*kernel),
+                                        I3(*stride), *_ws_args(ws), byref(slab), stream_ptr()), "rx_conv3d_fwd_slab")
+    if _PROF is None:
+        go()
+    else:
+        n = y.dims[0]
+        _PROF.run("fwd:" + LaunchProfiler.igemm_name(y.voxels, y.c), 2.0 * n * y.voxels * y.c * x.c * _taps(kernel), 1, go)
+    return slab if slab.ksplit > 0 else None
+
+
+def conv3d_bwd_data_slab(dy, w_bwd, dx, kernel, stride, accumulate=False, ws=None):
+    ws = workspace() if ws is None else ws
+    slab = _l.RxSlab()
+
+    def go():
+        check(load().rx_conv3d_bwd_data_slab(_code(dy.dtype), byref(dy.desc()), _ptr(w_bwd), byref(dx.desc()), I3(*kernel),
+                                             I3(*stride), int(accumulate), *_ws_args(ws), byref(slab), stream_ptr()),
+              "rx_conv3d_bwd_data_slab")
+    if _PROF is None:
+        go()
+    else:
+        n = dy.dims[0]
+        _PROF.run("dgrad:" + LaunchProfiler.igemm_name(dx.voxels, dx.c), 2.0 * n * dy.voxels * dy.c * dx.c * _taps(kernel), 1, go)
+    return slab if slab.ksplit > 0 else None
+
+
 def conv3d_bwd_data_instats(dy, w_bwd, dx, kernel, stride, accumulate, in_y, in_stats, slope, m12, ws=None):
     from ctypes import c_int
     ws = workspace() if ws is None else ws
@@ -408,6 +439,19 @@
                                      byref(out.desc()) if out is not None else None, float(slope), byref(dy.desc()),
                                      byref(d_residual.desc()) if d_residual is not None else None,
                                      int(accumulate_residual), *_ws_args(ws), stream_ptr()), "rx_instnorm_act_bwd")
+
+
+def instnorm_fwd_slab(slab, y, stats, out, slope=0.01, residual=None, eps=1e-5):
+    check(load().rx_instnorm_fwd_slab(_code(y.dtype), byref(slab), byref(y.desc()), eps, _ptr(stats),
+                                      byref(residual.desc()) if residual is not None else None, byref(out.desc()),
+                                      float(slope), stream_ptr()), "rx_instnorm_fwd_slab")
+
+
+def instnorm_act_bwd_slab(slab, g, y, stats, out, dy, slope=0.01, d_residual=None, accumulate_residual=False):
+    check(load().rx_instnorm_act_bwd_slab(_code(y.dtype), byref(slab), byref(g.desc()), byref(y.desc()), _ptr(stats),
+                                          byref(out.desc()) if out is not None else None, float(slope), byref(dy.desc()),
+                                          byref(d_residual.desc()) if d_residual is not None else None,
+                                          int(accumulate_residual), stream_ptr()), "rx_instnorm_act_bwd_slab")
 
 
 def instnorm_act_bwd_res(g, y, stats, out, dy, d_residual, slope=0.01, pool_dy=None, pool_stride=(1, 1, 1), ws=None):
@@ -663,6 +707,11 @@
 instnorm_act_fwd = _hbm("in_act_fwd", lambda y, stats, out, slope=0.01, residual=None: _tb(y) + _tb(out) + _tb(residual))(instnorm_act_fwd)
 instnorm_fwd = _hbm("in_fwd(stats+apply)", lambda y, stats, out, slope=0.01, residual=None, eps=1e-5, ws=None:
                     _tb(y) + _tb(out) + _tb(residual))(instnorm_fwd)
+instnorm_fwd_slab = _hbm("in_fwd(stats+apply)", lambda slab, y, stats, out, slope=0.01, residual=None, eps=1e-5:
+                         _tb(y) + _tb(out) + _tb(residual))(instnorm_fwd_slab)
+instnorm_act_bwd_slab = _hbm("in_act_bwd(colreduce+apply)",
+                             lambda slab, g, y, stats, out, dy, slope=0.01, d_residual=None, accumulate_residual=False:
+                             _bwd_bytes(g, y, out, dy, d_residual, accumulate_residual))(instnorm_act_bwd_slab)
 instnorm_act_bwd = _hbm("in_act_bwd(colreduce+apply)",
                         lambda g, y, stats, out, dy, slope=0.01, d_residual=None, accumulate_residual=False, ws=None:
                         _bwd_bytes(g, y, out, dy, d_residual, accumulate_residual))(instnorm_act_bwd)
diff --git a/multi-task-3d-resencoder-unet_amd/engine/plan.py b/multi-task-3d-resencoder-unet_amd/engine/plan.py
--- a/multi-task-3d-resencoder-unet_amd/engine/plan.py
+++ b/multi-task-3d-resencoder-unet_amd/engine/plan.py
@@ -540,6 +540,9 @@
                         and rec.a["y"].act.voxels > 512 and rec.a["y"].act.dims[3] >= 16):
                     rec.a["stats_to"] = nxt.a
                     nxt.a["stats_done"] = True
+                if (rec.kind == "conv" and nxt.kind == "inact" and nxt.a["y"] is rec.a["y"] and self.dtype != torch.float32
+                        and nxt.a["gate"] is None and rec.a["y"].act.voxels <= 512 and rec.a["y"].act.c % 32 == 0):
+                    rec.a["slab_to"] = nxt.a
                 if (rec.kind == "stem" and nxt.kind == "inact" and nxt.a["y"] is rec.a["y"] and self.dtype != torch.float32
                         and rec.a["y"].act.voxels > 512):
                     rec.a["stats_to"] = nxt.a
@@ -588,6 +591,10 @@
                             ops.conv3d_fwd_stats(a["x"].act, a["pk"]["w_fwd"], a["b"], a["y"].act, a["kernel"], a["stride"],
                                                  st["stats"], P._eps_now(st))
                             P._mask_dropped(st)
+                            return
+                        sl = a.get("slab_to")
+                        if sl is not None and not (sl["drop"] is not None and sl["drop"]["active"]):
+                            sl["slab"] = ops.conv3d_fwd_slab(a["x"].act, a["pk"]["w_fwd"], a["b"], a["y"].act, a["kernel"], a["stride"])
                         else:
                             ops.conv3d_fwd(a["x"].act, a["pk"]["w_fwd"], a["b"], a["y"].act, a["kernel"], a["stride"])
                     f.append(cstep)
@@ -612,6 +619,10 @@
                 elif rec.kind == "inact":
                     def step(a=a):
                         res = a["res"].act if a["res"] is not None else None
+                        slab = a.pop("slab", None)
+                        if slab is not None:
+                            ops.instnorm_fwd_slab(slab, a["y"].act, a["stats"], a["out"].act, a["slope"], res, a["eps"])
+                            return
                         head = a.get("head_to")
                         if head is not None:
                             if not a.get("stats_done"):
@@ -829,8 +840,21 @@
                         b.append(rstep)
                         continue
 
-                    def istep(a=a, gout=gout, dy=dy, gres=gres, acc=acc):
+                    fold = None
+                    if (gw[0] == "conv" and gw[1].get("pos") == len(b) - 1 and a.get("head_src") is None and "m12" not in a
+                            and self.dtype != torch.float32 and y.act.voxels <= 512 and y.act.c % 32 == 0
+                            and gw[1].get("gx") is gout):
+                        fold = gw[1]
+                        fold["fold"] = True
+
+                    def istep(a=a, gout=gout, dy=dy, gres=gres, acc=acc, fold=fold):
                         before_dy_write(dy)
+                        slab = fold.pop("slab", None) if fold is not None else None
+                        if slab is not None:
+                            ops.instnorm_act_bwd_slab(slab, gout, a["y"].act, a["stats"],
+                                                      a["out"].act if (a["slope"] != 1.0 and a["res"] is not None) else None, dy,
+                                                      a["slope"], gres, acc)
+                            return
                         mask_out = a["out"].act if (a["slope"] != 1.0 and a["res"] is not None) else None
                         hs = a.get("head_src")
                         dl = P._dlogits.get(hs["name"]) if hs is not None else None
@@ -881,14 +905,16 @@
                         x.written = True
                         if x.act.full_buffer:
                             mark_cat(x)
-                        bsinfo = {"inact": None}
+                        bsinfo = {"inact": None, "pos": len(b), "gx": gx}
                         wrote(x, "conv", bsinfo)
 
                         def dstep(a=a, dy=dy, gx=gx, acc=acc, bsinfo=bsinfo):
                             if "dgrad" in skip:
                                 return
                             ia = bsinfo["inact"]
-                            if ia is None:
+                            if ia is None and bsinfo.get("fold"):
+                                bsinfo["slab"] = ops.conv3d_bwd_data_slab(dy, a["pk"]["w_bwd"], gx, a["kernel"], a["stride"], acc)
+                            elif ia is None:
                                 ops.conv3d_bwd_data(dy, a["pk"]["w_bwd"], gx, a["kernel"], a["stride"], acc)
                             else:
                                 ia["m12_valid"] = ops.conv3d_bwd_data_instats(dy, a["pk"]["w_bwd"], gx, a["kernel"], a["stride"], acc,
```

Measured after the change: 118.3 patches/s. No clear change (-0.3%).
